# qinjr/SCoRe

Measured on AMD Instinct MI355X. Metric: train samples/sec @ batch=1024, higher is better.
Workload: dtype f32

## Files before the change

include/score_hip.h:

```cpp
#ifndef SCORE_HIP_H
#define SCORE_HIP_H

#include <stdint.h>

#ifdef __cplusplus
extern "C" {
#endif

#define SCORE_E_BADARG   (-1)
#define SCORE_E_SHAPE    (-2)
#define SCORE_E_WORKSPACE (-3)
#define SCORE_E_INDEX    (-4)

typedef void* score_context_t;
int score_context_create(score_context_t* ctx);
int score_context_destroy(score_context_t ctx);
int score_event_create(void** event);
int score_event_destroy(void* event);
int score_event_record(void* event, void* stream);
int score_stream_wait_event(void* stream, void* event);
int score_event_query(void* event);
int score_event_synchronize(void* event);

typedef struct {
// ... 17 lines not shown
  int32_t eb_dim;
  int32_t hidden_size;
  int32_t max_time_len;
  int32_t obj_per_time_slice;
  int32_t user_fnum;
  int32_t item_fnum;
  int32_t model_type;
} score_config_t;

typedef struct {
  char    name[64];
  int64_t offset;
  int32_t rows, cols;
  int32_t regularised;
  int32_t init;
} score_param_entry_t;

int score_param_layout(const score_config_t* cfg, score_param_entry_t* out, int32_t max_entries,
                       int64_t* n_floats, int64_t* n_reg_floats);

typedef struct {
  const int32_t* user_1hop;
  const int32_t* user_2hop;
  const int32_t* item_1hop;
  const int32_t* item_2hop;
  const int32_t* target_user;
  const int32_t* target_item;
  const int32_t* label;
  const int32_t* length;
  int32_t B;
  int32_t active_slices;
  const int32_t* length2;
} score_batch_t;

typedef struct {
  int64_t total_bytes;
  int64_t xside;
  int64_t atten_info;
  int64_t rsave;
  int64_t query;
  int64_t head_inp;
  int64_t att_score;
  int64_t logit;
  int64_t y_pred;
  int64_t loss;
  int64_t gru_out;
  int64_t gru_final;
  int64_t n_occurrences;
  int64_t plan_meta;
  int64_t plan_unique_rows;
  int64_t plan_remap[6];
} score_workspace_t;

int score_workspace_layout(const score_config_t* cfg, int32_t B, score_workspace_t* out);
int score_workspace_field(const score_config_t* cfg, int32_t B, const char* name, int64_t* offset, int64_t* second);


int score_stream_copy(float* dst, const float* src, int64_t n_floats, void* stream);

int score_table_init(float* table, int64_t n_local_rows, int32_t D, int64_t row_stride, int64_t row_first,
                     int64_t n_global_rows, uint64_t seed, void* stream);

int score_gather_fwd(const float* table, int64_t n_rows, int32_t D, const int32_t* idx,
                     int64_t n_idx, float* out, void* stream);

int score_coattn_fwd(const float* table, int64_t n_rows, int32_t D, int32_t F, int32_t K,
                     int32_t B, int32_t T, const int32_t* idx1, const int32_t* idx2,
                     const float* tgt, const float* W, const float* bias,
                     float* out1, int32_t ld1, float* out2, int32_t ld2,
                     float* info, int32_t ldi, float* rsave, int32_t mode, void* stream);

int score_coattn_bwd(const float* table, float* grad_table, int64_t n_rows, int32_t D, int32_t F,
                     int32_t K, int32_t B, int32_t T, const int32_t* idx1, const int32_t* idx2,
                     const float* W, const float* rsave,
                     const float* g1, int32_t ld1, const float* g2, int32_t ld2,
                     const float* ginfo, int32_t ldi, float* dzsum, float* dW,
                     float* scratch, int64_t scratch_floats, int32_t mode, void* stream);

int score_gemm(int32_t trans, int32_t M, int32_t N, int32_t K,
               const float* A, int32_t lda, const float* Bm, int32_t ldb,
               float* C, int32_t ldc, const float* bias, int32_t flags,
               float keep_prob, const uint8_t* drop_mask, uint64_t drop_seed,
               float* scratch, int64_t scratch_floats, void* stream);

int score_gemm_panel_products(int32_t trans_b, int32_t ngroups, int32_t M, int32_t N, int32_t K,
                              const float* const* A, int32_t lda, const float* const* Bm, int32_t ldb,
                              float* const* C, int32_t ldc, const float* const* bias,
                              float* images, int64_t image_floats, void* stream);
int score_gemm_panel_images(int32_t trans_b, int32_t ngroups, int32_t N, int32_t K, const float* const* Bm, int32_t ldb,
                            float* images, int64_t image_floats, void* stream);
int score_gemm_panel_run(int32_t ngroups, int32_t M, int32_t N, int32_t K, const float* const* A, int32_t lda,
                         float* const* C, int32_t ldc, const float* const* bias, const float* images,
                         int64_t image_floats, void* stream);

int score_gru_fwd(int32_t B, int32_t T, int32_t H, const float* xproj, const float* Wg, int32_t ldwg,
                  const float* Wc, int32_t ldwc, const int32_t* length,
                  float* out, int32_t ldo, float* gates_save, float* final_state, void* stream);

int score_gru_bwd(int32_t B, int32_t T, int32_t H, const float* Wg, int32_t ldwg, const float* Wc,
                  int32_t ldwc, const int32_t* length, const float* out, int32_t ldo,
                  const float* gates_save, const float* dout, int32_t lddo, const float* dfinal,
                  float* dxproj, float* rh, float* hprev, void* stream);

typedef struct {
  const int32_t* id_status;
  int32_t* skipped;
} score_guard_t;

int score_adam(float* p, float* m, float* v, const float* g, int64_t n, int64_t n_reg,
               float l2, float alpha, float beta1, float beta2, float eps, const score_guard_t* guard, void* stream);

int score_adam_dev(float* p, float* m, float* v, const float* g, int64_t n, int64_t n_reg, float l2,
                   const score_step_scalars_t* sc, float beta1, float beta2, float eps, const score_guard_t* guard,
                   void* stream);
int score_adam_rows_dev(float* p, float* m, float* v, const float* g, int64_t n_rows, int32_t D, uint8_t* row_flags,
                        const score_step_scalars_t* sc, float beta1, float beta2, float eps, const score_guard_t* guard,
                        void* stream);

int score_adam_rows(float* p, float* m, float* v, const float* g, int64_t n_rows, int32_t D,
                    uint8_t* row_flags, float alpha, float beta1, float beta2, float eps, const score_guard_t* guard,
                    void* stream);
int score_adam_rows_and_dense(float* p, float* m, float* v, const float* g, int64_t n_rows, int32_t D, uint8_t* row_flags,
                              float* wp, float* wm, float* wv, const float* wg, int64_t n, int64_t n_reg, float l2, float alpha,
                              float beta1, float beta2, float eps, const score_guard_t* guard, void* stream);

#define SCORE_ADAM_RING 64
typedef struct {
  float* p; float* m; float* v;
  const float* g;
  int64_t n_rows;
  int32_t D;
  int32_t reserved;
  uint8_t* row_flags;
  uint32_t* row_step;
  float* alpha_ring;
  float beta1, beta2, eps;
  int32_t reserved2;
  const int32_t* id_status;
  const int32_t* skipped_steps;
} score_adam_table_t;
int score_adam_touched(const score_adam_table_t* t, uint32_t step, float alpha, void* stream);
int score_adam_touched_and_dense(const score_adam_table_t* t, uint32_t step, float alpha, float* p, float* m, float* v,
                                 const float* g, int64_t n, int64_t n_reg, float l2, int32_t* skipped, void* stream);
int score_adam_unmark(const score_adam_table_t* t, uint32_t upto, void* stream);
int score_adam_touched_rows(const score_adam_table_t* t, const int32_t* rows, const int32_t* n_rows_dev, int64_t max_rows,
                            uint32_t step, float alpha, void* stream);
int score_adam_catchup_ids(const score_adam_table_t* t, const int32_t* ids, int64_t n_ids, uint32_t upto, void* stream);
int score_adam_catchup_ids_through(const score_adam_table_t* t, const int32_t* ids, int64_t n_ids, uint32_t step, float alpha,
                                   void* stream);
int score_adam_catchup_rows(const score_adam_table_t* t, int64_t row_begin, int64_t row_end, uint32_t upto, void* stream);


typedef struct {
  const float* table;
  int64_t n_table_rows;
  const float* w;
  float* workspace;
  int64_t workspace_bytes;
  int32_t scatter_mode;
  int32_t global_batch;
  int32_t gemm_mode;
  int32_t debug_flags;
  uint8_t* row_flags;
  void* gather_done_event;
  void* plan_done_event;
  const score_step_scalars_t* step_scalars;
// ... 101 lines not shown
```

score_amd/_lib.py:

```python
import ctypes as C
import os

_HERE = os.path.dirname(os.path.abspath(__file__))
LIB_PATH = os.path.join(_HERE, "lib", "libscore_hip.so")

MODEL_TYPES = {"SCORE": 0, "RIA": 1, "RCA": 2, "SCORE_USER": 3, "SCORE_ITEM": 4, "RRN": 5, "GCMC": 6, "GRU4Rec": 7, "Caser": 8, "DELF": 9,
               "DEEMS": 10, "SVDpp": 11}

MAX_PARAM_ENTRIES = 48

c_f = C.c_void_p
c_i = C.c_void_p


class Config(C.Structure):
    _fields_ = [("feature_size", C.c_int64), ("eb_dim", C.c_int32), ("hidden_size", C.c_int32),
                ("max_time_len", C.c_int32), ("obj_per_time_slice", C.c_int32),
                ("user_fnum", C.c_int32), ("item_fnum", C.c_int32), ("model_type", C.c_int32)]


class ParamEntry(C.Structure):
    _fields_ = [("name", C.c_char * 64), ("offset", C.c_int64), ("rows", C.c_int32), ("cols", C.c_int32),
                ("regularised", C.c_int32), ("init", C.c_int32)]


class Batch(C.Structure):
    _fields_ = [("user_1hop", c_i), ("user_2hop", c_i), ("item_1hop", c_i), ("item_2hop", c_i),
                ("target_user", c_i), ("target_item", c_i), ("label", c_i), ("length", c_i),
                ("B", C.c_int32), ("active_slices", C.c_int32), ("length2", c_i)]


class Workspace(C.Structure):
    _fields_ = [(n, C.c_int64) for n in
                ("total_bytes", "xside", "atten_info", "rsave", "query", "head_inp", "att_score",
                 "logit", "y_pred", "loss", "gru_out", "gru_final", "n_occurrences", "plan_meta",
                 "plan_unique_rows")] + [("plan_remap", C.c_int64 * 6)]


class State(C.Structure):
    _fields_ = [("table", c_f), ("n_table_rows", C.c_int64), ("w", c_f), ("workspace", c_f),
                ("workspace_bytes", C.c_int64), ("scatter_mode", C.c_int32), ("global_batch", C.c_int32),
                ("gemm_mode", C.c_int32), ("debug_flags", C.c_int32), ("row_flags", C.c_void_p),
                ("gather_done_event", C.c_void_p), ("plan_done_event", C.c_void_p), ("step_scalars", C.c_void_p),
                ("context", C.c_void_p), ("id_status", C.c_void_p), ("grads_done_event", C.c_void_p),
                ("loss_done_event", C.c_void_p), ("loss_host", C.c_void_p), ("plan_workspace", C.c_void_p),
                ("reserved4", C.c_int32), ("reserved3", C.c_int32)]


class Graph(C.Structure):
    _fields_ = [(n, C.c_void_p) for n in ("user_off1", "user_nbr1", "user_off2", "user_nbr2", "item_off1", "item_nbr1",
                                           "item_off2", "item_nbr2", "user_rows", "item_rows")] + \
               [(n, C.c_int32) for n in ("n_users", "n_items", "time_slice_num", "user_fnum", "item_fnum", "sample_mode")] + \
               [("user_deg2", C.c_void_p), ("item_deg2", C.c_void_p)]


class BatchOut(C.Structure):
    _fields_ = [(n, C.c_void_p) for n in ("user_1hop", "user_2hop", "item_1hop", "item_2hop", "target_user",
                                           "target_item", "label", "length")]


class AdamTable(C.Structure):
    _fields_ = [("p", C.c_void_p), ("m", C.c_void_p), ("v", C.c_void_p), ("g", C.c_void_p), ("n_rows", C.c_int64),
                ("D", C.c_int32), ("reserved", C.c_int32), ("row_flags", C.c_void_p), ("row_step", C.c_void_p),
                ("alpha_ring", C.c_void_p), ("beta1", C.c_float), ("beta2", C.c_float), ("eps", C.c_float),
                ("reserved2", C.c_int32), ("id_status", C.c_void_p), ("skipped_steps", C.c_void_p)]


class TrainStep(C.Structure):
    _fields_ = [("table", C.c_void_p), ("w", C.c_void_p), ("w_m", C.c_void_p), ("w_v", C.c_void_p), ("w_g", C.c_void_p),
                ("n_w", C.c_int64), ("n_reg", C.c_int64), ("skipped", C.c_void_p), ("reg_lambda", C.c_float),
                ("keep_prob", C.c_float), ("alpha", C.c_float), ("step", C.c_uint32), ("drop_seed", C.c_uint64),
                ("slice_lo", C.c_int64), ("slice_hi", C.c_int64), ("slice_upto", C.c_uint32), ("wait_ahead", C.c_int32),
                ("wait_sweep", C.c_int32), ("next_batch", C.c_void_p), ("next_ids", C.c_void_p), ("n_next_ids", C.c_int64),
                ("next_workspace", C.c_void_p), ("next_workspace_bytes", C.c_int64), ("loss_host", C.c_void_p),
                ("side_stream", C.c_void_p), ("ev_ahead", C.c_void_p), ("ev_sweep", C.c_void_p), ("ev_plan", C.c_void_p),
                ("ev_stage2", C.c_void_p), ("ev_b4", C.c_void_p), ("ev_grads", C.c_void_p), ("ev_loss", C.c_void_p),
                ("ev_plan_next", C.c_void_p), ("fwd_stage_events", C.c_void_p), ("plan_stream", C.c_void_p)]


class Guard(C.Structure):
    _fields_ = [("id_status", C.c_void_p), ("skipped", C.c_void_p)]


ADAM_RING = 64

_SIGS = {
    "score_context_create": [C.POINTER(C.c_void_p)],
    "score_context_destroy": [C.c_void_p],
    "score_id_status": [C.c_void_p, C.POINTER(C.c_int32), C.c_int32, C.c_void_p],
    "score_stream_copy": [c_f, c_f, C.c_int64, C.c_void_p],
    "score_table_init": [c_f, C.c_int64, C.c_int32, C.c_int64, C.c_int64, C.c_int64, C.c_uint64, C.c_void_p],
    "score_batch_assemble": [C.POINTER(Graph), c_i, c_i, C.c_int32, C.c_int32, C.c_int32, C.c_int32, C.c_int32,
                             C.c_int32, C.c_uint64, C.POINTER(BatchOut), C.c_void_p],
    "score_param_layout": [C.POINTER(Config), C.POINTER(ParamEntry), C.c_int32, C.POINTER(C.c_int64),
                           C.POINTER(C.c_int64)],
    "score_workspace_layout": [C.POINTER(Config), C.c_int32, C.POINTER(Workspace)],
    "score_workspace_field": [C.POINTER(Config), C.c_int32, C.c_char_p, C.POINTER(C.c_int64), C.POINTER(C.c_int64)],
    "score_gather_fwd": [c_f, C.c_int64, C.c_int32, c_i, C.c_int64, c_f, C.c_void_p],
    "score_coattn_fwd": [c_f, C.c_int64, C.c_int32, C.c_int32, C.c_int32, C.c_int32, C.c_int32, c_i, c_i,
                         c_f, c_f, c_f, c_f, C.c_int32, c_f, C.c_int32, c_f, C.c_int32, c_f, C.c_int32,
                         C.c_void_p],
    "score_coattn_bwd": [c_f, c_f, C.c_int64, C.c_int32, C.c_int32, C.c_int32, C.c_int32, C.c_int32, c_i, c_i,
                         c_f, c_f, c_f, C.c_int32, c_f, C.c_int32, c_f, C.c_int32, c_f, c_f, c_f, C.c_int64,
                         C.c_int32, C.c_void_p],
    "score_gemm": [C.c_int32, C.c_int32, C.c_int32, C.c_int32, c_f, C.c_int32, c_f, C.c_int32, c_f, C.c_int32,
                   c_f, C.c_int32, C.c_float, C.c_void_p, C.c_uint64, c_f, C.c_int64, C.c_void_p],
    "score_gemm_panel_images": [C.c_int32, C.c_int32, C.c_int32, C.c_int32, C.c_void_p, C.c_int32, c_f, C.c_int64, C.c_void_p],
    "score_gemm_panel_run": [C.c_int32, C.c_int32, C.c_int32, C.c_int32, C.c_void_p, C.c_int32, C.c_void_p, C.c_int32, C.c_void_p,
                             c_f, C.c_int64, C.c_void_p],
    "score_gemm_panel_products": [C.c_int32, C.c_int32, C.c_int32, C.c_int32, C.c_int32, C.c_void_p, C.c_int32, C.c_void_p,
                                  C.c_int32, C.c_void_p, C.c_int32, C.c_void_p, c_f, C.c_int64, C.c_void_p],
    "score_gru_fwd": [C.c_int32, C.c_int32, C.c_int32, c_f, c_f, C.c_int32, c_f, C.c_int32, c_i, c_f, C.c_int32,
                      c_f, c_f, C.c_void_p],
    "score_gru_bwd": [C.c_int32, C.c_int32, C.c_int32, c_f, C.c_int32, c_f, C.c_int32, c_i, c_f, C.c_int32, c_f,
                      c_f, C.c_int32, c_f, c_f, c_f, c_f, C.c_void_p],
    "score_adam": [c_f, c_f, c_f, c_f, C.c_int64, C.c_int64, C.c_float, C.c_float, C.c_float, C.c_float,
                   C.c_float, C.POINTER(Guard), C.c_void_p],
    "score_adam_dev": [c_f, c_f, c_f, c_f, C.c_int64, C.c_int64, C.c_float, C.c_void_p, C.c_float, C.c_float, C.c_float,
                       C.POINTER(Guard), C.c_void_p],
    "score_adam_rows_dev": [c_f, c_f, c_f, c_f, C.c_int64, C.c_int32, C.c_void_p, C.c_void_p, C.c_float, C.c_float,
                            C.c_float, C.POINTER(Guard), C.c_void_p],
    "score_adam_rows": [c_f, c_f, c_f, c_f, C.c_int64, C.c_int32, C.c_void_p, C.c_float, C.c_float, C.c_float,
                        C.c_float, C.POINTER(Guard), C.c_void_p],
    "score_adam_rows_and_dense": [c_f, c_f, c_f, c_f, C.c_int64, C.c_int32, C.c_void_p, c_f, c_f, c_f, c_f, C.c_int64, C.c_int64,
                                  C.c_float, C.c_float, C.c_float, C.c_float, C.c_float, C.POINTER(Guard), C.c_void_p],
    "score_adam_touched": [C.POINTER(AdamTable), C.c_uint32, C.c_float, C.c_void_p],
    "score_adam_touched_and_dense": [C.POINTER(AdamTable), C.c_uint32, C.c_float, c_f, c_f, c_f, c_f, C.c_int64, C.c_int64,
                                     C.c_float, C.c_void_p, C.c_void_p],
    "score_adam_unmark": [C.POINTER(AdamTable), C.c_uint32, C.c_void_p],
    "score_adam_touched_rows": [C.POINTER(AdamTable), c_i, c_i, C.c_int64, C.c_uint32, C.c_float, C.c_void_p],
    "score_adam_catchup_ids": [C.POINTER(AdamTable), c_i, C.c_int64, C.c_uint32, C.c_void_p],
    "score_adam_catchup_ids_through": [C.POINTER(AdamTable), c_i, C.c_int64, C.c_uint32, C.c_float, C.c_void_p],
    "score_adam_catchup_rows": [C.POINTER(AdamTable), C.c_int64, C.c_int64, C.c_uint32, C.c_void_p],
    "score_index_plan": [C.POINTER(Config), C.POINTER(State), C.POINTER(Batch), C.c_int32, C.c_int32, C.c_void_p],
    "score_sort_pairs": [C.c_void_p, C.c_void_p, C.c_void_p, C.c_void_p, C.c_int64, C.c_int32, C.c_void_p, C.c_int64,
                         C.POINTER(C.c_int32), C.c_void_p],
    "score_sort_pairs_temp_bytes": [C.c_int64],
    "score_segment_sum_rows": [c_i, c_f, C.c_int64, C.c_int32, C.c_int64, c_f, C.c_void_p, C.c_void_p, C.c_int64,
                               C.c_void_p],
    "score_segment_sum_scratch_bytes": [C.c_int64, C.c_int32],
    "score_rows_accumulate": [c_i, c_f, C.c_int64, C.c_int32, C.c_int64, c_f, C.c_void_p, C.c_void_p],
    "score_rows_accumulate_multi": [c_i, c_f, C.POINTER(C.c_int64), C.c_int32, C.c_int32, C.c_int64, c_f, C.c_void_p, C.c_void_p],
    "score_auc_logloss": [c_f, c_i, C.c_int64, C.c_void_p, C.c_void_p, C.c_int64, C.c_void_p],
    "score_auc_scratch_bytes": [C.c_int64],
    "score_ranking_quality": [c_f, c_i, C.c_int64, C.c_int32, c_f, c_i, c_f, C.c_int64, C.c_void_p],
    "score_persample_form": [C.POINTER(Config), C.POINTER(State), C.c_int32, C.c_int32],
    "score_event_create": [C.POINTER(C.c_void_p)],
    "score_event_destroy": [C.c_void_p],
    "score_event_record": [C.c_void_p, C.c_void_p],
    "score_stream_wait_event": [C.c_void_p, C.c_void_p],
    "score_event_query": [C.c_void_p],
    "score_event_synchronize": [C.c_void_p],
    "score_abi_struct_sizes": [C.POINTER(C.c_int64), C.c_int32],
    "score_train_step": [C.POINTER(Config), C.POINTER(State), C.POINTER(Batch), C.POINTER(TrainStep), C.c_void_p],
    "score_gemm_forms": [C.POINTER(Config), C.POINTER(State), C.c_int32, C.c_int32, C.POINTER(C.c_int32), C.POINTER(C.c_int32)],
    "score_forward": [C.POINTER(Config), C.POINTER(State), C.POINTER(Batch), C.c_float, C.c_float, C.c_void_p,
                      C.c_void_p, C.c_uint64, C.POINTER(C.c_void_p), C.c_void_p],
    "score_backward": [C.POINTER(Config), C.POINTER(State), C.POINTER(Batch), C.c_float, c_f, c_f,
                       C.POINTER(C.c_void_p), C.c_void_p],
}

EXPORTS = tuple(_SIGS)
_lib = None


class DevEvent(object):
    __slots__ = ("cuda_event", "_lib")

    def __init__(self):
        lib = load()
        h = C.c_void_p(0)
        check(lib.score_event_create(C.byref(h)), "score_event_create")
        self.cuda_event = h.value
        self._lib = lib

    def record(self, stream=None):
        import torch
        s = stream if stream is not None else torch.cuda.current_stream()
        check(self._lib.score_event_record(self.cuda_event, s.cuda_stream), "score_event_record")

    def wait(self, stream=None):
        import torch
        s = stream if stream is not None else torch.cuda.current_stream()
        check(self._lib.score_stream_wait_event(s.cuda_stream, self.cuda_event), "score_stream_wait_event")

    def query(self):
        rc = self._lib.score_event_query(self.cuda_event)
        if rc not in (0, 1):
            check(rc, "score_event_query")
# ... 99 lines not shown
```

score_amd/csrc/engine.hip:

```cpp
#include <string.h>
#include <stdlib.h>
#include <stdio.h>
#include <math.h>
#include <mutex>
#include <new>
#include "common.h"
#include "kernels.h"
#include "persample.h"

namespace {

const int FC1 = 200, FC2 = 80, AT1 = 80, AT2 = 40;
const int CASER_L = SCORE_CASER_L, CASER_HPAD = SCORE_CASER_HPAD;
const int MAX_ENTRIES = 48;

enum Family { FAM_SLICE, FAM_GCMC, FAM_G4R, FAM_CASER, FAM_DELF, FAM_DEEMS, FAM_SVDPP };

struct Dims {
  int64_t N;
  int D, H, T, K, Fu, Fi, mt;
  int Du, Di, I, Dq, NI, Dk, Dhead, nstate;
  int Is[2];
  bool coattn, attn;
  Family family;
// ... 397 lines not shown

void build_ws(const Dims& d, int B, WS* w) {
  struct Memo { bool ok; LayoutKey k; WS w; };
  static thread_local Memo memo = {};
  LayoutKey k = layout_key(d, B);
  if (!memo.ok || !same_key(memo.k, k)) {
    memset(&memo.k, 0, sizeof(memo.k));
    build_ws_raw(d, B, &memo.w);
    memo.k = k; memo.ok = true;
  }
  *w = memo.w;
}

struct SideStream { hipStream_t st; hipEvent_t fork, join, wx; int device; hipStream_t fwd_on; };
#define HIPTRY(call) do { hipError_t e_ = (call); if (e_ != hipSuccess) return (int)e_; } while (0)
#define SCORE_DEVICE_EVENT_FLAGS (hipEventDisableTiming | hipEventDisableSystemFence)
extern "C" int score_event_create(void** event) {
  if (!event) return SCORE_E_BADARG;
  hipEvent_t e;
  HIPTRY(hipEventCreateWithFlags(&e, SCORE_DEVICE_EVENT_FLAGS));
  *event = (void*)e;
  return 0;
}
extern "C" int score_event_destroy(void* event) {
  if (!event) return SCORE_E_BADARG;
  HIPTRY(hipEventDestroy((hipEvent_t)event));
  return 0;
}
extern "C" int score_event_record(void* event, void* stream) {
  if (!event) return SCORE_E_BADARG;
  HIPTRY(hipEventRecord((hipEvent_t)event, (hipStream_t)stream));
  return 0;
}
extern "C" int score_stream_wait_event(void* stream, void* event) {
  if (!event) return SCORE_E_BADARG;
  HIPTRY(hipStreamWaitEvent((hipStream_t)stream, (hipEvent_t)event, 0));
  return 0;
}
extern "C" int score_event_query(void* event) {
  if (!event) return SCORE_E_BADARG;
  const hipError_t e = hipEventQuery((hipEvent_t)event);
  return e == hipSuccess ? 0 : e == hipErrorNotReady ? 1 : (int)e;
}
extern "C" int score_event_synchronize(void* event) {
  if (!event) return SCORE_E_BADARG;
  HIPTRY(hipEventSynchronize((hipEvent_t)event));
  return 0;
}
static int side_stream_create(SideStream* sd) {
  int dev = 0;
  if (hipGetDevice(&dev) != hipSuccess) return SCORE_E_BADARG;
  hipStream_t st; hipEvent_t a, b, c;
  hipError_t e = hipStreamCreateWithFlags(&st, hipStreamNonBlocking);
  if (e != hipSuccess) return (int)e;
  if ((e = hipEventCreateWithFlags(&a, SCORE_DEVICE_EVENT_FLAGS)) != hipSuccess) { hipStreamDestroy(st); return (int)e; }
  if ((e = hipEventCreateWithFlags(&b, SCORE_DEVICE_EVENT_FLAGS)) != hipSuccess) { hipEventDestroy(a); hipStreamDestroy(st); return (int)e; }
  if ((e = hipEventCreateWithFlags(&c, SCORE_DEVICE_EVENT_FLAGS)) != hipSuccess) { hipEventDestroy(a); hipEventDestroy(b); hipStreamDestroy(st); return (int)e; }
  sd->st = st; sd->fork = a; sd->join = b; sd->wx = c; sd->device = dev; sd->fwd_on = nullptr;
  return 0;
}
static void side_stream_release(SideStream* sd) {
  if (!sd->st) return;
  hipStreamSynchronize(sd->st);
  hipEventDestroy(sd->fork); hipEventDestroy(sd->join); hipEventDestroy(sd->wx);
  hipStreamDestroy(sd->st);
  sd->st = nullptr;
}
#define SCORE_MAX_DEVICES 16
static SideStream g_default_ctx[SCORE_MAX_DEVICES];
static std::mutex g_default_mu;
static int side_stream(const score_state_t* st, SideStream** out) {
  if (st && st->context) { *out = reinterpret_cast<SideStream*>(st->context); return 0; }
  int dev = 0;
  if (hipGetDevice(&dev) != hipSuccess || dev < 0 || dev >= SCORE_MAX_DEVICES) return SCORE_E_BADARG;
  std::lock_guard<std::mutex> lock(g_default_mu);
  SideStream& sd = g_default_ctx[dev];
  if (!sd.st) SCORE_TRY(side_stream_create(&sd));
  *out = &sd;
  return 0;
}
enum {
  DF_GRU_STEPWISE = 1, DF_HEAD_FUSED_ANY_B = 2, DF_GRU_F32_REC = 4, DF_NO_PANEL = 8, DF_PANEL_DX = 16, DF_SORT_LIB = 32,
  DF_HEAD_UNFUSED = 64, DF_ATTN_UNFUSED = 128, DF_SORT_OWN = 256, DF_NO_PS = 512, DF_PS_FWD_ONLY = 1024, DF_PS_BWD_ONLY = 2048,
  DF_ONE_STREAM = 4096, DF_G4R_COMPOSED = 8192, DF_PRODUCTS_LATE = 16384
};
struct Flags {
  bool gru_stepwise, head_fused_any_b, gru_f32_rec, no_panel, panel_dx, sort_lib, head_unfused, attn_unfused, sort_own, no_ps,
      ps_fwd_only, ps_bwd_only, one_stream, g4r_composed, products_late;
};
static inline Flags flags_of(const score_state_t* st) {
  auto on = [st](int bit) { return (st->debug_flags & bit) != 0; };
  Flags o;
  o.gru_stepwise = on(DF_GRU_STEPWISE); o.head_fused_any_b = on(DF_HEAD_FUSED_ANY_B); o.gru_f32_rec = on(DF_GRU_F32_REC);
  o.no_panel = on(DF_NO_PANEL); o.panel_dx = on(DF_PANEL_DX); o.sort_lib = on(DF_SORT_LIB); o.sort_own = on(DF_SORT_OWN);
  o.head_unfused = on(DF_HEAD_UNFUSED); o.attn_unfused = on(DF_ATTN_UNFUSED); o.no_ps = on(DF_NO_PS);
  o.ps_fwd_only = on(DF_PS_FWD_ONLY); o.ps_bwd_only = on(DF_PS_BWD_ONLY); o.one_stream = on(DF_ONE_STREAM);
  o.g4r_composed = on(DF_G4R_COMPOSED); o.products_late = on(DF_PRODUCTS_LATE);
  return o;
}
static int side_stream(const score_state_t* st, hipStream_t s, SideStream** out) {
  SideStream* real = nullptr;
  SCORE_TRY(side_stream(st, &real));
  if (!st || !flags_of(st).one_stream) { *out = real; return 0; }
  static thread_local SideStream inl;
  const hipStream_t was = inl.fwd_on;
  inl = *real; inl.st = s; inl.fwd_on = was;
  *out = &inl;
  return 0;
}
static inline int fork_side(SideStream* side, hipStream_t s) {
  HIPTRY(hipEventRecord(side->fork, s));
  HIPTRY(hipStreamWaitEvent(side->st, side->fork, 0));
  return 0;
}

#define G(call) SCORE_TRY(call)
static inline int gemm_mode_call(int x3, int tr, int M, int N, int K, const float* A, int lda, const float* B,
                                 int ldb, float* C, int ldc, const float* bias, int flags, float keep,
                                 const uint8_t* mask, uint64_t seed, float* scratch, int64_t scratch_floats,
                                 void* s) {
  return score_gemm(tr, M, N, K, A, lda, B, ldb, C, ldc, bias, flags | x3, keep, mask, seed, scratch, scratch_floats,
                    s);
}
#define EV(i) \
  do { if (stage_events && stage_events[i]) HIPTRY(hipEventRecord((hipEvent_t)stage_events[i], s)); } while (0)

static inline uint32_t clamp_rows(int64_t n) { return (uint32_t)(n < 0x80000000ll ? n : 0x80000000ll); }
static inline int global_batch(const score_state_t* st, int B) { return st->global_batch > 0 ? st->global_batch : B; }

struct Pass {
  Dims d; Params P; WS w; Flags fl;
  const score_state_t* st; const score_batch_t* bt;
  int B, T, BT, H;
  int x3, Bg;
  uint32_t n_rows;
  int64_t weff_stride;
  float rs;
  float* ws; const float* W; float* scratch;
  hipStream_t s;
};
static int pass_fill(Pass* c, const score_state_t* st, const score_batch_t* bt, void* stream) {
  const Dims& d = c->d;
  build_layout(d, nullptr, 0, &c->P);
  c->st = st; c->bt = bt; c->fl = flags_of(st);
  c->B = bt->B; c->T = active_T(d, bt); c->H = d.H; c->BT = c->B * c->T;
  build_ws(d, c->B, &c->w);
  if (c->w.total * 4 > st->workspace_bytes) return SCORE_E_WORKSPACE;
  c->x3 = st->gemm_mode == 1 ? GF_X3 : 0; c->Bg = global_batch(st, c->B); c->n_rows = clamp_rows(st->n_table_rows);
  c->weff_stride = weff_copy_stride(d); c->rs = (float)(1.0 / sqrt(1.0 + 1e-3));
  c->ws = st->workspace; c->W = st->w; c->scratch = c->ws + c->w.scratch;
  c->s = (hipStream_t)stream;
  return 0;
}
static inline const float* wxcat(const Pass& c, int sd) { return c.ws + c.w.wxcat + (int64_t)sd * (c.d.Ic + 1) * 3 * c.H; }
static int weight_prep(const Pass& c, hipStream_t on) {
  const Dims& d = c.d; const Params& P = c.P; const WS& w = c.w; const float* W = c.W;
  return score_launch_weight_prep(W + P.gk[0], W + P.ck[0], W + P.gb[0], W + P.cb[0], W + P.gk[1], W + P.ck[1], W + P.gb[1],
                                  W + P.cb[1], d.Is[0], d.Is[1], d.Ic, d.H, c.ws + w.wxcat, d.Dk, AT1,
                                  d.attn ? W + P.at_w[1] : nullptr, c.ws + w.weff, c.ws + w.wq, SCORE_WEFF_COPIES, c.weff_stride, W,
                                  P.n_reg, c.ws + w.part, on);
}

static inline const float* gru_x_rows(const Pass& c, int sd) {
  return c.ws + (c.d.family == FAM_GCMC ? c.w.gcmc_z[sd] : (c.d.family == FAM_G4R && sd == 1) ? c.w.gru_out[0] : c.w.xside[sd]);
}

static void gru_header(const Pass& c, GruArgs* ga) {
  memset(ga, 0, sizeof(*ga));
  ga->B = c.B; ga->T = c.T; ga->H = c.H; ga->length = c.bt->length;
  ga->nw8 = 1;
  ga->tmp = c.ws + c.w.gru_tmp; ga->tmp_floats = c.w.gru_tmp_floats;
  ga->x3 = c.x3 != 0; ga->x3_rec = ga->x3 && !c.fl.gru_f32_rec; ga->stepwise = c.fl.gru_stepwise;
}
static void gru_side(const Pass& c, int sd, GruSide* g) {
  const int H = c.H;
  g->Wg = c.W + c.P.gk[sd] + (int64_t)c.d.Is[sd] * 2 * H; g->ldwg = 2 * H;
  g->Wc = c.W + c.P.ck[sd] + (int64_t)c.d.Is[sd] * H; g->ldwc = H;
  g->out = c.ws + c.w.gru_out[sd]; g->ldo = H; g->gates = c.ws + c.w.gates[sd];
}
static void gru_side_saved(const Pass& c, int sd, GruSide* g) {
// ... 216 lines not shown
  const int64_t per = score_gemm_panel_image_floats(p->Nh, p->K);
  for (int g = 0; g < p->n; ++g) {
    const int side = g / ns, half = g % ns;
    const float* cat = wxcat(c, side);
    p->src[g] = which == 0 ? cat + half * p->Nh : cat + (int64_t)half * p->Nh * 3 * H;
    p->img[g] = c.ws + (which == 0 ? c.w.pimg_x : c.w.pimg_d)[side] + half * per;
    PanelGroup& pg = p->pg[g];
    pg.A = A ? A[side] : nullptr; pg.img = p->img[g]; pg.C = C ? C[side] + half * p->Nh : nullptr;
    pg.bias = which == 0 ? cat + (int64_t)d.Is[side] * 3 * H + half * p->Nh : nullptr;
  }
}
static int panel_prep(const Pass& c, int which, hipStream_t on) {
  PanelGroups p;
  panel_groups(c, which, nullptr, nullptr, &p);
  return score_gemm_panel_prep(p.n, p.src, 3 * c.H, p.trans, p.Nh, p.K, p.img, on);
}
static int panel_launch(const Pass& c, int which, const float* const* A, float* const* C) {
  PanelGroups p;
  panel_groups(c, which, A, C, &p);
  return score_gemm_panel(p.n, p.pg, c.BT, p.Nh, p.K, p.lda, p.ldc, c.s);
}

static int loss_tail(const Pass& c, SideStream* sd, float reg_lambda) {
  const WS& w = c.w;
  hipStream_t ls = c.s;
  if (c.st->loss_done_event) { G(fork_side(sd, c.s)); ls = sd->st; }
  G(score_launch_loss_final(c.B, c.ws + w.lossb, c.ws + w.loss, reg_lambda, c.ws + w.part, c.Bg, ls, c.st->id_status));
  if (c.st->loss_done_event) HIPTRY(hipEventRecord((hipEvent_t)c.st->loss_done_event, ls));
  return 0;
}

static int row_scatter(const Pass& c, float* plan, float* grad_table) {
  const Dims& d = c.d; const Params& P = c.P; const WS& w = c.w; float* ws = c.ws; const float* W = c.W;
  PullArgs pa;
  memset(&pa, 0, sizeof(pa));
  pa.D = d.D; pa.K = d.K; pa.zero_is_dummy = 1;
  pa.flags = c.st->scatter_mode == 0 ? c.st->row_flags : nullptr;
  pa.uid = c.st->scatter_mode == 2 ? reinterpret_cast<const uint32_t*>(ws + w.uid) : nullptr;
  const float invK = 1.0f / (float)d.K;
  const float* Gm[6] = {ws + w.dxside[0], ws + w.dxside[1], ws + w.dxside[0], ws + w.dxside[1], ws + w.dtgt, ws + w.dtgt};
  const int ldg[6] = {d.I, d.I, d.I, d.I, d.Dq, d.Dq};
  const int gcol[6] = {0, d.Du, d.Di, 0, 0, d.Du};
  for (int g = 0; g < 6; ++g) { pa.G[g] = Gm[g]; pa.ldg[g] = ldg[g]; pa.gcol[g] = gcol[g]; pa.constA[g] = 1.0f; }
  if (d.coattn) {
    pa.cA[0] = ws + w.pcoef[0]; pa.cA[2] = ws + w.pcoef[1];
    pa.constA[1] = invK; pa.constA[3] = invK;
    pa.cB[0] = pa.cB[1] = ws + w.dzcoef[0]; pa.cB[2] = pa.cB[3] = ws + w.dzcoef[1];
    pa.Wv[0] = W + P.ca_w[0] + d.Di; pa.Wv[1] = W + P.ca_w[0] + 2 * d.Di;
    pa.Wv[2] = W + P.ca_w[1] + d.Du; pa.Wv[3] = W + P.ca_w[1] + 2 * d.Du;
  }
  const int64_t n_occ = (int64_t)c.B * (2 * (int64_t)c.T * d.K * (d.Fu + d.Fi) + d.Fu + d.Fi);
  return score_launch_pull(pa, reinterpret_cast<uint32_t*>(plan + w.keys_out), reinterpret_cast<uint32_t*>(plan + w.vals_out),
                           n_occ + 1, grad_table, ws + w.partials, w.partial_floats, c.s);
}

struct GradQueues { GemmQueue gq; ColsumJobs cq; };
static inline void queues_init(GradQueues* q) { q->gq.n = 0; q->cq.n = 0; q->cq.part_used = 0; }
static int queue_head(const Pass& c, GradQueues* q, float* gw, bool bn1_sums) {
  const Dims& d = c.d; const Params& P = c.P; const WS& w = c.w; float* ws = c.ws; const int B = c.B;
  G(gemm_queue_add(&q->gq, FC2, 1, B, ws + w.f2, FC2, ws + w.dlogit, 1, gw + P.fc_w[2], 1));
  G(colsum_queue_add(&q->cq, ws + w.dlogit, B, 1, 1, gw + P.fc_b[2], 0));
  G(gemm_queue_add(&q->gq, FC1, FC2, B, ws + w.f1, FC1, ws + w.dz2, FC2, gw + P.fc_w[1], FC2));
  G(colsum_queue_add(&q->cq, ws + w.dz2, B, FC2, FC2, gw + P.fc_b[1], 0));
  G(gemm_queue_add(&q->gq, d.Dhead, FC1, B, ws + w.bn, d.Dhead, ws + w.dz1, FC1, gw + P.fc_w[0], FC1));
  G(colsum_queue_add(&q->cq, ws + w.dz1, B, FC1, FC1, gw + P.fc_b[0], 0));
  if (bn1_sums) {
    G(colsum_queue_add(&q->cq, ws + w.dgstage, B, d.Dhead, d.Dhead, gw + P.bn_g, 0));
    G(colsum_queue_add(&q->cq, ws + w.dbn, B, d.Dhead, d.Dhead, gw + P.bn_b, 0));
  }
  return 0;
}
static int queue_head_tower(const Pass& c, GradQueues* q, float* gw, const DeemsArgs& a, int k) {
  const DeemsTower& t = a.t[k]; const DeemsVars v = deems_vars(c.P, k); const int B = c.B, ld = a.ld;
  G(gemm_queue_add(&q->gq, FC2, 1, B, t.f2, FC2, t.dlogit, 1, gw + v.fc_w[2], 1));
  G(colsum_queue_add(&q->cq, t.dlogit, B, 1, 1, gw + v.fc_b[2], 0));
  G(gemm_queue_add(&q->gq, FC1, FC2, B, t.f1, FC1, t.dz2, FC2, gw + v.fc_w[1], FC2));
  G(colsum_queue_add(&q->cq, t.dz2, B, FC2, FC2, gw + v.fc_b[1], 0));
  G(gemm_queue_add(&q->gq, t.Dh, FC1, B, a.bn + t.col, ld, t.dz1, FC1, gw + v.fc_w[0], FC1));
  G(colsum_queue_add(&q->cq, t.dz1, B, FC1, FC1, gw + v.fc_b[0], 0));
  G(colsum_queue_add(&q->cq, a.tmp + t.col, B, t.Dh, ld, gw + v.bn_g, 0));
  G(colsum_queue_add(&q->cq, a.dbn + t.col, B, t.Dh, ld, gw + v.bn_b, 0));
  return 0;
}
static int queue_attn(const Pass& c, GradQueues* q, float* gw) {
  const Dims& d = c.d; const Params& P = c.P; const WS& w = c.w; float* ws = c.ws; const int B = c.B, BT = c.BT;
  G(gemm_queue_add(&q->gq, AT2, 1, BT, ws + w.a2, AT2, ws + w.ds, 1, gw + P.at_w[3], 1));
  G(colsum_queue_add(&q->cq, ws + w.ds, BT, 1, 1, gw + P.at_b[3], 0));
  G(gemm_queue_add(&q->gq, AT1, AT2, BT, ws + w.a1, AT1, ws + w.da2, AT2, gw + P.at_w[2], AT2));
  G(colsum_queue_add(&q->cq, ws + w.da2, BT, AT2, AT2, gw + P.at_b[2], 0));
  G(gemm_queue_add(&q->gq, 2 * d.Dk, AT1, BT, ws + w.ainp, 2 * d.Dk, ws + w.da1, AT1, ws + w.dweff, AT1));
  G(colsum_queue_add(&q->cq, ws + w.da1, BT, AT1, AT1, gw + P.at_b[1], 0));
  G(gemm_queue_add(&q->gq, d.Dk, AT1, B, ws + w.q, d.Dk, ws + w.adzsum, AT1, ws + w.dwq, AT1));
  return 0;
}
static int queue_query(const Pass& c, GradQueues* q, float* gw) {
  const Dims& d = c.d; const Params& P = c.P; const WS& w = c.w;
  G(gemm_queue_add(&q->gq, d.Dq, d.Dk, c.B, c.ws + w.query, d.Dq, c.ws + w.dq, d.Dk, gw + P.at_w[0], d.Dk));
  G(colsum_queue_add(&q->cq, c.ws + w.dq, c.B, d.Dk, d.Dk, gw + P.at_b[0], 0));
  return 0;
}
static int queue_gru_side(const Pass& c, GradQueues* q, float* gw, int sd, int bias_rows) {
  const Dims& d = c.d; const Params& P = c.P; const WS& w = c.w; float* ws = c.ws;
  const int H = c.H, BT = c.BT, Is = d.Is[sd], ld = x_ld(d, sd);
  float* dxp = ws + w.dxproj[sd];
  const float* xin = gru_x_rows(c, sd);
  G(gemm_queue_add(&q->gq, Is, 2 * H, BT, xin, ld, dxp, 3 * H, gw + P.gk[sd], 2 * H));
  G(gemm_queue_add(&q->gq, Is, H, BT, xin, ld, dxp + 2 * H, 3 * H, gw + P.ck[sd], H));
  G(gemm_queue_add(&q->gq, H, 2 * H, BT, ws + w.hprev[sd], H, dxp, 3 * H, gw + P.gk[sd] + (int64_t)Is * 2 * H, 2 * H));
  G(gemm_queue_add(&q->gq, H, H, BT, ws + w.rh[sd], H, dxp + 2 * H, 3 * H, gw + P.ck[sd] + (int64_t)Is * H, H));
  const float* rows = bias_rows > 0 ? gru_bias_slab(c, sd) : dxp;
  const int nrows = bias_rows > 0 ? bias_rows : BT;
  G(colsum_queue_add(&q->cq, rows, nrows, 2 * H, 3 * H, gw + P.gb[sd], 0));
  G(colsum_queue_add(&q->cq, rows + 2 * H, nrows, H, 3 * H, gw + P.cb[sd], 0));
  return 0;
}

static int queue_delf(const Pass& c, GradQueues* q, float* gw) {
  const Dims& d = c.d; const Params& P = c.P; const WS& w = c.w; float* ws = c.ws; const int B = c.B, BT = c.BT;
  const int Cx[2] = {d.Di, d.Du};
  for (int s = 0; s < 2; ++s) {
    G(gemm_queue_add(&q->gq, Cx[s], Cx[s], BT, ws + w.xside[s], d.I, ws + w.delf_dpre[s], Cx[s], gw + P.dl_w[s], Cx[s]));
    G(colsum_queue_add(&q->cq, ws + w.delf_dpre[s], BT, Cx[s], Cx[s], gw + P.dl_b[s], 0));
  }
  const float* tu = ws + w.query; const float* ti = ws + w.query + d.Du;
  const float* ru = ws + w.delf_rep[0]; const float* ri = ws + w.delf_rep[1];
  const float* act = ws + w.delf_act; const float* dact = ws + w.delf_dact;
  const int LA = SCORE_DELF_ACT;
  const float* first[4] = {tu, ru, tu, ti}; const int ld1[4] = {d.Dq, d.Di, d.Dq, d.Dq}; const int n1[4] = {d.Du, d.Di, d.Du, d.Di};
  const float* second[4] = {ti, ri, ri, ru}; const int ld2[4] = {d.Dq, d.Du, d.Du, d.Di}; const int n2[4] = {d.Di, d.Du, d.Du, d.Di};
  for (int k = 0; k < 4; ++k) {
    float* gA = gw + P.dl_w[2 + 2 * k];
    G(gemm_queue_add(&q->gq, n1[k], 10, B, first[k], ld1[k], dact + 10 * k, LA, gA, 10));
    G(gemm_queue_add(&q->gq, n2[k], 10, B, second[k], ld2[k], dact + 10 * k, LA, gA + (int64_t)n1[k] * 10, 10));
    G(colsum_queue_add(&q->cq, dact + 10 * k, B, 10, LA, gw + P.dl_b[2 + 2 * k], 0));
    G(gemm_queue_add(&q->gq, 10, 4, B, act + 10 * k, LA, dact + 40 + 4 * k, LA, gw + P.dl_w[3 + 2 * k], 4));
    G(colsum_queue_add(&q->cq, dact + 40 + 4 * k, B, 4, LA, gw + P.dl_b[3 + 2 * k], 0));
  }
  G(gemm_queue_add(&q->gq, 4, 1, B, act + 56, LA, ws + w.dlogit, 1, gw + P.dl_w[10], 1));
  G(colsum_queue_add(&q->cq, ws + w.dlogit, B, 1, 1, gw + P.dl_b[10], 0));
  return 0;
}

static int queue_svdpp(const Pass& c, GradQueues* q, float* gw) {
  const int nv = c.d.Fu + c.d.Fi;
  for (int k = 0; k < nv; ++k)
    G(colsum_queue_add(&q->cq, c.ws + c.w.svdpp_dw + k, c.B, 1, nv, gw + c.P.sv_w + 4 * (int64_t)k, 0));
  return 0;
}

}

extern "C" int score_context_create(void** ctx) {
  if (!ctx) return SCORE_E_BADARG;
  SideStream* sd = new (std::nothrow) SideStream();
  if (!sd) return SCORE_E_BADARG;
  memset(sd, 0, sizeof(*sd));
  int rc = side_stream_create(sd);
  if (rc != 0) { delete sd; return rc; }
  *ctx = sd;
  return 0;
}

extern "C" int score_context_destroy(void* ctx) {
  if (ctx) {
    SideStream* sd = reinterpret_cast<SideStream*>(ctx);
    side_stream_release(sd);
    delete sd;
    return 0;
  }
  std::lock_guard<std::mutex> lock(g_default_mu);
  for (int i = 0; i < SCORE_MAX_DEVICES; ++i) side_stream_release(&g_default_ctx[i]);
  return 0;
}

extern "C" int score_id_status(int32_t* id_status, int32_t* bits, int32_t clear, void* stream) {
  if (!id_status) return SCORE_E_BADARG;
  hipStream_t s = (hipStream_t)stream;
  int32_t host = 0;
  HIPTRY(hipMemcpyAsync(&host, id_status, sizeof(host), hipMemcpyDeviceToHost, s));
  HIPTRY(hipStreamSynchronize(s));
  if (host && clear) {
    HIPTRY(hipMemsetAsync(id_status, 0, sizeof(host), s));
    HIPTRY(hipStreamSynchronize(s));
  }
  if (bits) *bits = host;
  return host ? SCORE_E_INDEX : 0;
}

extern "C" int score_param_layout(const score_config_t* cfg, score_param_entry_t* out, int32_t max_entries,
                                  int64_t* n_floats, int64_t* n_reg_floats) {
  Dims d;
  SCORE_TRY(make_dims(cfg, &d));
// ... 285 lines not shown

  {
    ReduceGroup rg;
    int cs_done = 0;
    G(gemm_queue_flush(&q.gq, 0, ws + w.dwslab, w.dwslab_floats, fs, &rg, &cq, ws + w.cs_part, w.cs_part_floats, &cs_done));
    W1Fold wf;
    memset(&wf, 0, sizeof(wf));
    wf.Dk = d.Dk; wf.NA = AT1; wf.dweff = ws + w.dweff; wf.dwq = ws + w.dwq; wf.gW1 = gw + P.at_w[1];
    G(score_launch_finish(&rg, &cq, ws + w.cs_part, w.cs_part_floats, fs, cs_done, &wf));
    if (fin_side) HIPTRY(hipEventRecord((hipEvent_t)st->grads_done_event, fs));
  }
  if (st->plan_done_event) HIPTRY(hipStreamWaitEvent(s, (hipEvent_t)st->plan_done_event, 0));
  G(row_scatter(c, st->plan_workspace ? st->plan_workspace : ws, grad_table));
  EV(4);
  EV(5);
  if (st->loss_done_event) HIPTRY(hipStreamWaitEvent(s, (hipEvent_t)st->loss_done_event, 0));
  return 0;
}
}

extern "C" int score_persample_form(const score_config_t* cfg, const score_state_t* st, int32_t B, int32_t active_slices) {
  Dims d;
  SCORE_TRY(make_dims(cfg, &d));
  if (!st || B <= 0 || active_slices < 0) return SCORE_E_BADARG;
  score_batch_t bt;
  memset(&bt, 0, sizeof(bt));
  bt.B = B; bt.active_slices = active_slices;
  PsPlan pp;
  return ps_path(d, st, &bt, active_T(d, &bt), &pp) ? 1 : 0;
}

namespace {
struct FwdState {
  float reg_lambda, keep_prob; const uint8_t *mask0, *mask1; uint64_t seed; void* const* stage_events;
  SideStream* sd;
  bool panel_x;
};

int fwd_open(const Pass& c, FwdState* f) {
  const Dims& d = c.d; const Params& P = c.P; const WS& w = c.w; const score_state_t* st = c.st; const score_batch_t* bt = c.bt;
  float* ws = c.ws; const float* W = c.W; const int B = c.B, x3 = c.x3; hipStream_t s = c.s;
  void* const* stage_events = f->stage_events;
  SideStream* sd = nullptr;
  G(side_stream(st, s, &sd));
  f->sd = sd;
  G(fork_side(sd, s));
  sd->fwd_on = s;
  G(score_launch_target_fwd(st->table, d.D, d.Fu, d.Fi, B, bt->target_user, bt->target_item, ws + w.query, d.Dq,
                            ws + w.head_inp, d.Dhead, d.off_ti, d.off_tu, sd->st, st->n_table_rows, st->id_status));
  G(weight_prep(c, sd->st));
  f->panel_x = panel_gemms(d, st, c.BT, 0);
  if (f->panel_x) G(panel_prep(c, 0, sd->st));
  if (panel_gemms(d, st, c.BT, 1)) G(panel_prep(c, 1, sd->st));
  HIPTRY(hipEventRecord(sd->wx, sd->st));
  if (d.attn) {
    float* scratch2 = ws + w.scratch2;
    G(gemm_mode_call(x3, 0, B, d.Dk, d.Dq, ws + w.query, d.Dq, W + P.at_w[0], d.Dk, ws + w.q, d.Dk, W + P.at_b[0], GF_BIAS,
                     1.f, nullptr, 0, scratch2, w.scratch_floats, sd->st));
    G(gemm_mode_call(x3, 0, B, AT1, d.Dk, ws + w.q, d.Dk, ws + w.wq, AT1, ws + w.qz, AT1, W + P.at_b[1], GF_BIAS, 1.f,
                     nullptr, 0, scratch2, w.scratch_floats, sd->st));
  }
  HIPTRY(hipEventRecord(sd->join, sd->st));
  EV(0);
  {
    CoattnArgs ca;
    CoattnCols k;
    coattn_args(c, &ca, &k);
    ca.id_status = st->id_status;
    ca.c[0].bit1 = 0; ca.c[0].bit2 = 3; ca.c[1].bit1 = 1; ca.c[1].bit2 = 2;
    const int32_t* tidx[2] = {bt->target_item, bt->target_user};
    for (int i = 0; i < 2; ++i) {
      CoattnCall& cc = ca.c[i];
      cc.tgt = ws + w.query + (i ? 0 : d.Du); cc.ldt = d.Dq; cc.tidx = tidx[i];
      cc.bias = d.coattn ? W + P.ca_b[i] : nullptr;
      cc.out1 = ws + w.xside[0] + k.col1[i]; cc.out2 = ws + w.xside[1] + k.col2[i]; cc.info = ws + w.info + k.info_col[i];
    }
    G(score_coattn_fwd_multi(ca, 2, d.D, B, s));
  }
  if (st->gather_done_event) HIPTRY(hipEventRecord((hipEvent_t)st->gather_done_event, s));
  EV(1);
  return 0;
}

int fwd_grus_two_sided(const Pass& c, const FwdState& f, const float* const* xin) {
  const Dims& d = c.d; const WS& w = c.w; float* ws = c.ws; const int H = c.H, BT = c.BT, x3 = c.x3; hipStream_t s = c.s;
  GruArgs ga;
  gru_header(c, &ga);
  float* xp[2] = {ws + w.xproj[0], ws + w.xproj[1]};
  if (d.Is[0] == d.Is[1]) {
    if (f.panel_x) {
      G(panel_launch(c, 0, xin, xp));
    } else {
      const float* Bx[2] = {wxcat(c, 0), wxcat(c, 1)};
      const float* bx[2] = {Bx[0] + (int64_t)d.Is[0] * 3 * H, Bx[1] + (int64_t)d.Is[1] * 3 * H};
      G(score_gemm_same_shape(0, 2, BT, 3 * H, d.Is[0], xin, x_ld(d, 0), Bx, 3 * H, xp, 3 * H, GF_BIAS, x3 != 0, c.scratch,
                              w.scratch_floats, s, bx));
    }
  }
  for (int sd = 0; sd < 2; ++sd) {
    const float* cat = wxcat(c, sd);
    if (d.Is[0] != d.Is[1])
      G(gemm_mode_call(x3, 0, BT, 3 * H, d.Is[sd], xin[sd], x_ld(d, sd), cat, 3 * H, xp[sd], 3 * H, cat + (int64_t)d.Is[sd] * 3 * H,
                       GF_BIAS, 1.f, nullptr, 0, c.scratch, w.scratch_floats, s));
    gru_side(c, sd, &ga.s[sd]);
    ga.s[sd].xproj = xp[sd]; ga.s[sd].final_state = ws + w.gru_final[sd];
  }
  return score_gru_fwd_multi(ga, 2, s);
}

int fwd_attention(const Pass& c, const FwdState& f) {
  const Dims& d = c.d; const Params& P = c.P; const WS& w = c.w; const score_batch_t* bt = c.bt;
  float* ws = c.ws; const float* W = c.W; const int B = c.B, T = c.T, H = c.H, BT = c.BT, x3 = c.x3; hipStream_t s = c.s;
  HIPTRY(hipStreamWaitEvent(s, f.sd->join, 0));
  int frc = c.fl.attn_unfused ? SCORE_E_SHAPE
                : score_launch_attn_fwd_fused(B, T, H, d.NI, AT1, AT2, ws + w.q, ws + w.gru_out[0], ws + w.gru_out[1],
                                              ws + w.info, ws + w.weff, ws + w.qz, W + P.at_w[2], W + P.at_b[2],
                                              W + P.at_w[3], W + P.at_b[3], bt->length, ws + w.ainp, ws + w.a1, ws + w.a2,
                                              ws + w.att_score, ws + w.head_inp, d.Dhead, d.off_u, d.off_i, s,
                                              SCORE_WEFF_COPIES, c.weff_stride);
  if (frc != SCORE_E_SHAPE) return frc;
  G(score_launch_attn_build_inp(B, T, H, d.NI, ws + w.q, ws + w.gru_out[0], ws + w.gru_out[1], ws + w.info,
                                ws + w.ainp, s));
  G(gemm_mode_call(x3, 0, BT, AT1, 2 * d.Dk, ws + w.ainp, 2 * d.Dk, ws + w.weff, AT1, ws + w.a1, AT1, ws + w.qz,
                   GF_BIAS | GF_RELU | (T << 16), 1.f, nullptr, 0, c.scratch, w.scratch_floats, s));
  int trc = c.fl.attn_unfused ? SCORE_E_SHAPE
                : score_launch_attn_tail_fwd(B, T, H, AT1, AT2, ws + w.a1, W + P.at_w[2], W + P.at_b[2], W + P.at_w[3],
                                             W + P.at_b[3], bt->length, ws + w.gru_out[0], ws + w.gru_out[1], ws + w.a2,
                                             ws + w.att_score, ws + w.head_inp, d.Dhead, d.off_u, d.off_i, s);
  if (trc != SCORE_E_SHAPE) return trc;
  G(gemm_mode_call(x3, 0, BT, AT2, AT1, ws + w.a1, AT1, W + P.at_w[2], AT2, ws + w.a2, AT2, W + P.at_b[2],
                   GF_BIAS | GF_RELU, 1.f, nullptr, 0, c.scratch, w.scratch_floats, s));
  return score_launch_attn_pool_fwd(B, T, H, AT2, ws + w.a2, W + P.at_w[3], W + P.at_b[3], bt->length,
                                    ws + w.gru_out[0], ws + w.gru_out[1], ws + w.att_score, ws + w.head_inp, d.Dhead,
                                    d.off_u, d.off_i, s);
}

int fwd_fc_head(const Pass& c, const FwdState& f) {
  const Dims& d = c.d; const Params& P = c.P; const WS& w = c.w; const score_state_t* st = c.st; const score_batch_t* bt = c.bt;
  float* ws = c.ws; const float* W = c.W; const int B = c.B, x3 = c.x3; hipStream_t s = c.s;
  const float keep_prob = f.keep_prob;
  const int dflag = keep_prob < 1.f ? GF_DROP : 0;
  int hrc = c.fl.head_unfused ? SCORE_E_SHAPE
                : score_launch_head_fwd_fused(B, d.Dhead, FC1, FC2, ws + w.head_inp, W + P.bn_g, W + P.bn_b, c.rs, W + P.fc_w[0],
                                              W + P.fc_b[0], W + P.fc_w[1], W + P.fc_b[1], W + P.fc_w[2], W + P.fc_b[2],
                                              keep_prob, f.mask0, f.mask1, f.seed, f.seed ^ 0x5DEECE66Dull,
                                              bt->label, ws + w.bn, ws + w.f1, ws + w.f2, ws + w.logit, ws + w.y_pred,
                                              ws + w.lossb, ws + w.dlogit, c.Bg, s,
                                              st->step_scalars ? &st->step_scalars->drop_seed : nullptr, ws + w.dz2,
                                              c.fl.head_fused_any_b ? 1 : 0);
  if (hrc == 0) return loss_tail(c, f.sd, f.reg_lambda);
  if (hrc != SCORE_E_SHAPE) return hrc;
  if (st->step_scalars && keep_prob < 1.f) return SCORE_E_SHAPE;
  G(score_launch_bn_fwd(B, d.Dhead, ws + w.head_inp, W + P.bn_g, W + P.bn_b, c.rs, ws + w.bn, s));
  G(gemm_mode_call(x3, 0, B, FC1, d.Dhead, ws + w.bn, d.Dhead, W + P.fc_w[0], FC1, ws + w.f1, FC1, W + P.fc_b[0],
                   GF_BIAS | GF_RELU | dflag, keep_prob, f.mask0, f.seed, c.scratch, w.scratch_floats, s));
  G(gemm_mode_call(x3, 0, B, FC2, FC1, ws + w.f1, FC1, W + P.fc_w[1], FC2, ws + w.f2, FC2, W + P.fc_b[1],
                   GF_BIAS | GF_RELU | dflag, keep_prob, f.mask1, f.seed ^ 0x5DEECE66Dull, c.scratch, w.scratch_floats, s));
  G(score_launch_head_out(B, FC2, ws + w.f2, W + P.fc_w[2], W + P.fc_b[2], bt->label, ws + w.logit, ws + w.y_pred,
                          ws + w.lossb, ws + w.dlogit, ws + w.loss, f.reg_lambda, ws + w.part, c.Bg, s, st->id_status));
  if (st->loss_done_event) HIPTRY(hipEventRecord((hipEvent_t)st->loss_done_event, s));
  return 0;
}

int fwd_slice(const Pass& c, const FwdState& f) {
  const Dims& d = c.d; const WS& w = c.w; float* ws = c.ws; const int B = c.B, H = c.H; hipStream_t s = c.s;
  void* const* stage_events = f.stage_events;
  HIPTRY(hipStreamWaitEvent(s, f.sd->wx, 0));
  const float* xin[2] = {ws + w.xside[0], ws + w.xside[1]};
  G(fwd_grus_two_sided(c, f, xin));
  EV(2);
  if (d.attn) {
    G(fwd_attention(c, f));
  } else {
    G(score_launch_copy2d(B, H, ws + w.gru_final[0], H, ws + w.head_inp, d.Dhead, s));
    G(score_launch_copy2d(B, H, ws + w.gru_final[1], H, ws + w.head_inp + H, d.Dhead, s));
  }
  EV(3);
  if (!d.attn) HIPTRY(hipStreamWaitEvent(s, f.sd->join, 0));
  G(fwd_fc_head(c, f));
  EV(4);
  return 0;
}

int fwd_gcmc(const Pass& c, const FwdState& f) {
  const Dims& d = c.d; const Params& P = c.P; const WS& w = c.w;
  float* ws = c.ws; const float* W = c.W; const int B = c.B, H = c.H, BT = c.BT; hipStream_t s = c.s;
  void* const* stage_events = f.stage_events;
  for (int sd = 0; sd < 2; ++sd) {
    const int Dx = d.Is[sd];
    G(gemm_mode_call(c.x3, 0, BT, Dx, Dx, ws + w.xside[sd], d.I, W + P.gm_a[sd], Dx, ws + w.gcmc_a[sd], Dx, nullptr, GF_RELU, 1.f,
                     nullptr, 0, c.scratch, w.scratch_floats, s));
    G(gemm_mode_call(c.x3, 0, BT, Dx, Dx, ws + w.gcmc_a[sd], Dx, W + P.gm_c[sd], Dx, ws + w.gcmc_z[sd], Dx, nullptr, GF_RELU, 1.f,
                     nullptr, 0, c.scratch, w.scratch_floats, s));
  }
  HIPTRY(hipStreamWaitEvent(s, f.sd->wx, 0));
  const float* xin[2] = {ws + w.gcmc_z[0], ws + w.gcmc_z[1]};
  G(fwd_grus_two_sided(c, f, xin));
  EV(2);
  EV(3);
  HIPTRY(hipStreamWaitEvent(s, f.sd->join, 0));
// ... 97 lines not shown
extern "C" int score_forward(const score_config_t* cfg, const score_state_t* st, const score_batch_t* bt,
                             float reg_lambda, float keep_prob, const uint8_t* drop_mask0,
                             const uint8_t* drop_mask1, uint64_t drop_seed, void* const* stage_events,
                             void* stream) {
  Pass c;
  SCORE_TRY(make_dims(cfg, &c.d));
  if (!st || !bt || !st->table || !st->w || !st->workspace || bt->B <= 0) return SCORE_E_BADARG;
  if (!bt->user_1hop || !bt->user_2hop || !bt->item_1hop || !bt->item_2hop || !bt->target_user ||
      !bt->target_item || !bt->label || !bt->length)
    return SCORE_E_BADARG;
  if ((c.d.family == FAM_DELF || c.d.family == FAM_DEEMS) && !bt->length2) return SCORE_E_BADARG;
  if (!(keep_prob > 0.f) || keep_prob > 1.f) return SCORE_E_BADARG;
  SCORE_TRY(pass_fill(&c, st, bt, stream));
  {
    PsPlan pp;
    if (!c.fl.ps_bwd_only && ps_path(c.d, st, bt, c.T, &pp))
      return forward_ps(c, pp, reg_lambda, keep_prob, drop_mask0, drop_mask1, drop_seed, stage_events);
  }
  FwdState f = {reg_lambda, keep_prob, drop_mask0, drop_mask1, drop_seed, stage_events, nullptr, false};
  SCORE_TRY(fwd_open(c, &f));
  switch (c.d.family) {
    case FAM_SLICE: return fwd_slice(c, f);
    case FAM_GCMC: return fwd_gcmc(c, f);
    case FAM_G4R: return fwd_g4r(c, f);
    case FAM_CASER: return fwd_caser(c, f);
    case FAM_DELF: return fwd_delf(c, f);
    case FAM_DEEMS: return fwd_deems(c, f);
    case FAM_SVDPP: return fwd_svdpp(c, f);
  }
  return SCORE_E_BADARG;
}

namespace {
struct BwdState {
  float keep_prob; float* gw; float* grad_table; void* const* stage_events;
  SideStream* side;
  GradQueues q;
  const float* dfinal[2];
  int gru_bias_rows;
};
inline int64_t slab_half(const WS& w) { return (w.dwslab_floats / 4) & ~(int64_t)3; }

int bwd_open(const Pass& c, BwdState* b) {
  hipStream_t s = c.s;
  void* const* stage_events = b->stage_events;
  SideStream* side = nullptr;
  G(side_stream(c.st, s, &side));
  b->side = side;
  const bool forked = side->fwd_on == s;
  side->fwd_on = nullptr;
  if (!forked) G(fork_side(side, s));
  HIPTRY(hipMemsetAsync(b->gw, 0, c.P.n_floats * sizeof(float), side->st));
  EV(0);
  return 0;
}

int bwd_fc_head(const Pass& c, BwdState* b) {
  const Dims& d = c.d; const Params& P = c.P; const WS& w = c.w;
  float* ws = c.ws; const float* W = c.W; float* gw = b->gw; const int B = c.B, x3 = c.x3; hipStream_t s = c.s;
  const float keep_prob = b->keep_prob; const int64_t SF = w.scratch_floats;
  if (c.fl.head_unfused || !score_head_fwd_fused_fits(B, d.Dhead, FC1, FC2))
    G(score_launch_outer_relu_bwd(B, FC2, ws + w.dlogit, W + P.fc_w[2], ws + w.f2, keep_prob, ws + w.dz2, s));
  int hbrc = c.fl.head_unfused ? SCORE_E_SHAPE
                 : score_launch_head_bwd_fused(B, d.Dhead, FC1, FC2, ws + w.dz2, W + P.fc_w[1], ws + w.f1, keep_prob,
                                               W + P.fc_w[0], ws + w.head_inp, W + P.bn_g, c.rs, ws + w.dz1, ws + w.dbn,
                                               ws + w.dhead, ws + w.dgstage, s);
  if (hbrc != 0 && hbrc != SCORE_E_SHAPE) return hbrc;
  G(queue_head(c, &b->q, gw, hbrc == 0));
  if (hbrc == SCORE_E_SHAPE) {
    G(gemm_mode_call(x3, 1, B, FC1, FC2, ws + w.dz2, FC2, W + P.fc_w[1], FC2, ws + w.dz1, FC1, nullptr, GF_RELUGRAD, keep_prob,
                     reinterpret_cast<const uint8_t*>(ws + w.f1), 0, c.scratch, SF, s));
    G(gemm_mode_call(x3, 1, B, d.Dhead, FC1, ws + w.dz1, FC1, W + P.fc_w[0], FC1, ws + w.dbn, d.Dhead, nullptr, 0, 1.f,
                     nullptr, 0, c.scratch, SF, s));
    G(score_launch_bn_bwd(B, d.Dhead, ws + w.head_inp, W + P.bn_g, c.rs, ws + w.dbn, ws + w.dhead, gw + P.bn_g,
                          gw + P.bn_b, ws + w.dgstage, c.scratch, SF, &b->q.cq, s));
  }
  return 0;
}

int bwd_attention(const Pass& c, BwdState* b) {
  const Dims& d = c.d; const Params& P = c.P; const WS& w = c.w; const score_batch_t* bt = c.bt;
  float* ws = c.ws; const float* W = c.W; const int B = c.B, T = c.T, H = c.H, BT = c.BT, x3 = c.x3; hipStream_t s = c.s;
  const int64_t SF = w.scratch_floats;
  G(queue_attn(c, &b->q, b->gw));
  const bool pool_in_fused = !c.fl.attn_unfused && (int64_t)B * T < 8192 &&
                             score_attn_inp_bwd_fused_fits(B, T, H, d.NI, AT1, AT2, d.Dhead, d.off_u, d.off_i, true);
  int prc = pool_in_fused ? 0 : c.fl.attn_unfused ? SCORE_E_SHAPE
                : score_launch_attn_pool_bwd(B, T, H, AT2, ws + w.a2, W + P.at_w[3], bt->length, ws + w.gru_out[0],
                                             ws + w.gru_out[1], ws + w.att_score, ws + w.dhead, d.Dhead, d.off_u,
                                             d.off_i, ws + w.ds, ws + w.da2, s, AT1, W + P.at_w[2], ws + w.a1, ws + w.da1);
  if (prc != 0 && prc != SCORE_E_SHAPE) return prc;
  const bool da1_done = prc == 0;
  if (!da1_done) {
    G(score_launch_attn_pool_bwd(B, T, H, AT2, ws + w.a2, W + P.at_w[3], bt->length, ws + w.gru_out[0],
                                 ws + w.gru_out[1], ws + w.att_score, ws + w.dhead, d.Dhead, d.off_u, d.off_i,
                                 ws + w.ds, ws + w.da2, s));
    G(gemm_mode_call(x3, 1, BT, AT1, AT2, ws + w.da2, AT2, W + P.at_w[2], AT2, ws + w.da1, AT1, nullptr, GF_RELUGRAD, 1.f,
                     reinterpret_cast<const uint8_t*>(ws + w.a1), 0, c.scratch, SF, s));
  }
  int brc = c.fl.attn_unfused ? SCORE_E_SHAPE
            : pool_in_fused
                ? score_launch_attn_inp_bwd_fused(B, T, H, d.NI, AT1, nullptr, ws + w.weff, ws + w.q, ws + w.gru_out[0],
                                                  ws + w.gru_out[1], ws + w.info, ws + w.att_score, ws + w.dhead, d.Dhead,
                                                  d.off_u, d.off_i, ws + w.dgru[0], ws + w.dgru[1], ws + w.dinfo, ws + w.dq, s,
                                                  AT2, ws + w.a2, ws + w.a1, W + P.at_w[3], W + P.at_w[2], bt->length,
                                                  ws + w.ds, ws + w.da2, ws + w.da1)
                : score_launch_attn_inp_bwd_fused(B, T, H, d.NI, AT1, ws + w.da1, ws + w.weff, ws + w.q, ws + w.gru_out[0],
                                                  ws + w.gru_out[1], ws + w.info, ws + w.att_score, ws + w.dhead, d.Dhead,
                                                  d.off_u, d.off_i, ws + w.dgru[0], ws + w.dgru[1], ws + w.dinfo, ws + w.dq, s);
  if (pool_in_fused && brc != 0) return brc == SCORE_E_SHAPE ? SCORE_E_BADARG : brc;
  if (brc != 0 && brc != SCORE_E_SHAPE) return brc;
  if (brc == SCORE_E_SHAPE) {
    G(gemm_mode_call(x3, 1, BT, 2 * d.Dk, AT1, ws + w.da1, AT1, ws + w.weff, AT1, ws + w.dainp, 2 * d.Dk, nullptr, 0,
                     1.f, nullptr, 0, c.scratch, SF, s));
    G(score_launch_attn_inp_bwd(B, T, H, d.NI, ws + w.dainp, ws + w.q, ws + w.gru_out[0], ws + w.gru_out[1],
                                ws + w.info, ws + w.att_score, ws + w.dhead, d.Dhead, d.off_u, d.off_i,
                                nullptr, ws + w.dgru[0], ws + w.dgru[1], ws + w.dinfo, ws + w.dq, s));
  }
  return 0;
}

int bwd_zero_dinfo(const Pass& c) {
  HIPTRY(hipMemsetAsync(c.ws + c.w.dinfo, 0, (int64_t)c.BT * 4 * c.d.K * sizeof(float), c.s));
  return 0;
}
int bwd_final_state(const Pass& c, BwdState* b, int sd, int head_col, bool zero_dout) {
  const WS& w = c.w; float* ws = c.ws; const int H = c.H;
  if (head_col >= 0) G(score_launch_copy2d(c.B, H, ws + w.dhead + head_col, c.d.Dhead, ws + w.dfinal[sd], H, c.s));
  b->dfinal[sd] = ws + w.dfinal[sd];
  if (zero_dout) HIPTRY(hipMemsetAsync(ws + w.dgru[sd], 0, (int64_t)c.BT * H * sizeof(float), c.s));
  return 0;
}
int bwd_final_states(const Pass& c, BwdState* b, bool from_head) {
  for (int sd = 0; sd < 2; ++sd) G(bwd_final_state(c, b, sd, from_head ? sd * c.H : -1, true));
  return bwd_zero_dinfo(c);
}

int bwd_side_products(const Pass& c, BwdState* b) {
  const Dims& d = c.d; const Params& P = c.P; const WS& w = c.w; const score_state_t* st = c.st;
  float* ws = c.ws; const float* W = c.W; float* gw = b->gw; const int B = c.B, x3 = c.x3; hipStream_t s = c.s;
  const int64_t SF = w.scratch_floats;
  SideStream* side = b->side;
  G(fork_side(side, s));
  const bool q_on_side = st->scatter_mode != 2;
  hipStream_t qs = q_on_side ? side->st : s;
  if (d.attn) {
    float* scratch2 = q_on_side ? ws + w.scratch2 : c.scratch;
    G(score_launch_attn_dzsum(B, c.T, AT1, ws + w.da1, ws + w.adzsum, qs));
    G(gemm_mode_call(x3, 1, B, d.Dk, AT1, ws + w.adzsum, AT1, ws + w.wq, AT1, ws + w.dq, d.Dk, nullptr, GF_ACC, 1.f, nullptr,
                     0, scratch2, SF, qs));
    G(queue_query(c, &b->q, gw));
    G(gemm_mode_call(x3, 1, B, d.Dq, d.Dk, ws + w.dq, d.Dk, W + P.at_w[0], d.Dk, ws + w.dquery, d.Dq, nullptr, 0, 1.f,
                     nullptr, 0, scratch2, SF, qs));
    if (q_on_side) HIPTRY(hipEventRecord(side->wx, side->st));
    else G(fork_side(side, s));
  }
  G(gemm_queue_flush(&b->q.gq, x3 != 0, ws + w.dwslab, slab_half(w), side->st));
  if (d.attn) G(score_launch_attn_w1_grad(d.Dk, AT1, ws + w.dweff, ws + w.dwq, gw + P.at_w[1], side->st));
  if (q_on_side) G(colsum_queue_flush(&b->q.cq, ws + w.cs_part, w.cs_part_floats / 2, side->st));
  HIPTRY(hipEventRecord(side->join, side->st));
  return 0;
}

int bwd_grus_two_sided(const Pass& c, BwdState* b) {
  GruArgs ga;
  gru_header(c, &ga);
  for (int sd = 0; sd < 2; ++sd) {
    gru_side(c, sd, &ga.s[sd]);
    gru_side_bwd(c, sd, b->dfinal[sd], &ga.s[sd]);
  }
  G(score_gru_bwd_multi(ga, 2, c.s));
  b->gru_bias_rows = ga.bias_slab_rows;
  return 0;
}

int bwd_dx_slice(const Pass& c, BwdState* b) {
  const Dims& d = c.d; const WS& w = c.w; float* ws = c.ws; const int H = c.H, BT = c.BT, x3 = c.x3; hipStream_t s = c.s;
  const int64_t SF = w.scratch_floats;
  for (int sd = 0; sd < 2; ++sd) {
    G(queue_gru_side(c, &b->q, b->gw, sd, b->gru_bias_rows));
    if (d.Is[sd] != d.I)
      HIPTRY(hipMemsetAsync(ws + w.dxside[sd], 0, (int64_t)BT * d.I * sizeof(float), s));
    if (d.Is[0] != d.Is[1])
      G(gemm_mode_call(x3, 1, BT, d.Is[sd], 3 * H, ws + w.dxproj[sd], 3 * H, wxcat(c, sd), 3 * H, ws + w.dxside[sd], d.I, nullptr, 0,
                       1.f, nullptr, 0, c.scratch, SF, s));
  }
  if (d.Is[0] == d.Is[1]) {
    const float* Ad[2] = {ws + w.dxproj[0], ws + w.dxproj[1]};
    float* Cd[2] = {ws + w.dxside[0], ws + w.dxside[1]};
    if (panel_gemms(d, c.st, BT, 1)) {
      G(panel_launch(c, 1, Ad, Cd));
    } else {
      const float* Bd[2] = {wxcat(c, 0), wxcat(c, 1)};
      G(score_gemm_same_shape(1, 2, BT, d.Is[0], 3 * H, Ad, 3 * H, Bd, 3 * H, Cd, d.I, 0, x3 != 0, c.scratch, SF, s));
    }
  }
  return 0;
}

int bwd_dx_gcmc(const Pass& c, BwdState* b) {
  const Dims& d = c.d; const Params& P = c.P; const WS& w = c.w;
  float* ws = c.ws; const float* W = c.W; float* gw = b->gw; const int H = c.H, BT = c.BT, x3 = c.x3; hipStream_t s = c.s;
  const int64_t SF = w.scratch_floats;
  GemmQueue& gq = b->q.gq;
  for (int sd = 0; sd < 2; ++sd) {
    G(queue_gru_side(c, &b->q, gw, sd, b->gru_bias_rows));
    HIPTRY(hipMemsetAsync(ws + w.dxside[sd], 0, (int64_t)BT * d.I * sizeof(float), s));
    const int Dx = d.Is[sd];
    float* dz = ws + w.gcmc_dz[sd];
    float* da = ws + w.gcmc_da[sd];
    G(gemm_mode_call(x3, 1, BT, Dx, 3 * H, ws + w.dxproj[sd], 3 * H, wxcat(c, sd), 3 * H, dz, Dx, nullptr, GF_RELUGRAD, 1.f,
                     reinterpret_cast<const uint8_t*>(ws + w.gcmc_z[sd]), 0, c.scratch, SF, s));
    G(gemm_queue_add(&gq, Dx, Dx, BT, ws + w.gcmc_a[sd], Dx, dz, Dx, gw + P.gm_c[sd], Dx));
    G(gemm_mode_call(x3, 1, BT, Dx, Dx, dz, Dx, W + P.gm_c[sd], Dx, da, Dx, nullptr, GF_RELUGRAD, 1.f,
                     reinterpret_cast<const uint8_t*>(ws + w.gcmc_a[sd]), 0, c.scratch, SF, s));
    G(gemm_queue_add(&gq, Dx, Dx, BT, ws + w.xside[sd], d.I, da, Dx, gw + P.gm_a[sd], Dx));
    G(gemm_mode_call(x3, 1, BT, Dx, Dx, da, Dx, W + P.gm_a[sd], Dx, ws + w.dxside[sd], d.I, nullptr, 0, 1.f, nullptr, 0,
                     c.scratch, SF, s));
  }
  return 0;
}

int bwd_dx_g4r(const Pass& c, BwdState* b) {
  const Dims& d = c.d; const WS& w = c.w; float* ws = c.ws; const int H = c.H, BT = c.BT; hipStream_t s = c.s;
  G(queue_gru_side(c, &b->q, b->gw, 0, b->gru_bias_rows));
  HIPTRY(hipMemsetAsync(ws + w.dxside[0], 0, (int64_t)BT * d.I * sizeof(float), s));
  G(gemm_mode_call(c.x3, 1, BT, d.Di, 3 * H, ws + w.dxproj[0], 3 * H, wxcat(c, 0), 3 * H, ws + w.dxside[0], d.I, nullptr, 0, 1.f,
                   nullptr, 0, c.scratch, w.scratch_floats, s));
  G(queue_gru_side(c, &b->q, b->gw, 1, b->gru_bias_rows));
  HIPTRY(hipMemsetAsync(ws + w.dxside[1], 0, (int64_t)BT * d.I * sizeof(float), s));
  return 0;
}

int bwd_close(const Pass& c, BwdState* b) {
  const Dims& d = c.d; const Params& P = c.P; const WS& w = c.w; const score_state_t* st = c.st; const score_batch_t* bt = c.bt;
  float* ws = c.ws; const float* W = c.W; float* gw = b->gw; float* grad_table = b->grad_table;
  const int B = c.B, x3 = c.x3; hipStream_t s = c.s;
  void* const* stage_events = b->stage_events;
  SideStream* side = b->side;
  GemmQueue& gq = b->q.gq;
  ColsumJobs& cq = b->q.cq;
  const int64_t half = slab_half(w);
  ReduceGroup rg; rg.n = rg.blocks = 0;
  const bool products_early = st->scatter_mode != 2 && !c.fl.products_late && gq.n > 0;
  const bool fin_side = st->grads_done_event != nullptr;
  const bool fin_early = products_early && fin_side;
  if (products_early) {
    G(fork_side(side, s));
    G(gemm_queue_flush(&gq, x3 != 0, ws + w.dwslab + half, w.dwslab_floats - half, side->st, &rg));
    HIPTRY(hipEventRecord(side->join, side->st));
  }
  EV(3);
  const bool atomic = st->scatter_mode == 1;
  {
    CoattnArgs ca;
    CoattnCols k;
    coattn_args(c, &ca, &k);
    ca.gtable = grad_table;
    for (int i = 0; i < 2; ++i) {
      CoattnCall& cc = ca.c[i];
      cc.g1 = ws + w.dxside[0] + k.col1[i]; cc.g2 = ws + w.dxside[1] + k.col2[i]; cc.ginfo = ws + w.dinfo + k.info_col[i];
      cc.dzsum = ws + w.dzsum[i]; cc.pcoef = ws + w.pcoef[i]; cc.dzcoef = ws + w.dzcoef[i];
    }
// ... 201 lines not shown
```

score_amd/csrc/gemm.hip:

```cpp
#include <cstring>
#include "common.h"
#include "kernels.h"

typedef float f32x16 __attribute__((ext_vector_type(16)));

#define BK_ALIGN 32
#ifndef GEMM_SPLITK_MIN_K
#define GEMM_SPLITK_MIN_K 512
#define GEMM_SPLITK_MIN_CHUNK 128
#endif

#define KF_MASK (15 | 64 | 0x7FFF0000)

template <int TRANS, int WM, int WN, int BK>
__device__ __forceinline__ void gemm_f32_body(const GemmGroup& grp, int blk, const float* __restrict__ bias, int flags,
                                              float keep, const uint8_t* __restrict__ mask, uint64_t seed) {
  int pi = 0, local = blk;
  while (pi + 1 < grp.n && local >= ((grp.p[pi].nblocks + 7) & ~7)) { local -= (grp.p[pi].nblocks + 7) & ~7; ++pi; }
  const GemmProb& pr = grp.p[pi];
  if (local >= pr.nblocks) return;
  const int M = pr.M, N = pr.N, K = pr.K, lda = pr.lda, ldb = pr.ldb, ldc = pr.ldc, k_chunk = pr.k_chunk;
  const float* __restrict__ A = pr.A;
  const float* __restrict__ Bm = pr.B;
  float* __restrict__ C = pr.C;
// ... 103 lines not shown
    __syncthreads();
    if (k0 + BK >= kend) break;
    store_tiles(ra1, rb1);
    __syncthreads();
    if (k0 + 3 * BK < kend) load_tiles(k0 + 3 * BK, ra1, rb1);
    mfma_tile();
    __syncthreads();
  }

#pragma unroll
  for (int i = 0; i < WM; ++i)
#pragma unroll
    for (int j = 0; j < WN; ++j) {
      const int col = bn + bcol + 32 * j;
      if (col >= N) continue;
#pragma unroll
      for (int r = 0; r < 16; ++r) {
        const int row = bm + wm * 32 * WM + 32 * i + (r & 3) + 8 * (r >> 2) + 4 * khalf;
        if (row >= M) continue;
        if (slab) {
          slab[((int64_t)bz * M + row) * N + col] = acc[i][j][r];
        } else {
          float v = gemm_epilogue(acc[i][j][r], row, col, N, pr.bias ? pr.bias : bias, flags, keep, mask, seed);
          float* dst = C + (int64_t)row * ldc + col;
          *dst = (flags & GF_ACC) ? *dst + v : v;
        }
      }
    }
}
template <int TRANS, int WM, int WN, int BK>
__global__ __launch_bounds__(256) void gemm_f32_kernel(const GemmGroup grp, const float* __restrict__ bias, int flags,
                                                       float keep, const uint8_t* __restrict__ mask, uint64_t seed) {
  gemm_f32_body<TRANS, WM, WN, BK>(grp, (int)blockIdx.x, bias, flags, keep, mask, seed);
}

__global__ void splitk_reduce_kernel(const float* __restrict__ slab, int nsplit, int M, int N,
                                     float* __restrict__ C, int ldc, const float* __restrict__ bias, int flags,
                                     float keep, const uint8_t* __restrict__ mask, uint64_t seed) {
  int64_t i = (int64_t)blockIdx.x * blockDim.x + threadIdx.x;
  if (i >= (int64_t)M * N) return;
  int row = (int)(i / N), col = (int)(i - (int64_t)row * N);
  const int64_t stride = (int64_t)M * N;
  float s = 0.f;
  int z = 0;
  for (; z + 8 <= nsplit; z += 8) {
    float v[8];
#pragma unroll
    for (int q = 0; q < 8; ++q) v[q] = slab[(int64_t)(z + q) * stride + i];
#pragma unroll
    for (int q = 0; q < 8; ++q) s += v[q];
  }
  for (; z < nsplit; ++z) s += slab[(int64_t)z * stride + i];
  float v = gemm_epilogue(s, row, col, N, bias, flags, keep, mask, seed);
  float* dst = C + (int64_t)row * ldc + col;
  *dst = (flags & GF_ACC) ? *dst + v : v;
}

__device__ __forceinline__ void splitk_reduce_group_body(const ReduceGroup& g, int blk) {
  int ji = 0;
  while (ji + 1 < g.n && blk >= g.j[ji + 1].first_block) ++ji;
  const ReduceJob& job = g.j[ji];
  const int64_t n = (int64_t)job.M * job.N;
  const int64_t i = (int64_t)(blk - job.first_block) * blockDim.x + threadIdx.x;
  if (i >= n) return;
  const int row = (int)(i / job.N), col = (int)(i - (int64_t)row * job.N);
  float s = 0.f;
  int z = 0;
  for (; z + 8 <= job.ns; z += 8) {
    float v[8];
#pragma unroll
    for (int q = 0; q < 8; ++q) v[q] = job.slab[(int64_t)(z + q) * n + i];
#pragma unroll
    for (int q = 0; q < 8; ++q) s += v[q];
  }
  for (; z < job.ns; ++z) s += job.slab[(int64_t)z * n + i];
  job.C[(int64_t)row * job.ldc + col] = s;
}
__global__ void splitk_reduce_group_kernel(const ReduceGroup g) { splitk_reduce_group_body(g, (int)blockIdx.x); }

static void fill_prob(GemmProb* p, int M, int N, int K, const float* A, int lda, const float* B, int ldb, float* C,
                      int ldc, int k_chunk, float* slab, int gx, int gy, int gz) {
  p->A = A; p->B = B; p->C = C; p->slab = slab; p->bias = nullptr; p->M = M; p->N = N; p->K = K; p->lda = lda; p->ldb = ldb;
  p->ldc = ldc; p->k_chunk = k_chunk; p->gx = gx; p->gy = gy; p->nblocks = gx * gy * gz;
}

extern "C" int score_gemm(int32_t trans, int32_t M, int32_t N, int32_t K, const float* A, int32_t lda,
                          const float* Bm, int32_t ldb, float* C, int32_t ldc, const float* bias,
                          int32_t flags, float keep_prob, const uint8_t* drop_mask, uint64_t drop_seed,
                          float* scratch, int64_t scratch_floats, void* stream) {
  if (!A || !Bm || !C || M <= 0 || N <= 0 || K <= 0) return SCORE_E_BADARG;
  if (trans < 0 || trans > 2) return SCORE_E_BADARG;
  if ((flags & GF_BIAS) && !bias) return SCORE_E_BADARG;
  if (flags < 0) return SCORE_E_BADARG;
  if ((flags & GF_RELUGRAD) && (!drop_mask || (flags & GF_DROP))) return SCORE_E_BADARG;
  hipStream_t s = (hipStream_t)stream;
  const bool a_kc = trans != 2, b_kc = trans == 1;
  const bool al_a = (lda & 3) == 0 && (reinterpret_cast<uintptr_t>(A) & 15) == 0;
  const bool al_b = (ldb & 3) == 0 && (reinterpret_cast<uintptr_t>(Bm) & 15) == 0;
  const bool x3_ok = al_a && al_b && (a_kc ? (K & 3) == 0 : (M & 3) == 0) && (b_kc ? (K & 3) == 0 : (N & 3) == 0);
  const bool x3_shape = (trans == 0 && M >= 4096 && N >= 64) ||
                        (trans == 1 && M >= 4096 && N >= 256) ||
                        (trans == 2 && (int64_t)M * N >= 32768 && K >= 4096);
  const bool x3_force = (flags & 32) != 0;
  if ((flags & (GF_X3 | 32)) && x3_ok && M >= 64 && N >= 32 && K >= 32 && (x3_shape || x3_force)) {
    auto rounds = [&](int wm_) {
      int64_t blocks = (int64_t)((N + 127) / 128) * ((M + 64 * wm_ - 1) / (64 * wm_));
      return (double)((blocks + 255) / 256) * (wm_ == 2 ? 1.0 : 0.57);
    };
    const int wm3 = rounds(1) < rounds(2) ? 1 : 2;
    dim3 g3((N + 127) / 128, (M + 64 * wm3 - 1) / (64 * wm3), 1);
    int ns = 1;
    int64_t t3 = (int64_t)g3.x * g3.y;
    if (t3 < 256 && K >= 512 && scratch) {
      ns = (int)((320 + t3 - 1) / t3);
      if (ns > K / 128) ns = K / 128;
      while (ns > 1 && (int64_t)ns * M * N > scratch_floats) --ns;
      if (ns < 1) ns = 1;
    }
    int kc = K;
    float* sl = nullptr;
    if (ns > 1) {
      kc = (int)align_up64(cdiv64(K, ns), 32);
      ns = (int)cdiv64(K, kc);
      g3.z = ns;
      sl = ns > 1 ? scratch : nullptr;
    }
    GemmGroup grp;
    grp.n = 1;
    fill_prob(&grp.p[0], M, N, K, A, lda, Bm, ldb, C, ldc, kc, sl, (int)g3.x, (int)g3.y, (int)g3.z);
    grp.total_blocks = (grp.p[0].nblocks + 7) & ~7;
    SCORE_TRY(score_launch_gemm_bf16x3(trans, wm3, grp, bias, flags & KF_MASK, keep_prob, drop_mask, drop_seed, s));
    if (sl) {
      int64_t n = (int64_t)M * N;
      hipLaunchKernelGGL(splitk_reduce_kernel, dim3((unsigned)cdiv64(n, 256)), dim3(256), 0, s, sl, ns, M, N, C, ldc,
                         bias, flags & KF_MASK, keep_prob, drop_mask, drop_seed);
      SCORE_CHECK_LAUNCH();
    }
    return 0;
  }
  flags &= KF_MASK;
  int WMs = 1, WNs = 1;
  auto nblocks = [&](int wm_, int wn_) { return (int64_t)((N + 64 * wn_ - 1) / (64 * wn_)) * ((M + 64 * wm_ - 1) / (64 * wm_)); };
  const int64_t want = 384;
  const int64_t ksplit_cap = (K >= GEMM_SPLITK_MIN_K && scratch) ? K / GEMM_SPLITK_MIN_CHUNK : 1;
  if (N > 64 && nblocks(1, 2) * ksplit_cap >= want) WNs = 2;
  if (M > 64 && nblocks(2, WNs) * ksplit_cap >= want) WMs = 2;
  const int BMh = 64 * WMs, BNh = 64 * WNs;
  dim3 grid((N + BNh - 1) / BNh, (M + BMh - 1) / BMh, 1);
  int nsplit = 1;
  int64_t tiles = (int64_t)grid.x * grid.y;
  if (tiles < 256 && K >= GEMM_SPLITK_MIN_K && scratch) {
    nsplit = (int)((320 + tiles - 1) / tiles);
    int max_split = K / GEMM_SPLITK_MIN_CHUNK;
    if (nsplit > max_split) nsplit = max_split;
    while (nsplit > 1 && (int64_t)nsplit * M * N > scratch_floats) --nsplit;
    if (nsplit < 1) nsplit = 1;
  }
  int k_chunk = K;
  float* slab = nullptr;
  if (nsplit > 1) {
    k_chunk = (int)align_up64(cdiv64(K, nsplit), BK_ALIGN);
    nsplit = (int)cdiv64(K, k_chunk);
    grid.z = nsplit;
    slab = nsplit > 1 ? scratch : nullptr;
  }
  GemmGroup grp;
  grp.n = 1;
  fill_prob(&grp.p[0], M, N, K, A, lda, Bm, ldb, C, ldc, k_chunk, slab, (int)grid.x, (int)grid.y, (int)grid.z);
  grp.total_blocks = (grp.p[0].nblocks + 7) & ~7;
#define LAUNCH(TR, WMv, WNv)                                                                                       \
  hipLaunchKernelGGL((gemm_f32_kernel<TR, WMv, WNv, 16>), dim3(grp.total_blocks), dim3(256), 0, s, grp, bias, flags, \
                     keep_prob, drop_mask, drop_seed)
#define LAUNCH_T(TR)                                      \
  do {                                                    \
    if (WMs == 2 && WNs == 2) LAUNCH(TR, 2, 2);           \
    else if (WMs == 2) LAUNCH(TR, 2, 1);                  \
    else if (WNs == 2) LAUNCH(TR, 1, 2);                  \
    else LAUNCH(TR, 1, 1);                                \
  } while (0)
  if (trans == 0) LAUNCH_T(0);
  else if (trans == 1) LAUNCH_T(1);
  else LAUNCH_T(2);
#undef LAUNCH_T
#undef LAUNCH
  SCORE_CHECK_LAUNCH();
  if (slab) {
    int64_t n = (int64_t)M * N;
    hipLaunchKernelGGL(splitk_reduce_kernel, dim3((unsigned)cdiv64(n, 256)), dim3(256), 0, s, slab, nsplit, M, N,
                       C, ldc, bias, flags, keep_prob, drop_mask, drop_seed);
    SCORE_CHECK_LAUNCH();
  }
  return 0;
}

int score_gemm_same_shape(int trans, int nprob, int M, int N, int K, const float* const* A, int lda,
                          const float* const* B, int ldb, float* const* C, int ldc, int flags, int x3, float* scratch,
                          int64_t scratch_floats, hipStream_t s, const float* const* bias) {
  if (nprob <= 0 || nprob > GEMM_GROUP_MAX || trans < 0 || trans > 2 || (flags & ~(GF_ACC | GF_BIAS))) return SCORE_E_BADARG;
  if ((flags & GF_BIAS) && !bias) return SCORE_E_BADARG;
  bool al = (lda & 3) == 0 && (ldb & 3) == 0;
  for (int i = 0; i < nprob; ++i)
    al = al && (reinterpret_cast<uintptr_t>(A[i]) & 15) == 0 && (reinterpret_cast<uintptr_t>(B[i]) & 15) == 0;
  const bool a_kc = trans != 2, b_kc = trans == 1;
  const bool x3_ok = al && (a_kc ? (K & 3) == 0 : (M & 3) == 0) && (b_kc ? (K & 3) == 0 : (N & 3) == 0) && M >= 64 &&
                     N >= 32 && K >= 32;
  const bool x3_shape = (trans == 0 && M >= 4096 && N >= 64) || (trans == 1 && M >= 4096 && N >= 256);
  GemmGroup grp;
  grp.n = nprob; grp.total_blocks = 0;
  if (x3 && x3_ok && x3_shape) {
    const int64_t t2 = (int64_t)nprob * ((N + 127) / 128) * ((M + 127) / 128);
    const int64_t t1 = (int64_t)nprob * ((N + 127) / 128) * ((M + 63) / 64);
    auto rounds = [](int64_t blocks, double w) { return (double)((blocks + 255) / 256) * w; };
    const int wm = rounds(t1, 0.57) < rounds(t2, 1.0) ? 1 : 2;
    if ((wm == 2 ? t2 : t1) >= 128) {
      for (int i = 0; i < nprob; ++i) {
        fill_prob(&grp.p[i], M, N, K, A[i], lda, B[i], ldb, C[i], ldc, K, nullptr, (N + 127) / 128,
                  (M + 64 * wm - 1) / (64 * wm), 1);
        grp.p[i].bias = bias ? bias[i] : nullptr;
        grp.total_blocks += (grp.p[i].nblocks + 7) & ~7;
      }
      return score_launch_gemm_bf16x3(trans, wm, grp, nullptr, flags, 1.f, nullptr, 0, s);
    }
  }
  const int64_t tiles = (int64_t)nprob * ((N + 63) / 64) * ((M + 63) / 64);
  if (tiles < 128 && K >= GEMM_SPLITK_MIN_K && scratch) {
    for (int i = 0; i < nprob; ++i)
      SCORE_TRY(score_gemm(trans, M, N, K, A[i], lda, B[i], ldb, C[i], ldc, bias ? bias[i] : nullptr, flags | (x3 ? GF_X3 : 0),
                           1.f, nullptr, 0, scratch, scratch_floats, s));
    return 0;
  }
  for (int i = 0; i < nprob; ++i) {
    fill_prob(&grp.p[i], M, N, K, A[i], lda, B[i], ldb, C[i], ldc, K, nullptr, (N + 63) / 64, (M + 63) / 64, 1);
    grp.p[i].bias = bias ? bias[i] : nullptr;
    grp.total_blocks += (grp.p[i].nblocks + 7) & ~7;
  }
#define LS(TR) hipLaunchKernelGGL((gemm_f32_kernel<TR, 1, 1, 16>), dim3(grp.total_blocks), dim3(256), 0, s, grp, nullptr, \
                                  flags, 1.f, nullptr, 0)
  if (trans == 0) LS(0); else if (trans == 1) LS(1); else LS(2);
#undef LS
  SCORE_CHECK_LAUNCH();
  return 0;
}

int gemm_queue_add(GemmQueue* q, int M, int N, int K, const float* A, int lda, const float* B, int ldb, float* C,
                   int ldc) {
  if (!q || !A || !B || !C || M <= 0 || N <= 0 || K <= 0) return SCORE_E_BADARG;
  if (q->n >= 2 * GEMM_GROUP_MAX) return SCORE_E_WORKSPACE;
  GemmQueueJob& j = q->j[q->n++];
  j.A = A; j.B = B; j.C = C; j.M = M; j.N = N; j.K = K; j.lda = lda; j.ldb = ldb; j.ldc = ldc;
  return 0;
}

__global__ void gemm_colsum_kernel(const GemmGroup grp, const ColsumJobs jobs, float* __restrict__ part, int gemm_blocks, int gx);
int gemm_queue_flush(GemmQueue* q, int x3, float* slab, int64_t slab_floats, hipStream_t s, ReduceGroup* defer,
                     const ColsumJobs* with_colsums, float* cs_part, int64_t cs_part_floats, int* colsums_done) {
  if (colsums_done) *colsums_done = 0;
  if (defer) defer->n = defer->blocks = 0;
  if (!q || q->n == 0) return 0;
  if (!slab) return SCORE_E_BADARG;
  GemmGroup g3, gf;
  g3.n = gf.n = 0; g3.total_blocks = gf.total_blocks = 0;
  int fam[2 * GEMM_GROUP_MAX];
  int64_t work[2] = {0, 0};
  for (int i = 0; i < q->n; ++i) {
    const GemmQueueJob& j = q->j[i];
    const bool al = (j.lda & 3) == 0 && (j.ldb & 3) == 0 && (reinterpret_cast<uintptr_t>(j.A) & 15) == 0 &&
                    (reinterpret_cast<uintptr_t>(j.B) & 15) == 0 && (j.M & 3) == 0 && (j.N & 3) == 0;
    fam[i] = (x3 && al && j.M >= 64 && j.N >= 32 && (int64_t)j.M * j.N >= 16384 && j.K >= 4096) ? 1 : 0;
    const int64_t tiles = fam[i] ? (int64_t)((j.M + 127) / 128) * ((j.N + 127) / 128)
                                 : (int64_t)((j.M + 63) / 64) * ((j.N + 63) / 64);
    work[fam[i]] += tiles * j.K;
  }
  int kc[2];
  kc[1] = (int)align_up64(cdiv64(work[1] > 0 ? work[1] : 1, 512), 32);
  if (kc[1] < 256) kc[1] = 256;
  for (int guard = 0; guard < 256; ++guard) {
    int64_t blocks = 0;
    for (int i = 0; i < q->n; ++i)
      if (fam[i]) {
        const GemmQueueJob& j = q->j[i];
        blocks += ((int64_t)((j.M + 127) / 128) * ((j.N + 127) / 128) * cdiv64(j.K, kc[1]) + 7) & ~(int64_t)7;
      }
    if (blocks <= 512 || kc[1] >= 1 << 24) break;
    kc[1] += (int)align_up64(kc[1] / 64 > 32 ? kc[1] / 64 : 32, 32);
  }
  kc[0] = (int)align_up64(cdiv64(work[0] > 0 ? work[0] : 1, 1024), BK_ALIGN);
  if (kc[0] < 128) kc[0] = 128;
  ReduceGroup rg;
  rg.n = 0;
  int rblocks = 0;
  int64_t used = 0;
  for (int i = 0; i < q->n; ++i) {
    const GemmQueueJob& j = q->j[i];
    GemmGroup& g = fam[i] ? g3 : gf;
    if (g.n >= GEMM_GROUP_MAX) return SCORE_E_WORKSPACE;
    const int gx = fam[i] ? (j.N + 127) / 128 : (j.N + 63) / 64, gy = fam[i] ? (j.M + 127) / 128 : (j.M + 63) / 64;
    int chunk = kc[fam[i]];
    int ns = (int)cdiv64(j.K, chunk);
    const int64_t mn = (int64_t)j.M * j.N;
    while (ns > 1 && used + (int64_t)ns * mn > slab_floats) {
      chunk *= 2;
      ns = (int)cdiv64(j.K, chunk);
    }
    float* sl = nullptr;
    if (ns > 1) {
      sl = slab + used;
      used += align_up64((int64_t)ns * mn, 4);
      ReduceJob& r = rg.j[rg.n++];
      r.slab = sl; r.C = j.C; r.ns = ns; r.M = j.M; r.N = j.N; r.ldc = j.ldc; r.first_block = rblocks; r.pad = 0;
      rblocks += (int)cdiv64(mn, 256);
    } else {
      chunk = j.K;
    }
    fill_prob(&g.p[g.n], j.M, j.N, j.K, j.A, j.lda, j.B, j.ldb, j.C, j.ldc, chunk, sl, gx, gy, ns);
    g.total_blocks += (g.p[g.n].nblocks + 7) & ~7;
    ++g.n;
  }
  if (g3.n) SCORE_TRY(score_launch_gemm_bf16x3(2, 2, g3, nullptr, 0, 1.f, nullptr, 0, s));
  if (gf.n && with_colsums && with_colsums->n > 0 && cs_part && with_colsums->part_used <= cs_part_floats) {
    int gx = 1;
    for (int i = 0; i < with_colsums->n; ++i)
      gx = max(gx, (with_colsums->job[i].N + with_colsums->job[i].cols - 1) / with_colsums->job[i].cols);
    const int64_t cs_blocks = (int64_t)gx * COLSUM_MAX_PARTS * with_colsums->n;
    hipLaunchKernelGGL(gemm_colsum_kernel, dim3((unsigned)(gf.total_blocks + cs_blocks)), dim3(256), 0, s, gf, *with_colsums, cs_part,
                       gf.total_blocks, gx);
    SCORE_CHECK_LAUNCH();
    if (colsums_done) *colsums_done = 1;
  } else if (gf.n) {
    hipLaunchKernelGGL((gemm_f32_kernel<2, 1, 1, 16>), dim3(gf.total_blocks), dim3(256), 0, s, gf, nullptr, 0, 1.f, nullptr,
                       0);
    SCORE_CHECK_LAUNCH();
  }
  rg.blocks = rblocks;
  if (defer) {
    *defer = rg;
  } else if (rg.n) {
    hipLaunchKernelGGL(splitk_reduce_group_kernel, dim3(rblocks), dim3(256), 0, s, rg);
    SCORE_CHECK_LAUNCH();
  }
  q->n = 0;
  return 0;
}

__global__ __launch_bounds__(256) void colsum_stage1(const float* __restrict__ X, int M, int N, int ld, int cols,
                                                     int rows_per_block, float* __restrict__ part) {
  __shared__ float sh[256];
  const int tx = threadIdx.x % cols, ty = threadIdx.x / cols, nty = 256 / cols;
  const int n = blockIdx.x * cols + tx;
  const int m0 = blockIdx.y * rows_per_block, m1 = min(M, m0 + rows_per_block);
  float s = 0.f;
  if (n < N)
    for (int m = m0 + ty; m < m1; m += nty) s += X[(int64_t)m * ld + n];
  sh[threadIdx.x] = s;
  __syncthreads();
  if (ty == 0 && n < N) {
    float t = 0.f;
    for (int r = 0; r < nty; ++r) t += sh[r * cols + tx];
    part[(int64_t)blockIdx.y * N + n] = t;
  }
}
__global__ void colsum_stage2(const float* __restrict__ part, int nparts, int N, float* __restrict__ out,
                              int accumulate) {
  int n = blockIdx.x * blockDim.x + threadIdx.x;
  if (n >= N) return;
  float s = 0.f;
  for (int p = 0; p < nparts; ++p) s += part[(int64_t)p * N + n];
  out[n] = accumulate ? out[n] + s : s;
}

int score_launch_colsum(const float* X, int M, int N, int ld, float* out, int accumulate, float* scratch,
                        int64_t scratch_floats, hipStream_t s) {
  int cols = 1;
  while (cols < N && cols < 64) cols <<= 1;
  int rpb = 128;
  int nparts = (M + rpb - 1) / rpb;
  if (nparts > 32) { nparts = 32; rpb = (M + nparts - 1) / nparts; nparts = (M + rpb - 1) / rpb; }
  if ((int64_t)nparts * N > scratch_floats) return SCORE_E_WORKSPACE;
  hipLaunchKernelGGL(colsum_stage1, dim3((N + cols - 1) / cols, nparts), dim3(256), 0, s, X, M, N, ld, cols, rpb,
                     scratch);
  SCORE_CHECK_LAUNCH();
  hipLaunchKernelGGL(colsum_stage2, dim3((N + 63) / 64), dim3(64), 0, s, scratch, nparts, N, out, accumulate);
  SCORE_CHECK_LAUNCH();
  return 0;
}

__device__ __forceinline__ void colsum_multi_stage1_body(const ColsumJobs& jobs, float* __restrict__ part, int bx, int by, int bz) {
  __shared__ float sh[256];
  const ColsumJob& j = jobs.job[bz];
  const int cols = j.cols, nty = 256 / cols;
  if (by >= j.nparts || bx * cols >= j.N) return;
  const int tx = threadIdx.x % cols, ty = threadIdx.x / cols;
  const int n = bx * cols + tx;
  const int m0 = by * j.rpb, m1 = min(j.M, m0 + j.rpb);
  float s = 0.f;
  if (n < j.N) {
    const float* x = j.X + n;
    int m = m0 + ty;
    float s0 = 0.f, s1 = 0.f, s2 = 0.f, s3 = 0.f;
    if (j.scale) {
      const float* sc = j.scale;
      for (; m + 3 * nty < m1; m += 4 * nty) {
        const float v0 = x[(int64_t)m * j.ld], v1 = x[(int64_t)(m + nty) * j.ld];
        const float v2 = x[(int64_t)(m + 2 * nty) * j.ld], v3 = x[(int64_t)(m + 3 * nty) * j.ld];
        const float c0 = sc[m], c1 = sc[m + nty], c2 = sc[m + 2 * nty], c3 = sc[m + 3 * nty];
        s0 = fmaf(v0, c0, s0); s1 = fmaf(v1, c1, s1); s2 = fmaf(v2, c2, s2); s3 = fmaf(v3, c3, s3);
      }
      for (; m < m1; m += nty) s0 = fmaf(x[(int64_t)m * j.ld], sc[m], s0);
    } else {
      for (; m + 3 * nty < m1; m += 4 * nty) {
        const float v0 = x[(int64_t)m * j.ld], v1 = x[(int64_t)(m + nty) * j.ld];
        const float v2 = x[(int64_t)(m + 2 * nty) * j.ld], v3 = x[(int64_t)(m + 3 * nty) * j.ld];
        s0 += v0; s1 += v1; s2 += v2; s3 += v3;
      }
      for (; m < m1; m += nty) s0 += x[(int64_t)m * j.ld];
    }
    s = (s0 + s1) + (s2 + s3);
  }
  sh[threadIdx.x] = s;
  __syncthreads();
  if (ty == 0 && n < j.N) {
    float t = 0.f;
    for (int r = 0; r < nty; ++r) t += sh[r * cols + tx];
    part[j.part_off + (int64_t)by * j.N + n] = t;
  }
// ... 140 lines not shown
```

score_amd/csrc/gemm_bf16x3.hip:

```cpp
#include <type_traits>
#include "common.h"
#include "kernels.h"

typedef __bf16 bf16x8 __attribute__((ext_vector_type(8)));
typedef float f32x16 __attribute__((ext_vector_type(16)));

#define TBN 128
#define TBK 32
#define TLD 40

template <int TRANS, int WM>
__global__ __launch_bounds__(256, 2) void gemm_bf16x3_kernel(const GemmGroup grp, const float* __restrict__ bias, int flags,
                                                             float keep, const uint8_t* __restrict__ mask,
                                                             uint64_t seed) {
  int pi = 0, local = (int)blockIdx.x;
  while (pi + 1 < grp.n && local >= ((grp.p[pi].nblocks + 7) & ~7)) { local -= (grp.p[pi].nblocks + 7) & ~7; ++pi; }
  const GemmProb& pr = grp.p[pi];
  if (local >= pr.nblocks) return;
  const int M = pr.M, N = pr.N, K = pr.K, lda = pr.lda, ldb = pr.ldb, ldc = pr.ldc, k_chunk = pr.k_chunk;
  const float* __restrict__ A = pr.A;
  const float* __restrict__ Bm = pr.B;
  float* __restrict__ C = pr.C;
  float* __restrict__ slab = pr.slab;
  constexpr int TBM = 64 * WM;
  constexpr int EA = TBM * TBK / 256;
  __shared__ __attribute__((aligned(16))) unsigned short Ap[3][TBM * TLD];
  __shared__ __attribute__((aligned(16))) unsigned short Bp[3][TBN * TLD];
  const int tid = threadIdx.x;
  const int lane = tid & 63;
  const int wave = tid >> 6;
  const int wm = wave >> 1, wn = wave & 1;
  int bx, by, bz;
  xcd_tile_coords_n(pr.nblocks, local, pr.gx, pr.gy, bx, by, bz);
  const int bm = by * TBM, bn = bx * TBN;
  const int kbeg = bz * k_chunk;
  const int kend = min(K, kbeg + k_chunk);
  constexpr bool A_KCONTIG = (TRANS != 2);
  constexpr bool B_KCONTIG = (TRANS == 1);

  constexpr int XA = A_KCONTIG ? EA : 16;
  constexpr int NA4 = XA / 4;
  float xa[XA], xb[16];
  uint32_t pa[3 * XA / 2], pb[24];
  uint32_t offa[NA4], offb[4];
  int ka[NA4], kb4[4];
  const bool a_mine = A_KCONTIG || (tid >> 3) * 4 < TBM;
#pragma unroll
  for (int rep = 0; rep < NA4; ++rep) {
    if (A_KCONTIG) {
      const int q = tid + 256 * (rep >> 1);
      const int kq = (q & 3) * 8 + (rep & 1) * 4;
      offa[rep] = (uint32_t)min(bm + (q >> 2), M - 1) * (uint32_t)lda + (uint32_t)kq;
      ka[rep] = kq;
    } else {
      offa[rep] = (uint32_t)((tid & 7) * 4 + rep) * (uint32_t)lda + (uint32_t)min(bm + (tid >> 3) * 4, M - 4);
      ka[rep] = (tid & 7) * 4 + rep;
    }
  }
#pragma unroll
  for (int rep = 0; rep < 4; ++rep) {
    if (B_KCONTIG) {
      const int q = tid + 256 * (rep >> 1);
      const int kq = (q & 3) * 8 + (rep & 1) * 4;
      offb[rep] = (uint32_t)min(bn + (q >> 2), N - 1) * (uint32_t)ldb + (uint32_t)kq;
      kb4[rep] = kq;
    } else {
      offb[rep] = (uint32_t)((tid & 7) * 4 + rep) * (uint32_t)ldb + (uint32_t)min(bn + (tid >> 3) * 4, N - 4);
      kb4[rep] = (tid & 7) * 4 + rep;
    }
  }
  constexpr int NQ = NA4 + 4;
  auto quad_src = [&](int qd, int e) -> float& {
    if (qd < NA4) return A_KCONTIG ? xa[qd * 4 + e] : xa[e * 4 + qd];
    return B_KCONTIG ? xb[(qd - NA4) * 4 + e] : xb[e * 4 + (qd - NA4)];
  };
  auto quad_k = [&](int qd, int e) -> int {
    if (qd < NA4) return A_KCONTIG ? ka[qd] : ka[e];
    return B_KCONTIG ? kb4[qd - NA4] : kb4[e];
  };
  auto quad_dst = [&](int qd, int p, int d) -> uint32_t& {
    if (qd < NA4) return A_KCONTIG ? pa[p * 2 * NA4 + qd * 2 + d] : pa[p * 8 + qd * 2 + d];
    return B_KCONTIG ? pb[p * 8 + (qd - NA4) * 2 + d] : pb[p * 8 + (qd - NA4) * 2 + d];
  };
  auto load_one = [&](int which, int rep, int k0, auto kcheck) {
    constexpr bool KCHECK = decltype(kcheck)::value;
    const bool kc = which == 0 ? A_KCONTIG : B_KCONTIG;
    const float* X = which == 0 ? A : Bm;
    const int ld = which == 0 ? lda : ldb;
    const uint32_t off = which == 0 ? offa[rep] : offb[rep];
    const int krel = which == 0 ? ka[rep] : kb4[rep];
    const float* src = X + (kc ? (int64_t)k0 : (int64_t)k0 * ld) + off;
    if (KCHECK) src = (k0 + krel < kend) ? src : X;
#if defined(X3_PROBE_NOLOADA) || defined(X3_PROBE_NOLOADB)
#ifdef X3_PROBE_NOLOADA
    if (which == 0) return;
#endif
#ifdef X3_PROBE_NOLOADB
    if (which == 1) return;
#endif
#endif
    const float4 v = ld4(src);
    float* dst = which == 0 ? &xa[rep * 4] : &xb[rep * 4];
    dst[0] = v.x; dst[1] = v.y; dst[2] = v.z; dst[3] = v.w;
  };
  auto load_all = [&](int k0, auto kcheck) {
#pragma unroll
    for (int rep = 0; rep < NA4; ++rep) load_one(0, rep, k0, kcheck);
#pragma unroll
    for (int rep = 0; rep < 4; ++rep) load_one(1, rep, k0, kcheck);
  };
  uint32_t sh[4], sm[4], sl[4];
  auto split_micro = [&](int m, int k1, int k2, auto kcheck) {
    constexpr bool KCHECK = decltype(kcheck)::value;
    const int qd = m / 5, step = m % 5;
    if (step < 4) {
      float x = quad_src(qd, step);
      if (KCHECK) x = (k1 + quad_k(qd, step) < kend) ? x : 0.f;
#ifdef X3_PROBE_NOSPLIT
      sh[step] = sm[step] = sl[step] = __float_as_uint(x);
#else
      split3(x, sh[step], sm[step], sl[step]);
#endif
      if (step == 3) {
        const bool is_a = qd < NA4;
        const bool kc = is_a ? A_KCONTIG : B_KCONTIG;
        if (kc) {
          load_one(is_a ? 0 : 1, is_a ? qd : qd - NA4, k2, kcheck);
        } else if (qd == (is_a ? NA4 - 1 : NQ - 1)) {
#pragma unroll
          for (int rep = 0; rep < 4; ++rep) load_one(is_a ? 0 : 1, rep, k2, kcheck);
        }
      }
    } else {
      quad_dst(qd, 0, 0) = pack2(sh[0], sh[1]); quad_dst(qd, 0, 1) = pack2(sh[2], sh[3]);
      quad_dst(qd, 1, 0) = pack2(sm[0], sm[1]); quad_dst(qd, 1, 1) = pack2(sm[2], sm[3]);
      quad_dst(qd, 2, 0) = pack2(sl[0], sl[1]); quad_dst(qd, 2, 1) = pack2(sl[2], sl[3]);
    }
  };
  auto write_tiles = [&]() {
#ifdef X3_PROBE_NOLDSW
    if (pa[0] != 0x12345678u || pb[0] != 0x12345678u) return;
#endif
    if (A_KCONTIG) {
#pragma unroll
      for (int pr = 0; pr < NA4 / 2; ++pr) {
        const int q = tid + 256 * pr;
#pragma unroll
        for (int p = 0; p < 3; ++p)
          *reinterpret_cast<uint4*>(&Ap[p][(q >> 2) * TLD + (q & 3) * 8]) =
              make_uint4(pa[p * 2 * NA4 + pr * 4], pa[p * 2 * NA4 + pr * 4 + 1], pa[p * 2 * NA4 + pr * 4 + 2],
                         pa[p * 2 * NA4 + pr * 4 + 3]);
      }
    } else if (a_mine) {
#pragma unroll
      for (int e = 0; e < 4; ++e)
#pragma unroll
        for (int p = 0; p < 3; ++p)
          *reinterpret_cast<uint2*>(&Ap[p][((tid >> 3) * 4 + e) * TLD + (tid & 7) * 4]) =
              make_uint2(pa[p * 8 + e * 2], pa[p * 8 + e * 2 + 1]);
    }
    if (B_KCONTIG) {
#pragma unroll
      for (int pr = 0; pr < 2; ++pr) {
        const int q = tid + 256 * pr;
#pragma unroll
        for (int p = 0; p < 3; ++p)
          *reinterpret_cast<uint4*>(&Bp[p][(q >> 2) * TLD + (q & 3) * 8]) =
              make_uint4(pb[p * 8 + pr * 4], pb[p * 8 + pr * 4 + 1], pb[p * 8 + pr * 4 + 2], pb[p * 8 + pr * 4 + 3]);
      }
    } else {
#pragma unroll
      for (int e = 0; e < 4; ++e)
#pragma unroll
        for (int p = 0; p < 3; ++p)
          *reinterpret_cast<uint2*>(&Bp[p][((tid >> 3) * 4 + e) * TLD + (tid & 7) * 4]) =
              make_uint2(pb[p * 8 + e * 2], pb[p * 8 + e * 2 + 1]);
    }
  };

  f32x16 acc[WM][2];
#pragma unroll
  for (int i = 0; i < WM; ++i)
#pragma unroll
    for (int j = 0; j < 2; ++j)
#pragma unroll
      for (int e = 0; e < 16; ++e) acc[i][j][e] = 0.f;

  const int r31 = lane & 31, kh = lane >> 5;
  constexpr int KS = TBK / 16;
  constexpr int NM1 = 6 * WM * 2;
  constexpr int NM = KS * NM1;
  constexpr int NF1 = 3 * (WM + 2);
  constexpr int MU = NQ * 5;
  bf16x8 af[KS][WM][3], bf[KS][2][3];
  auto read_frag = [&](int ks, int f) {
    const int p = f / (WM + 2), i = f % (WM + 2);
#ifdef X3_PROBE_NOLDSR
    {
      uint4 z = make_uint4(pa[0], pa[1], pb[0], pb[1] + (uint32_t)f);
      if (i < WM) af[ks][i][p] = __builtin_bit_cast(bf16x8, z); else bf[ks][i - WM][p] = __builtin_bit_cast(bf16x8, z);
      return;
    }
#endif
    if (i < WM) {
      const uint4 va = *reinterpret_cast<const uint4*>(&Ap[p][(wm * 32 * WM + i * 32 + r31) * TLD + ks * 16 + kh * 8]);
      af[ks][i][p] = __builtin_bit_cast(bf16x8, va);
    } else {
      const uint4 vb = *reinterpret_cast<const uint4*>(&Bp[p][(wn * 64 + (i - WM) * 32 + r31) * TLD + ks * 16 + kh * 8]);
      bf[ks][i - WM][p] = __builtin_bit_cast(bf16x8, vb);
    }
  };
  auto phase = [&](int k0, auto kcheck) {
    constexpr int TA[6] = {1, 0, 2, 0, 1, 0}, TB[6] = {1, 2, 0, 1, 0, 0};
#pragma unroll
    for (int f = 0; f < NF1; ++f) read_frag(0, f);
#ifdef X3_SETPRIO
    __builtin_amdgcn_s_setprio(X3_SETPRIO);
#endif
#pragma unroll
    for (int g = 0; g < NM; ++g) {
      const int ks = g / NM1, t = (g % NM1) / (WM * 2), i = (g / 2) % WM, j = g % 2;
      if (KS > 1 && g >= NM1 - NF1 - 2 && g < NM1 - 2) read_frag(1, g - (NM1 - NF1 - 2));
#ifdef X3_PROBE_NOMFMA
      acc[i][j][g % 16] += (float)af[ks][i][TA[t]][0] * (float)bf[ks][j][TB[t]][0];
#else
      acc[i][j] = __builtin_amdgcn_mfma_f32_32x32x16_bf16(af[ks][i][TA[t]], bf[ks][j][TB[t]], acc[i][j], 0, 0, 0);
#endif
#pragma unroll
      for (int m = g * MU / NM; m < (g + 1) * MU / NM; ++m) split_micro(m, k0 + TBK, k0 + 2 * TBK, kcheck);
      __builtin_amdgcn_sched_barrier(0);
    }
#ifdef X3_SETPRIO
    __builtin_amdgcn_s_setprio(0);
#endif
  };

  const int nfull = (kend - kbeg) / TBK;
  load_all(kbeg, std::true_type());
#pragma unroll
  for (int m = 0; m < MU; ++m) {
    const int qd = m / 5, step = m % 5;
    (void)qd; (void)step;
    split_micro(m, kbeg, kbeg + TBK, std::true_type());
  }
  int k0 = kbeg;
  for (int t = 0; t + 2 < nfull; ++t, k0 += TBK) {
    write_tiles();
    __syncthreads();
    phase(k0, std::false_type());
    __syncthreads();
  }
  for (; k0 < kend; k0 += TBK) {
    write_tiles();
    __syncthreads();
    phase(k0, std::true_type());
    __syncthreads();
  }

#pragma unroll
  for (int i = 0; i < WM; ++i)
#pragma unroll
    for (int j = 0; j < 2; ++j) {
      const int col = bn + wn * 64 + j * 32 + r31;
      if (col >= N) continue;
      const float* bsrc = pr.bias ? pr.bias : bias;
      const int bg = flags >> 16;
      float eb[16], ey[16], ec[16];
      const bool has_b = !slab && (flags & GF_BIAS), has_y = !slab && (flags & GF_RELUGRAD), has_c = !slab && (flags & GF_ACC);
      int rows[16];
#pragma unroll
      for (int r = 0; r < 16; ++r) rows[r] = min(bm + wm * 32 * WM + i * 32 + (r & 3) + 8 * (r >> 2) + 4 * kh, M - 1);
      if (has_b) {
        if (bg) {
#pragma unroll
          for (int r = 0; r < 16; ++r) eb[r] = bsrc[(int64_t)(rows[r] / bg) * N + col];
        } else {
          const float b0 = bsrc[col];
#pragma unroll
          for (int r = 0; r < 16; ++r) eb[r] = b0;
        }
      }
      if (has_y) {
#pragma unroll
        for (int r = 0; r < 16; ++r) ey[r] = reinterpret_cast<const float*>(mask)[(int64_t)rows[r] * N + col];
      }
      if (has_c) {
#pragma unroll
        for (int r = 0; r < 16; ++r) ec[r] = C[(int64_t)rows[r] * ldc + col];
      }
#pragma unroll
      for (int r = 0; r < 16; ++r) {
        const int row = bm + wm * 32 * WM + i * 32 + (r & 3) + 8 * (r >> 2) + 4 * kh;
        if (row >= M) continue;
#ifdef X3_PROBE_NOSTORE
        if (acc[i][j][r] != 12345.678f) continue;
#endif
        if (slab) {
          slab[((int64_t)bz * M + row) * N + col] = acc[i][j][r];
        } else {
          float v = acc[i][j][r];
          if (has_b) v += eb[r];
          if (flags & GF_RELU) v = fmaxf(v, 0.f);
          if (flags & GF_DROP) {
            const uint64_t e = (uint64_t)row * (uint64_t)N + (uint64_t)col;
            const bool on = mask ? (mask[e] != 0) : (hash_uniform(seed, e) < keep);
            v = on ? v / keep : 0.f;
          }
          if (has_y) v = ey[r] > 0.f ? v / keep : 0.f;
          C[(int64_t)row * ldc + col] = has_c ? ec[r] + v : v;
        }
      }
    }
}

int score_launch_gemm_bf16x3(int trans, int wm, const GemmGroup& g, const float* bias, int flags, float keep,
                             const uint8_t* mask, uint64_t seed, hipStream_t s) {
#define LX(TR, WMv)                                                                                              \
  hipLaunchKernelGGL((gemm_bf16x3_kernel<TR, WMv>), dim3(g.total_blocks), dim3(256), 0, s, g, bias, flags, keep, mask, \
                     seed)
  if (wm == 2) {
    if (trans == 0) LX(0, 2);
    else if (trans == 1) LX(1, 2);
    else LX(2, 2);
  } else {
    if (trans == 0) LX(0, 1);
    else if (trans == 1) LX(1, 1);
    else LX(2, 1);
  }
#undef LX
  SCORE_CHECK_LAUNCH();
  return 0;
}
```

score_amd/csrc/gru_x3.hip:

```cpp
#include <algorithm>
#include "common.h"
#include "kernels.h"
#if defined(XGP_DIVRCP)
#define SCORE_GRU_RCP(x) __frcp_rn(x)
#endif
#include "cell.h"

namespace {

typedef __bf16 bf16x8 __attribute__((ext_vector_type(8)));
typedef float f32x4 __attribute__((ext_vector_type(4)));

constexpr int XH = 128, XNW = 8, XRB = 16;
#ifndef XG_PREFETCH
#define XG_PREFETCH 3
#endif
constexpr int XKS = XH / 32;
constexpr int XLD = XH + 8;
constexpr int XLD2 = 2 * XH + 8;

#if defined(XGP_NOSTORE)
#define XG_STORE(lhs, v) do { if ((v) == 123.456f) lhs = (v); } while (0)
#else
#define XG_STORE(lhs, v) lhs = (v)
// ... 93 lines not shown
  float x[3][4];
  auto fetch_x = [&](int g, int t) {
    const int64_t u3 = ((int64_t)min(t, T - 1) * 3 * H + g * H) * 4;
#pragma unroll
    for (int r = 0; r < 4; ++r) x[g][r] = ldg(sd.xproj, u3, rb3[r]);
  };
  fetch_x(0, 0); fetch_x(1, 0); fetch_x(2, 0);
#if XG_PREFETCH
  const int pfl = min(lane, 23), pfL = wave * 24 + pfl;
  const uint32_t pfoff = (uint32_t)(((int64_t)min(b0 + pfL / 12, a.B - 1) * T * 3 * H) * 4 + (pfL % 12) * 128);
  float pfv = 0.f;
  uint32_t pfsink = 0;
#endif
  const int aoff = lc * XLD + 8 * lq;
  auto step = [&](const int t) {
    const int64_t u3 = (int64_t)t * 3 * H * 4;
#if XG_PREFETCH
    pfsink ^= __float_as_uint(pfv);
    pfv = ldg(sd.xproj, (int64_t)min(t + XG_PREFETCH, T - 1) * 3 * H * 4, pfoff);
#endif
    f32x4 ar = {0.f, 0.f, 0.f, 0.f}, au = {0.f, 0.f, 0.f, 0.f};
    {
      bf16x8 af[XKS][3];
#pragma unroll
      for (int s = 0; s < XKS; ++s) get3(hp, PS, aoff + 32 * s, af[s]);
#pragma unroll
      for (int s = 0; s < XKS; ++s) {
        ar = mfma6(af[s], wr[s], ar);
        au = mfma6(af[s], wu[s], au);
      }
    }
#pragma unroll
    for (int r = 0; r < 4; ++r) {
      const int i = lq * 4 + r;
      const float rg = gru_sigmoid(ar[r] + x[0][r]);
      if (rok[r]) XG_STORE(*stp(sd.gates, u3, rb3[r]), rg);
      put3(rp, PS, i * XLD + j, rg * h[r]);
    }
    fetch_x(0, t + 1);
    __syncthreads();
    f32x4 ac = {0.f, 0.f, 0.f, 0.f};
    float u[4];
    {
      bf16x8 af[XKS][3];
#pragma unroll
      for (int s = 0; s < XKS; ++s) get3(rp, PS, aoff + 32 * s, af[s]);
#pragma unroll
      for (int r = 0; r < 4; ++r) {
        u[r] = gru_sigmoid(au[r] + x[1][r]);
        if (rok[r]) XG_STORE(*stp(sd.gates, u3 + H * 4, rb3[r]), u[r]);
      }
      fetch_x(1, t + 1);
#pragma unroll
      for (int s = 0; s < XKS; ++s) ac = mfma6(af[s], wc[s], ac);
    }
#pragma unroll
    for (int r = 0; r < 4; ++r) {
      const int i = lq * 4 + r;
      const float c = gru_tanh(ac[r] + x[2][r]);
      const float hn = gru_blend(u[r], h[r], c);
      const bool live = t < len[r];
      if (rok[r]) {
        XG_STORE(*stp(sd.gates, u3 + 2 * H * 4, rb3[r]), c);
        XG_STORE(*stp(sd.out, (int64_t)t * sd.ldo * 4, rbo[r]), (live ? hn : 0.f));
      }
      h[r] = live ? hn : h[r];
      put3(hp, PS, i * XLD + j, h[r]);
    }
    fetch_x(2, t + 1);
    __syncthreads();
  };
  step(0);
  for (int t = 1; t < T; ++t) step(t);
#if XG_PREFETCH
  asm volatile("" : : "v"(pfsink ^ __float_as_uint(pfv)));
#endif
  if (sd.final_state) {
#pragma unroll
    for (int r = 0; r < 4; ++r)
      sd.final_state[(int64_t)min(b0 + lq * 4 + r, a.B - 1) * H + j] = h[r];
  }
}

__global__ __launch_bounds__(64 * XNW) void gru_bwd_x3_kernel(const GruArgs a) {
  constexpr int H = XH, PS = XRB * XLD, PS2 = XRB * XLD2;
  __shared__ __attribute__((aligned(16))) unsigned short dpc[3 * PS], dpg[3 * PS2];
  __shared__ float sbias[3][64 * XNW];
  const int tiles_b = (a.B + XRB - 1) / XRB;
  const int side = blockIdx.x / tiles_b;
  const GruSide& sd = a.s[side];
  const int b0 = (blockIdx.x - side * tiles_b) * XRB;
  const int tid = threadIdx.x, lane = tid & 63, wave = tid >> 6;
  sbias[0][tid] = 0.f; sbias[1][tid] = 0.f; sbias[2][tid] = 0.f;
  const int lc = lane & 15, lq = lane >> 4;
  const int T = a.T;
  const int j = wave * 16 + lc;

  bf16x8 wct[XKS][3], wgt[2 * XKS][3];
#pragma unroll
  for (int s = 0; s < 2 * XKS; ++s) {
    float xg[8];
#pragma unroll
    for (int jj = 0; jj < 8; ++jj) xg[jj] = sd.Wg[(int64_t)j * sd.ldwg + 32 * s + 8 * lq + jj];
    split8(xg, wgt[s]);
    if (s < XKS) {
      float xc[8];
#pragma unroll
      for (int jj = 0; jj < 8; ++jj) xc[jj] = sd.Wc[(int64_t)j * sd.ldwc + 32 * s + 8 * lq + jj];
      split8(xc, wct[s]);
    }
  }
  int len[4];
  bool rok[4];
  const int nreal = a.B - (b0 + lq * 4);
  uint32_t rb3[4], rbh[4], rbo[4], rbd[4];
  float dh[4];
  const bool want_bias = sd.bias_slab != nullptr;
#pragma unroll
  for (int r = 0; r < 4; ++r) {
    const int b = b0 + lq * 4 + r;
    rok[r] = true;
    const int bc = min(b, a.B - 1);
    len[r] = a.length[bc];
    rb3[r] = (uint32_t)(((int64_t)bc * T * 3 * H + j) * 4);
    rbh[r] = (uint32_t)(((int64_t)bc * T * H + j) * 4);
    rbo[r] = (uint32_t)(((int64_t)bc * T * sd.ldo + j) * 4);
    rbd[r] = (uint32_t)(((int64_t)bc * T * sd.lddo + j) * 4);
    dh[r] = (sd.dfinal && rok[r]) ? sd.dfinal[(int64_t)bc * H + j] : 0.f;
  }
  float n_u[4], n_c[4], n_r[4], n_hp[4], n_do[4];
  auto fetch_ucd = [&](int t) {
    const int64_t tc = max(t, 0);
#pragma unroll
    for (int r = 0; r < 4; ++r) {
      n_u[r] = ldg(sd.gates, (tc * 3 * H + H) * 4, rb3[r]); n_c[r] = ldg(sd.gates, (tc * 3 * H + 2 * H) * 4, rb3[r]);
      n_do[r] = ldg(sd.dout, tc * sd.lddo * 4, rbd[r]);
    }
  };
  auto fetch_r = [&](int t) {
    const int64_t tc = max(t, 0);
#pragma unroll
    for (int r = 0; r < 4; ++r) n_r[r] = ldg(sd.gates, tc * 3 * H * 4, rb3[r]);
  };
  auto fetch_hp = [&](int t) {
    const int64_t tp = max(t - 1, 0);
#pragma unroll
    for (int r = 0; r < 4; ++r) n_hp[r] = ldg(sd.out, tp * sd.ldo * 4, rbo[r]);
  };
  fetch_ucd(T - 1); fetch_r(T - 1); fetch_hp(T - 1);
  const int aoff = lc * XLD + 8 * lq, aoff2 = lc * XLD2 + 8 * lq;

  auto step = [&](const int t) {
    float c_hp[4];
#pragma unroll
    for (int r = 0; r < 4; ++r) c_hp[r] = (t < len[r] && t > 0) ? n_hp[r] : 0.f;
    __builtin_amdgcn_sched_barrier(0);
    fetch_hp(t - 1);
    float su = 0.f, sc = 0.f;
#pragma unroll
    for (int r = 0; r < 4; ++r) {
      const int i = lq * 4 + r;
      const bool live = t < len[r];
      const float u = n_u[r], c = n_c[r];
      const float d = dh[r] + n_do[r];
      const float dc = gru_dc(d, u), du = gru_du(d, c_hp[r], c);
      const float v_dpu = gru_dpu(du, u, live);
      const float v_dpc = gru_dpc(dc, c, live);
      dh[r] = live ? d * u : dh[r];
      su += r < nreal ? v_dpu : 0.f;
      sc += r < nreal ? v_dpc : 0.f;
      if (rok[r]) {
        XG_STORE(*stp(sd.hprev, (int64_t)t * H * 4, rbh[r]), c_hp[r]);
        XG_STORE(*stp(sd.dxproj, ((int64_t)t * 3 * H + H) * 4, rb3[r]), v_dpu);
        XG_STORE(*stp(sd.dxproj, ((int64_t)t * 3 * H + 2 * H) * 4, rb3[r]), v_dpc);
      }
      put3(dpc, PS, i * XLD + j, v_dpc);
      put3(dpg, PS2, i * XLD2 + H + j, v_dpu);
    }
    if (want_bias) { atomicAdd(&sbias[1][tid], su); atomicAdd(&sbias[2][tid], sc); }
    __builtin_amdgcn_sched_barrier(0);
    fetch_ucd(t - 1);
    __syncthreads();
    {
      f32x4 acc = {0.f, 0.f, 0.f, 0.f};
#pragma unroll
      for (int s = 0; s < XKS; ++s) {
        bf16x8 af[3];
        get3(dpc, PS, aoff + 32 * s, af);
        acc = mfma6(af, wct[s], acc);
      }
      float sr = 0.f;
#pragma unroll
      for (int r = 0; r < 4; ++r) {
        const int i = lq * 4 + r;
        const bool live = t < len[r];
        const float rr = live ? n_r[r] : 0.f, hp = c_hp[r];
        const float drh = acc[r];
        const float v_dpr = gru_dpr(drh, hp, rr, live);
        dh[r] += live ? drh * rr : 0.f;
        sr += r < nreal ? v_dpr : 0.f;
        if (rok[r]) {
          XG_STORE(*stp(sd.dxproj, (int64_t)t * 3 * H * 4, rb3[r]), v_dpr);
          XG_STORE(*stp(sd.rh, (int64_t)t * H * 4, rbh[r]), (rr * hp));
        }
        put3(dpg, PS2, i * XLD2 + j, v_dpr);
      }
      if (want_bias) atomicAdd(&sbias[0][tid], sr);
      __builtin_amdgcn_sched_barrier(0);
      fetch_r(t - 1);
    }
    __syncthreads();
    {
      f32x4 acc = {0.f, 0.f, 0.f, 0.f};
#pragma unroll
      for (int s = 0; s < 2 * XKS; ++s) {
        bf16x8 af[3];
        get3(dpg, PS2, aoff2 + 32 * s, af);
        acc = mfma6(af, wgt[s], acc);
      }
#pragma unroll
      for (int r = 0; r < 4; ++r) dh[r] += acc[r];
    }
    __syncthreads();
    };
  step(T - 1);
  for (int t = T - 2; t >= 0; --t) step(t);
  if (want_bias) {
    float sb_r = sbias[0][tid], sb_u = sbias[1][tid], sb_c = sbias[2][tid];
    sb_r += __shfl_xor(sb_r, 16, 64); sb_u += __shfl_xor(sb_u, 16, 64); sb_c += __shfl_xor(sb_c, 16, 64);
    sb_r += __shfl_xor(sb_r, 32, 64); sb_u += __shfl_xor(sb_u, 32, 64); sb_c += __shfl_xor(sb_c, 32, 64);
    if (lq == 0) {
      float* o = sd.bias_slab + (int64_t)(blockIdx.x - side * tiles_b) * 3 * H;
      o[j] = sb_r; o[H + j] = sb_u; o[2 * H + j] = sb_c;
    }
  }
}

}

bool score_gru_x3_ok(int H, int nw8) { return H == XH && nw8 != 0; }
static bool x3_fits(const GruArgs& a, int nsides) {
  int64_t ld = 3 * XH;
  for (int i = 0; i < nsides; ++i) ld = std::max<int64_t>(ld, std::max(a.s[i].ldo, a.s[i].lddo));
  return (int64_t)a.B * a.T * ld * 4 < ((int64_t)1 << 32);
}

int score_gru_fwd_x3(GruArgs& a, int nsides, hipStream_t s) {
  if (!score_gru_x3_ok(a.H, a.nw8) || a.B <= 0 || a.T <= 0 || !x3_fits(a, nsides)) return SCORE_E_SHAPE;
  dim3 grid(nsides * ((a.B + XRB - 1) / XRB));
  hipLaunchKernelGGL(gru_fwd_x3_kernel, grid, dim3(64 * XNW), 0, s, a);
  SCORE_CHECK_LAUNCH();
  return 0;
}

int score_gru_bwd_x3(GruArgs& a, int nsides, hipStream_t s) {
  if (!score_gru_x3_ok(a.H, a.nw8) || a.B <= 0 || a.T <= 0 || !x3_fits(a, nsides)) return SCORE_E_SHAPE;
  dim3 grid(nsides * ((a.B + XRB - 1) / XRB));
  hipLaunchKernelGGL(gru_bwd_x3_kernel, grid, dim3(64 * XNW), 0, s, a);
  SCORE_CHECK_LAUNCH();
  bool slabs = true;
  for (int i = 0; i < nsides; ++i) slabs = slabs && a.s[i].bias_slab != nullptr;
  a.bias_slab_rows = slabs ? (a.B + XRB - 1) / XRB : 0;
  return 0;
}
```

score_amd/csrc/head_fused.hip:

```cpp
#include "common.h"
#include "kernels.h"
#include "cell.h"
#include "head_tiles.h"

namespace {

struct HeadFwdArgs {
  int B, Dh, N1, N2, Bglobal;
  const float* x; const float* gamma; const float* beta; float rs;
  const float* W1; const float* b1; const float* W2; const float* b2; const float* W3; const float* b3;
  float keep; int drop; const uint8_t* mask0; const uint8_t* mask1; uint64_t seed0, seed1;
  const uint64_t* seed_dev;
  const int32_t* label;
  float* bn; float* f1; float* f2; float* logit; float* y; float* lossb; float* dlogit;
  float* dz2;
  int phase;
};

__global__ __launch_bounds__(64 * HF_NW) void head_fwd_fused_kernel(const HeadFwdArgs a) {
  extern __shared__ float sm[];
  const uint64_t seed0 = a.seed_dev ? *a.seed_dev : a.seed0;
  const uint64_t seed1 = a.seed_dev ? (seed0 ^ 0x5DEECE66Dull) : a.seed1;
  const int Dh = a.Dh, N1 = a.N1, N2 = a.N2;
  const int Kp0 = (Dh + 15) & ~15, LD0 = Kp0 + 4;
// ... 115 lines not shown
    if (n0[0] >= 0 && col < N2) {
      const float bias = bias2;
#pragma unroll
      for (int r = 0; r < 4; ++r) {
        const int i = lq * 4 + r, row = b0 + i;
        const float v = relu_dropout(acc[0][r], bias, a.drop, a.keep, a.mask1, seed1, row, col, N2);
        f2s[i * LD2 + col] = v;
        if (row < a.B) a.f2[(int64_t)row * N2 + col] = v;
      }
    }
  }
  __syncthreads();

  if (wave == 0) {
    const int i = lane >> 2, part = lane & 3;
    float s = 0.f;
    for (int n = part; n < N2; n += 4) s = fmaf(f2s[i * LD2 + n], a.W3[n], s);
    s += __shfl_xor(s, 1, 64);
    s += __shfl_xor(s, 2, 64);
    const int row = b0 + i;
    if (part == 0 && row < a.B) {
      const float z = s + a.b3[0];
      const float p = sigmoidf_(z);
      const float lab = (float)a.label[row];
      a.logit[row] = z;
      a.y[row] = p;
      a.lossb[row] = logloss_term(p, lab);
      const float dl = logloss_dlogit(p, lab, a.Bglobal);
      a.dlogit[row] = dl;
      xs[i] = dl;
    }
  }
  __syncthreads();
  if (a.dz2) {
    for (int e = tid; e < HF_ROWS * N2; e += 64 * HF_NW) {
      const int i = e / N2, n = e - i * N2, row = b0 + i;
      const float q = xs[i] * a.W3[n] / a.keep;
      if (row < a.B) a.dz2[(int64_t)row * N2 + n] = f2s[i * LD2 + n] > 0.f ? q : 0.f;
    }
  }
}


constexpr int AF_NW = 8;

struct AttnFwdArgs {
  int B, T, H, NI, N1, N2, S;
  const float* q; const float* ur; const float* ir; const float* info;
  const float* Weff; const float* qz;
  const float* W4; const float* b4; const float* w5; const float* b5; const int32_t* length;
  float* inp; float* a1; float* a2; float* score; float* head; int ldh, off_u, off_i;
  int wcopies; int64_t wstride;
};

__device__ __forceinline__ void af_build(const AttnFwdArgs& a, float* __restrict__ xs, int LD, int Kp, int row0,
                                         int row_end, int t0, int nthr) {
  const int Dk = 2 * a.H + a.NI, Dk4 = Dk >> 2, K2 = 2 * Dk;
  const int total = 16 * Dk4;
  constexpr int U = 4;
  for (int e0 = t0; e0 < total; e0 += U * nthr) {
    float4 k[U], qq[U];
    int ii[U], jj[U], gg[U];
    bool ok[U];
#pragma unroll
    for (int u = 0; u < U; ++u) {
      const int e = e0 + u * nthr;
      const int ec = e < total ? e : 0;
      ii[u] = ec / Dk4; jj[u] = (ec - ii[u] * Dk4) * 4;
      gg[u] = row0 + ii[u];
      ok[u] = e < total && gg[u] < row_end;
      const int g = gg[u] < row_end ? gg[u] : row_end - 1;
      const int j = jj[u];
      const float* src = j < a.H ? a.ur + (int64_t)g * a.H + j
                                 : (j < 2 * a.H ? a.ir + (int64_t)g * a.H + (j - a.H) : a.info + (int64_t)g * a.NI + (j - 2 * a.H));
      k[u] = ld4(src);
      qq[u] = ld4(a.q + (int64_t)(g / a.T) * Dk + j);
    }
#pragma unroll
    for (int u = 0; u < U; ++u) {
      if (e0 + u * nthr >= total) continue;
      float4 kk = k[u], qk = make_float4(qq[u].x * kk.x, qq[u].y * kk.y, qq[u].z * kk.z, qq[u].w * kk.w);
      if (ok[u]) {
#ifndef AFP_NOINP
        st4(a.inp + (int64_t)gg[u] * K2 + jj[u], kk);
        st4(a.inp + (int64_t)gg[u] * K2 + Dk + jj[u], qk);
#endif
      } else {
        kk = make_float4(0.f, 0.f, 0.f, 0.f); qk = kk;
      }
      *reinterpret_cast<float4*>(xs + ii[u] * LD + jj[u]) = kk;
      *reinterpret_cast<float4*>(xs + ii[u] * LD + Dk + jj[u]) = qk;
    }
  }
  for (int e = t0; e < 16 * (Kp - K2); e += nthr) {
    const int i = e / (Kp - K2), j = e - i * (Kp - K2);
    xs[i * LD + K2 + j] = 0.f;
  }
}

template <int KQ>
__global__ __launch_bounds__(64 * AF_NW) void attn_fwd_fused_kernel(const AttnFwdArgs a) {
  extern __shared__ float sm[];
  const int T = a.T, H = a.H, N1 = a.N1, N2 = a.N2;
  const int Dk = 2 * H + a.NI, K2 = 2 * Dk, Kp = 4 * KQ, LD = Kp + 4;
  const int L1 = N1 + 1, L2 = N2 + 1;
  float* xs0 = sm;
  float* xs1 = xs0 + 16 * LD;
  float* a1s = xs1 + 16 * LD;
  float* w4s = a1s + a.S * T * L1;
  float* a2s = w4s + N1 * N2;
  float* scs = a2s + a.S * T * L2;
  const int tid = threadIdx.x, lane = tid & 63, wave = tid >> 6;
  const int lc = lane & 15, lq = lane >> 4;
  const int b0 = blockIdx.x * a.S;
  const int ns = min(a.S, a.B - b0);
  const int row0 = b0 * T, row_end = row0 + ns * T;
  const int ntile = (ns * T + 15) >> 4;
  const int ntn = (N1 + 15) >> 4;

  float breg[KQ];
  if (wave < ntn) {
    const int col = wave * 16 + lc;
    const float* Wsrc = a.Weff + (int64_t)((blockIdx.x >> 3) % a.wcopies) * a.wstride;
#pragma unroll
    for (int s_ = 0; s_ < KQ; ++s_) {
      const int k = lq * KQ + s_;
#ifdef AFP_NOPRELOAD
      const float w = (float)(k + col) * 1e-3f;
#else
      const float w = Wsrc[(int64_t)(k < K2 ? k : K2 - 1) * N1 + (col < N1 ? col : N1 - 1)];
#endif
      breg[s_] = w * ((k < K2 && col < N1) ? 1.0f : 0.0f);
    }
  }
  for (int i = tid; i < N1 * N2; i += 64 * AF_NW) w4s[i] = a.W4[i];
  af_build(a, xs0, LD, Kp, row0, row_end, tid, 64 * AF_NW);
  __syncthreads();
  for (int m = 0; m < ntile; ++m) {
    float* xs = (m & 1) ? xs1 : xs0;
    if (wave < ntn) {
      hf_f32x4 acc[1] = {{0.f, 0.f, 0.f, 0.f}};
      const int n0[1] = {wave * 16};
      const float* xrow = xs + lc * LD + lq * KQ;
#ifndef AFP_NOMFMA
#ifdef AFP_TWOACC
      hf_f32x4 acc2 = {0.f, 0.f, 0.f, 0.f};
#pragma unroll
      for (int s4 = 0; s4 < KQ; s4 += 4) {
        const float4 av = *reinterpret_cast<const float4*>(xrow + s4);
        acc[0] = __builtin_amdgcn_mfma_f32_16x16x4f32(av.x, breg[s4 + 0], acc[0], 0, 0, 0);
        acc2 = __builtin_amdgcn_mfma_f32_16x16x4f32(av.y, breg[s4 + 1], acc2, 0, 0, 0);
        acc[0] = __builtin_amdgcn_mfma_f32_16x16x4f32(av.z, breg[s4 + 2], acc[0], 0, 0, 0);
        acc2 = __builtin_amdgcn_mfma_f32_16x16x4f32(av.w, breg[s4 + 3], acc2, 0, 0, 0);
      }
      acc[0] += acc2;
#else
#pragma unroll
      for (int s4 = 0; s4 < KQ; s4 += 4) {
        const float4 av = *reinterpret_cast<const float4*>(xrow + s4);
        acc[0] = __builtin_amdgcn_mfma_f32_16x16x4f32(av.x, breg[s4 + 0], acc[0], 0, 0, 0);
        acc[0] = __builtin_amdgcn_mfma_f32_16x16x4f32(av.y, breg[s4 + 1], acc[0], 0, 0, 0);
        acc[0] = __builtin_amdgcn_mfma_f32_16x16x4f32(av.z, breg[s4 + 2], acc[0], 0, 0, 0);
        acc[0] = __builtin_amdgcn_mfma_f32_16x16x4f32(av.w, breg[s4 + 3], acc[0], 0, 0, 0);
      }
#endif
#else
      acc[0][0] = xrow[0] * breg[0] + breg[KQ - 1];
#endif
// ... 255 lines not shown
          o.x = fmaf(d3.x, qq[u].x, d1.x) + pl[u].x * sc[u]; o.y = fmaf(d3.y, qq[u].y, d1.y) + pl[u].y * sc[u];
          o.z = fmaf(d3.z, qq[u].z, d1.z) + pl[u].z * sc[u]; o.w = fmaf(d3.w, qq[u].w, d1.w) + pl[u].w * sc[u];
          float* dst = j < H ? a.dur + (int64_t)gg[u] * H + j
                             : (j < 2 * H ? a.dir + (int64_t)gg[u] * H + (j - H) : a.dinfo + (int64_t)gg[u] * NI + (j - 2 * H));
          st4(dst, o);
          pr = make_float4(d3.x * kv[u].x, d3.y * kv[u].y, d3.z * kv[u].z, d3.w * kv[u].w);
        }
        *reinterpret_cast<float4*>(o1) = pr;
      }
    }
    __syncthreads();
    for (int e = tid; e < ns * Dk4; e += 64 * AF_NW) {
      const int s_ = e / Dk4, j = (e - s_ * Dk4) * 4;
      const int lo = max(0, s_ * T - m * 16), hi = min(16, (s_ + 1) * T - m * 16);
      if (lo < hi) {
        float4 acc = *reinterpret_cast<const float4*>(dqs + s_ * Dk + j);
        for (int i = lo; i < hi; ++i) {
          const float4 v = *reinterpret_cast<const float4*>(ot + i * LDO + j);
          acc.x += v.x; acc.y += v.y; acc.z += v.z; acc.w += v.w;
        }
        *reinterpret_cast<float4*>(dqs + s_ * Dk + j) = acc;
      }
    }
    __syncthreads();
  }
  for (int e = tid; e < ns * Dk4; e += 64 * AF_NW) {
    const int s_ = e / Dk4, j = (e - s_ * Dk4) * 4;
    st4(a.dq + (int64_t)(b0 + s_) * Dk + j, *reinterpret_cast<const float4*>(dqs + s_ * Dk + j));
  }
}


__global__ __launch_bounds__(64 * HF_NW) void head_bwd_fused_kernel(const HeadBwdArgs a) {
  head_bwd_body(a, (int)blockIdx.y, (int)gridDim.y);
}

}

bool score_head_fwd_fused_fits(int B, int Dh, int N1, int N2) {
  const int LD0 = ((Dh + 15) & ~15) + 4, LD1 = ((N1 + 15) & ~15) + 4, LD2 = ((N2 + 15) & ~15) + 4;
  return B > 0 && (size_t)HF_ROWS * (LD0 + LD1 + LD2) * sizeof(float) <= 150 * 1024;
}

int score_launch_head_fwd_fused(int B, int Dh, int N1, int N2, const float* x, const float* gamma, const float* beta,
                                float rs, const float* W1, const float* b1, const float* W2, const float* b2,
                                const float* W3, const float* b3, float keep, const uint8_t* mask0, const uint8_t* mask1,
                                uint64_t seed0, uint64_t seed1, const int32_t* label, float* bn, float* f1, float* f2,
                                float* logit, float* y, float* lossb, float* dlogit, int Bglobal, hipStream_t s,
                                const uint64_t* seed_dev, float* dz2, int single_launch) {
  const int LD0 = ((Dh + 15) & ~15) + 4, LD1 = ((N1 + 15) & ~15) + 4, LD2 = ((N2 + 15) & ~15) + 4;
  const size_t lds = (size_t)HF_ROWS * (LD0 + LD1 + LD2) * sizeof(float);
  if (!score_head_fwd_fused_fits(B, Dh, N1, N2)) return SCORE_E_SHAPE;
  static thread_local bool attr_set = false;
  if (!attr_set && lds > 48 * 1024) {
    hipError_t e = hipFuncSetAttribute(reinterpret_cast<const void*>(head_fwd_fused_kernel),
                                       hipFuncAttributeMaxDynamicSharedMemorySize, 150 * 1024);
    if (e != hipSuccess) return (int)e;
    attr_set = true;
  }
  HeadFwdArgs a;
  a.B = B; a.Dh = Dh; a.N1 = N1; a.N2 = N2; a.Bglobal = Bglobal;
  a.x = x; a.gamma = gamma; a.beta = beta; a.rs = rs;
  a.W1 = W1; a.b1 = b1; a.W2 = W2; a.b2 = b2; a.W3 = W3; a.b3 = b3;
  a.keep = keep; a.drop = keep < 1.f ? 1 : 0; a.mask0 = mask0; a.mask1 = mask1; a.seed0 = seed0; a.seed1 = seed1; a.seed_dev = seed_dev;
  a.label = label; a.bn = bn; a.f1 = f1; a.f2 = f2; a.logit = logit; a.y = y; a.lossb = lossb; a.dlogit = dlogit;
  a.dz2 = dz2;
  const int mt = (B + HF_ROWS - 1) / HF_ROWS, nt1 = (N1 + 15) >> 4;
  const bool split = !single_launch && nt1 >= 4 && mt >= 32;
  if (!split) {
    a.phase = 0;
    hipLaunchKernelGGL(head_fwd_fused_kernel, dim3(mt), dim3(64 * HF_NW), lds, s, a);
    SCORE_CHECK_LAUNCH();
    return 0;
  }
  a.phase = 1;
  hipLaunchKernelGGL(head_fwd_fused_kernel, dim3(mt, 4), dim3(64 * HF_NW), lds, s, a);
  SCORE_CHECK_LAUNCH();
  a.phase = 2;
  hipLaunchKernelGGL(head_fwd_fused_kernel, dim3(mt), dim3(64 * HF_NW), lds, s, a);
  SCORE_CHECK_LAUNCH();
  return 0;
}

int score_launch_attn_fwd_fused(int B, int T, int H, int NI, int N1, int N2, const float* q, const float* ur,
                                const float* ir, const float* info, const float* Weff, const float* qz, const float* W4,
                                const float* b4, const float* w5, const float* b5, const int32_t* length, float* inp,
                                float* a1, float* a2, float* score, float* head, int ldh, int off_u, int off_i,
                                hipStream_t s, int weff_copies, int64_t weff_copy_stride) {
  if (B <= 0 || T <= 0 || (H & 3) || (NI & 3) || N1 > 16 * 5 || N1 <= 0 || N2 <= 0 || (int64_t)B * T >= (1LL << 30))
    return SCORE_E_SHAPE;
  const int K2 = 2 * (2 * H + NI), Kp = (K2 + 15) & ~15, LD = Kp + 4;
  int S = B >= 4 * 256 ? 4 : B >= 2 * 256 ? 2 : 1;
  size_t lds = 0;
  for (; S >= 1; S >>= 1) {
    lds = ((size_t)2 * 16 * LD + (size_t)S * T * (N1 + 1) + (size_t)N1 * N2 + (size_t)S * T * (N2 + 1) + (size_t)S * T) * sizeof(float);
    if (lds <= 150 * 1024) break;
  }
  if (S < 1) return SCORE_E_SHAPE;
  const int kq = Kp / 4;
  if (kq != 148 && kq != 52 && kq != 44 && kq != 36 && kq != 84) return SCORE_E_SHAPE;
  static thread_local bool attr_set = false;
  if (!attr_set) {
    for (const void* f : {reinterpret_cast<const void*>(attn_fwd_fused_kernel<148>),
                          reinterpret_cast<const void*>(attn_fwd_fused_kernel<52>),
                          reinterpret_cast<const void*>(attn_fwd_fused_kernel<44>),
                          reinterpret_cast<const void*>(attn_fwd_fused_kernel<36>),
                          reinterpret_cast<const void*>(attn_fwd_fused_kernel<84>)}) {
      hipError_t e = hipFuncSetAttribute(f, hipFuncAttributeMaxDynamicSharedMemorySize, 150 * 1024);
      if (e != hipSuccess) return (int)e;
    }
    attr_set = true;
  }
  AttnFwdArgs a;
  a.B = B; a.T = T; a.H = H; a.NI = NI; a.N1 = N1; a.N2 = N2; a.S = S;
  a.q = q; a.ur = ur; a.ir = ir; a.info = info; a.Weff = Weff; a.qz = qz;
  a.W4 = W4; a.b4 = b4; a.w5 = w5; a.b5 = b5; a.length = length;
  a.inp = inp; a.a1 = a1; a.a2 = a2; a.score = score; a.head = head; a.ldh = ldh; a.off_u = off_u; a.off_i = off_i;
  a.wcopies = weff_copies > 0 ? weff_copies : 1; a.wstride = weff_copy_stride;
  const dim3 grid((B + S - 1) / S), block(64 * AF_NW);
  switch (Kp / 4) {
    case 148: hipLaunchKernelGGL(attn_fwd_fused_kernel<148>, grid, block, lds, s, a); break;
    case 52: hipLaunchKernelGGL(attn_fwd_fused_kernel<52>, grid, block, lds, s, a); break;
    case 44: hipLaunchKernelGGL(attn_fwd_fused_kernel<44>, grid, block, lds, s, a); break;
    case 36: hipLaunchKernelGGL(attn_fwd_fused_kernel<36>, grid, block, lds, s, a); break;
    case 84: hipLaunchKernelGGL(attn_fwd_fused_kernel<84>, grid, block, lds, s, a); break;
    default: return SCORE_E_SHAPE;
  }
  SCORE_CHECK_LAUNCH();
  return 0;
}

static bool ab_plan(int B, int T, int H, int NI, int N1, int N2, int ldh, int off_u, int off_i, bool pool, int* S_out,
                    size_t* lds_out) {
  const int Dk = 2 * H + NI, K2 = 2 * Dk;
  if (B <= 0 || T <= 0 || (H & 3) || (NI & 3) || N1 != 4 * AB_KQ || K2 > 16 * AF_NW * AB_NTW || (int64_t)B * T >= (1LL << 30) ||
      (ldh & 3) || (off_u >= 0 && (off_u & 3)) || (off_i >= 0 && (off_i & 3)) || (pool && N2 <= 0))
    return false;
  const int S = B >= 4 * 256 ? 4 : B >= 2 * 256 ? 2 : 1;
  const int RT = ((S * T + 15) >> 4) << 4;
  const size_t lds = ((size_t)RT * (N1 + 4) + (size_t)16 * (K2 + 4) + (size_t)S * Dk +
                      (pool ? (size_t)S * T + (size_t)S * T * (N2 + 1) + (size_t)N1 * (N2 + 1) : 0)) * sizeof(float);
  if (lds > 150 * 1024) return false;
  *S_out = S; *lds_out = lds;
  return true;
}
bool score_attn_inp_bwd_fused_fits(int B, int T, int H, int NI, int N1, int N2, int ldh, int off_u, int off_i, bool pool) {
  int S; size_t lds;
  return ab_plan(B, T, H, NI, N1, N2, ldh, off_u, off_i, pool, &S, &lds);
}

int score_launch_attn_inp_bwd_fused(int B, int T, int H, int NI, int N1, const float* da1, const float* Weff, const float* q,
                                    const float* ur, const float* ir, const float* info, const float* score,
                                    const float* dhead, int ldh, int off_u, int off_i, float* dur, float* dir, float* dinfo,
                                    float* dq, hipStream_t s, int N2, const float* a2, const float* a1, const float* w5,
                                    const float* W4, const int32_t* length, float* ds, float* da2, float* da1_out) {
  const int pool = a2 != nullptr;
  if (pool && (!a1 || !w5 || !W4 || !length || !ds || !da2 || !da1_out)) return SCORE_E_BADARG;
  int S; size_t lds;
  if (!ab_plan(B, T, H, NI, N1, N2, ldh, off_u, off_i, pool != 0, &S, &lds)) return SCORE_E_SHAPE;
  static thread_local bool attr_set = false;
  if (!attr_set) {
    hipError_t e = hipFuncSetAttribute(reinterpret_cast<const void*>(attn_inp_bwd_fused_kernel),
                                       hipFuncAttributeMaxDynamicSharedMemorySize, 150 * 1024);
    if (e != hipSuccess) return (int)e;
    attr_set = true;
  }
  AttnBwdArgs a;
  a.B = B; a.T = T; a.H = H; a.NI = NI; a.S = S;
  a.da1 = da1; a.Weff = Weff; a.q = q; a.ur = ur; a.ir = ir; a.info = info; a.score = score; a.dhead = dhead;
  a.ldh = ldh; a.off_u = off_u; a.off_i = off_i; a.dur = dur; a.dir = dir; a.dinfo = dinfo; a.dq = dq;
  a.pool = pool; a.N2 = pool ? N2 : 0; a.a2 = a2; a.a1 = a1; a.w5 = w5; a.W4 = W4; a.length = length; a.ds = ds; a.da2 = da2;
  a.da1_out = da1_out;
  hipLaunchKernelGGL(attn_inp_bwd_fused_kernel, dim3((B + S - 1) / S), dim3(64 * AF_NW), lds, s, a);
  SCORE_CHECK_LAUNCH();
  return 0;
}

int score_launch_head_bwd_fused(int B, int Dh, int N1, int N2, const float* dz2, const float* W2, const float* f1, float keep,
                                const float* W1, const float* x, const float* gamma, float rs, float* dz1, float* dbn,
                                float* dhead, float* tmp, hipStream_t s) {
  if (B <= 0 || Dh <= 0 || N1 != 200 || N2 != 80) return SCORE_E_SHAPE;
  HeadBwdArgs a;
  a.B = B; a.Dh = Dh; a.ld = Dh; a.dz2 = dz2; a.W2 = W2; a.f1 = f1; a.keep = keep; a.W1 = W1; a.x = x; a.gamma = gamma; a.rs = rs;
// ... 8 lines not shown
```

score_amd/csrc/kernels.h:

```cpp
#pragma once
#include "common.h"

#define GEMM_GROUP_MAX 16
struct GemmProb {
  const float* A; const float* B; float* C; float* slab;
  const float* bias;
  int M, N, K, lda, ldb, ldc, k_chunk, gx, gy, nblocks;
};
struct GemmGroup { int n; int total_blocks; GemmProb p[GEMM_GROUP_MAX]; };
enum { GF_BIAS = 1, GF_RELU = 2, GF_ACC = 4, GF_DROP = 8, GF_X3 = 16, GF_X3F = 32, GF_RELUGRAD = 64 };
__device__ __forceinline__ int64_t bias_index(int flags, int row, int col, int N) {
  const int g = flags >> 16;
  return g ? (int64_t)(row / g) * N + col : col;
}
__device__ __forceinline__ float gemm_epilogue(float v, int row, int col, int N, const float* bias, int flags,
                                               float keep, const uint8_t* mask, uint64_t seed) {
  if (flags & GF_BIAS) v += bias[bias_index(flags, row, col, N)];
  if (flags & GF_RELU) v = fmaxf(v, 0.f);
  if (flags & GF_DROP) {
    uint64_t e = (uint64_t)row * (uint64_t)N + (uint64_t)col;
    bool on = mask ? (mask[e] != 0) : (hash_uniform(seed, e) < keep);
    v = on ? v / keep : 0.f;
  }
  if (flags & GF_RELUGRAD) {
    const float y = reinterpret_cast<const float*>(mask)[(int64_t)row * N + col];
    v = y > 0.f ? v / keep : 0.f;
  }
  return v;
}
int score_launch_gemm_bf16x3(int trans, int wm, const GemmGroup& g, const float* bias, int flags, float keep,
                             const uint8_t* mask, uint64_t seed, hipStream_t s);
struct GemmQueueJob { const float* A; const float* B; float* C; int M, N, K, lda, ldb, ldc; };
struct GemmQueue { int n; GemmQueueJob j[2 * GEMM_GROUP_MAX]; };
int gemm_queue_add(GemmQueue* q, int M, int N, int K, const float* A, int lda, const float* B, int ldb, float* C,
                   int ldc);
struct ReduceJob { const float* slab; float* C; int ns, M, N, ldc, first_block, pad; };
struct ReduceGroup { int n; int blocks; ReduceJob j[2 * GEMM_GROUP_MAX]; };
struct ColsumJobs;
int gemm_queue_flush(GemmQueue* q, int x3, float* slab, int64_t slab_floats, hipStream_t s, ReduceGroup* defer = nullptr,
                     const ColsumJobs* with_colsums = nullptr, float* cs_part = nullptr, int64_t cs_part_floats = 0,
                     int* colsums_done = nullptr);
#define COLSUM_MAX_JOBS 24
#define COLSUM_MAX_PARTS 128
struct ColsumJob { const float* X; float* out; const float* scale; int M, N, ld, acc, cols, rpb, nparts; int64_t part_off; };
struct ColsumJobs { ColsumJob job[COLSUM_MAX_JOBS]; int n; int64_t part_used; };
int colsum_queue_add(ColsumJobs* q, const float* X, int M, int N, int ld, float* out, int acc, const float* scale = nullptr);
int colsum_queue_flush(ColsumJobs* q, float* part, int64_t part_floats, hipStream_t s);
struct W1Fold { int Dk, NA; const float* dweff; const float* dwq; float* gW1; const float* slab_e; const float* slab_q; int ns_e, ns_q; };
int score_launch_finish(const ReduceGroup* rg, ColsumJobs* q, float* part, int64_t part_floats, hipStream_t s, int stage1_done = 0,
                        const W1Fold* w1 = nullptr);
int score_launch_colsum(const float* X, int M, int N, int ld, float* out, int accumulate,
                        float* scratch, int64_t scratch_floats, hipStream_t s);
struct CoattnCall {
  const int32_t* idx1; const int32_t* idx2;
  const float* tgt; int ldt;
  const int32_t* tidx;
  const float* W; const float* bias;
  float* out1; int ld1; float* out2; int ld2;
  float* info; int ldi; float* rsave;
  const float* g1; const float* g2; const float* ginfo;
  float* dzsum; float* slab;
  float* pcoef; float* dzcoef;
  int F, GS, nslots, first_block;
  int bit1, bit2;
};
struct CoattnArgs {
  CoattnCall c[2];
  const float* table; float* gtable;
  int D4, K, T, n_units, mode;
  int Tidx;
  uint32_t n_rows; int32_t* id_status;
};
int score_coattn_fwd_multi(CoattnArgs& a, int ncalls, int D, int B, hipStream_t s);
int score_coattn_bwd_multi(CoattnArgs& a, int ncalls, int D, int B, float* const dW[2], float* scratch,
                           int64_t scratch_floats, int atomic_scatter, ColsumJobs* cq, hipStream_t s);
int score_launch_target_fwd(const float* table, int D, int Fu, int Fi, int B, const int32_t* tu,
                            const int32_t* ti, float* query, int ldq, float* head, int ldh,
                            int off_ti, int off_tu, hipStream_t s, int64_t n_rows = 0, int32_t* id_status = nullptr);
int score_launch_target_bwd(float* grad_table, int D, int Fu, int Fi, int B, int T, const int32_t* tu,
                            const int32_t* ti, const float* dquery, int ldq, const float* dhead, int ldh,
                            int off_ti, int off_tu, const float* query, const float* W1, const float* W2,
                            const float* dzsum1, const float* dzsum2, float* S ,
                            float* dW1, float* dB1, float* dW2, float* dB2, float* dtgt_out, float* scratch,
                            int64_t scratch_floats, ColsumJobs* cq, struct GemmQueue* gq, hipStream_t s,
                            int64_t n_rows = 0);
int score_launch_attn_build_inp(int B, int T, int H, int NI, const float* q, const float* ur, const float* ir,
                                const float* info, float* inp, hipStream_t s);
int score_launch_attn_pool_fwd(int B, int T, int H, int NA, const float* a2, const float* w5, const float* b5,
                               const int32_t* length, const float* ur, const float* ir, float* score, float* head,
                               int ldh, int off_u, int off_i, hipStream_t s);
int score_launch_attn_tail_fwd(int B, int T, int H, int N1, int N2, const float* a1, const float* W4, const float* b4,
                               const float* w5, const float* b5, const int32_t* length, const float* ur, const float* ir,
                               float* a2, float* score, float* head, int ldh, int off_u, int off_i, hipStream_t s);
int score_launch_attn_pool_bwd(int B, int T, int H, int NA, const float* a2, const float* w5,
                               const int32_t* length, const float* ur, const float* ir, const float* score,
                               const float* dhead, int ldh, int off_u, int off_i, float* ds, float* da2,
                               hipStream_t s, int N1 = 0, const float* W4 = nullptr, const float* a1 = nullptr,
                               float* da1 = nullptr);
int score_launch_attn_inp_bwd(int B, int T, int H, int NI, const float* dinp, const float* q, const float* ur,
                              const float* ir, const float* info, const float* score, const float* dhead, int ldh,
                              int off_u, int off_i, const float* dqd, float* dur, float* dir, float* dinfo, float* dq,
                              hipStream_t s);
int score_launch_attn_inp_bwd_fused(int B, int T, int H, int NI, int N1, const float* da1, const float* Weff, const float* q,
                                    const float* ur, const float* ir, const float* info, const float* score,
                                    const float* dhead, int ldh, int off_u, int off_i, float* dur, float* dir, float* dinfo,
                                    float* dq, hipStream_t s, int N2 = 0, const float* a2 = nullptr, const float* a1 = nullptr,
                                    const float* w5 = nullptr, const float* W4 = nullptr, const int32_t* length = nullptr,
                                    float* ds = nullptr, float* da2 = nullptr, float* da1_out = nullptr);
bool score_attn_inp_bwd_fused_fits(int B, int T, int H, int NI, int N1, int N2, int ldh, int off_u, int off_i, bool pool);
#define SCORE_WEFF_COPIES 8
int score_launch_attn_dzsum(int B, int T, int NA, const float* dz, float* dzsum, hipStream_t s);
int score_launch_attn_w1_grad(int Dk, int NA, const float* dweff, const float* dwq, float* gW1, hipStream_t s);
int score_launch_bn_fwd(int B, int Dh, const float* x, const float* gamma, const float* beta, float rs, float* y,
                        hipStream_t s);
int score_launch_bn_bwd(int B, int Dh, const float* x, const float* gamma, float rs, const float* dy, float* dx,
                        float* dgamma, float* dbeta, float* tmp, float* scratch, int64_t scratch_floats,
                        ColsumJobs* cq, hipStream_t s);
int score_launch_weight_prep(const float* gk0, const float* ck0, const float* gb0, const float* cb0, const float* gk1,
                             const float* ck1, const float* gb1, const float* cb1, int I0, int I1, int Imax, int H, float* cat,
                             int Dk, int NA, const float* W1, float* weff, float* wq, int copies, int64_t copy_stride,
                             const float* wreg, int64_t n_reg, float* part, hipStream_t s);
int score_launch_head_out(int B, int NF, const float* f2, const float* w3, const float* b3, const int32_t* label,
                          float* logit, float* y, float* lossb, float* dlogit, float* loss, float lambda,
                          const float* part, int Bglobal, hipStream_t s, const int32_t* id_status = nullptr);
int score_launch_loss_final(int B, const float* lossb, float* loss, float lambda, const float* part, int Bglobal,
                            hipStream_t s, const int32_t* id_status = nullptr);
int score_launch_head_fwd_fused(int B, int Dh, int N1, int N2, const float* x, const float* gamma, const float* beta,
                                float rs, const float* W1, const float* b1, const float* W2, const float* b2,
                                const float* W3, const float* b3, float keep, const uint8_t* mask0, const uint8_t* mask1,
                                uint64_t seed0, uint64_t seed1, const int32_t* label, float* bn, float* f1, float* f2,
                                float* logit, float* y, float* lossb, float* dlogit, int Bglobal, hipStream_t s,
                                const uint64_t* seed_dev = nullptr, float* dz2 = nullptr, int single_launch = 0);
bool score_head_fwd_fused_fits(int B, int Dh, int N1, int N2);
int score_launch_head_bwd_fused(int B, int Dh, int N1, int N2, const float* dz2, const float* W2, const float* f1, float keep,
                                const float* W1, const float* x, const float* gamma, float rs, float* dz1, float* dbn,
                                float* dhead, float* tmp, hipStream_t s);
int score_launch_attn_fwd_fused(int B, int T, int H, int NI, int N1, int N2, const float* q, const float* ur,
                                const float* ir, const float* info, const float* Weff, const float* qz, const float* W4,
                                const float* b4, const float* w5, const float* b5, const int32_t* length, float* inp,
                                float* a1, float* a2, float* score, float* head, int ldh, int off_u, int off_i,
                                hipStream_t s, int weff_copies = 1, int64_t weff_copy_stride = 0);
int score_launch_outer_relu_bwd(int B, int NF, const float* dlogit, const float* w, const float* f, float keep,
                                float* dz, hipStream_t s);
int score_launch_copy2d(int64_t rows, int cols, const float* src, int lds_, float* dst, int ldd, hipStream_t s);

struct PlanFillArgs {
  const int32_t* idx[6];
  int64_t off[7];
  int F[6];
  int K, G, shift;
  int T, TA;
  uint32_t n_rows;
  int32_t* id_status;
};
struct PullArgs {
  const float* G[6]; int ldg[6]; int gcol[6];
  const float* cA[6]; const float* cB[6];
  const float* Wv[6];
  float constA[6];
  const uint32_t* uid;
  int D, K, LPRp;
  int zero_is_dummy;
  uint8_t* flags;
};
struct PlanRemapArgs { int32_t* out[6]; int F[6]; int K; int T, TA; };
int score_launch_plan_unique(const PlanRemapArgs& ra, const uint32_t* keys, const uint32_t* vals, int64_t n,
                             uint32_t* flags_scratch, uint32_t* uid, uint32_t* unique_keys, int32_t* unique_rows,
                             int32_t* meta, int G, int shift, void* temp, size_t temp_bytes, hipStream_t s,
                             bool remap = true);
int score_scan_temp_bytes(int64_t n, size_t* bytes);
int score_plan_temp_bytes(int64_t n, int end_bit, size_t* bytes);
int score_launch_plan(const PlanFillArgs& a, int key_bits, uint32_t* keys_in, uint32_t* vals_in, uint32_t* keys_out,
                      uint32_t* vals_out, void* temp, size_t temp_bytes, hipStream_t s, int which = 0);
int score_launch_plan_own(const PlanFillArgs& a, int key_bits, uint32_t* keys_in, uint32_t* vals_in, uint32_t* keys_out,
                          uint32_t* vals_out, void* temp, size_t temp_bytes, hipStream_t s);
size_t score_sort_temp_bytes(int64_t n);
int score_pull_window(int64_t n);
int score_launch_pull(PullArgs& a, const uint32_t* keys, const uint32_t* vals, int64_t n, float* out,
                      float* partials, int64_t partial_floats, hipStream_t s);

struct GruSide {
  const float* xproj;
  const float* Wg; int ldwg;
  const float* Wc; int ldwc;
  float* out; int ldo;
  float* gates;
  float* final_state;
  const float* dout; int lddo;
  const float* dfinal;
  float* dxproj;
  float* rh;
  float* hprev;
  float* bias_slab;
  const int32_t* length;
};
struct GruArgs {
  GruSide s[2];
  const int32_t* length;
  int B, T, H;
  int nw8;
  float* tmp; int64_t tmp_floats; int x3; int stepwise;
  int x3_rec;
  int bias_slab_rows;
};
int score_gemm_same_shape(int trans, int nprob, int M, int N, int K, const float* const* A, int lda,
                          const float* const* B, int ldb, float* const* C, int ldc, int flags, int x3, float* scratch,
                          int64_t scratch_floats, hipStream_t s, const float* const* bias = nullptr);
struct PanelGroup { const float* A; const float* img; float* C; const float* bias; };
bool score_gemm_panel_ok(int ngroups, int M, int N, int K, int lda, int ldc, int* mt_out);
int64_t score_gemm_panel_image_floats(int N, int K);
int score_gemm_panel_prep(int nimg, const float* const* B, int ldb, int trans, int N, int K, float* const* img, hipStream_t s);
int score_gemm_panel(int ngroups, const PanelGroup* g, int M, int N, int K, int lda, int ldc, hipStream_t s);
bool score_gru_stream_ok(int H);
int64_t score_gru_stream_tmp_floats(int H, int nsides);
int score_gru_fwd_stream(GruArgs& a, int nsides, hipStream_t s);
int score_gru_bwd_stream(GruArgs& a, int nsides, hipStream_t s);
bool score_gru_x3_ok(int H, int nw8);
int score_gru_fwd_x3(GruArgs& a, int nsides, hipStream_t s);
int score_gru_bwd_x3(GruArgs& a, int nsides, hipStream_t s);
int score_gru_fwd_multi(GruArgs& a, int nsides, hipStream_t s);
int score_gru_bwd_multi(GruArgs& a, int nsides, hipStream_t s);
bool score_gru_reg_route(const GruArgs& a, int nsides);
int score_launch_gcmc_head_fwd(int B, int H, const float* hu, const float* hi, const float* W4, const float* W5,
                               const int32_t* label, float* y, float* lossb, float* p, float* n, float* g, int Bglobal,
// ... 75 lines not shown
```

Before: 909,300.

## Recompute attention-input and GRU hprev/rh rows inside weight-gradient GEMM loads

Adds a 'view' mode to the bf16x3 weight-gradient GEMM, so its A operand is rebuilt on the fly from the source tensors. The attention input rows come from q, the GRU outputs and info, and the GRU hprev and r*h rows come from out, gates and length. The forward attention kernel no longer stores ainp, and the GRU backward kernel skips writing the hprev/rh buffers. This removes large intermediate writes and reads, at the cost of extra index math and gathered loads inside the GEMM tile loader. The path runs by default, and new debug flags restore the stored-operand path.

```diff
diff --git a/include/score_hip.h b/include/score_hip.h
--- a/include/score_hip.h
+++ b/include/score_hip.h
@@ -123,6 +123,11 @@
                float* C, int32_t ldc, const float* bias, int32_t flags,
                float keep_prob, const uint8_t* drop_mask, uint64_t drop_seed,
                float* scratch, int64_t scratch_floats, void* stream);
+
+int score_gemm_tn_view(int32_t kind, int32_t M, int32_t N, int32_t K, int32_t T, int32_t H, int32_t NI,
+                       const float* p0, const float* p1, const float* p2, const float* q, const int32_t* length,
+                       int32_t ldo, const float* A, const float* Bm, int32_t ldb, float* C, int32_t ldc, int32_t x3,
+                       float* scratch, int64_t scratch_floats, int32_t* used_view, void* stream);
 
 int score_gemm_panel_products(int32_t trans_b, int32_t ngroups, int32_t M, int32_t N, int32_t K,
                               const float* const* A, int32_t lda, const float* const* Bm, int32_t ldb,
diff --git a/score_amd/_lib.py b/score_amd/_lib.py
--- a/score_amd/_lib.py
+++ b/score_amd/_lib.py
@@ -11,6 +11,10 @@
 
 c_f = C.c_void_p
 c_i = C.c_void_p
+
+DF_STORED_OPERANDS = 32768
+DF_STORED_ATTN_ROWS = 65536
+DF_STORED_GRU_ROWS = 131072
 
 
 class Config(C.Structure):
@@ -105,6 +109,9 @@
                          C.c_int32, C.c_void_p],
     "score_gemm": [C.c_int32, C.c_int32, C.c_int32, C.c_int32, c_f, C.c_int32, c_f, C.c_int32, c_f, C.c_int32,
                    c_f, C.c_int32, C.c_float, C.c_void_p, C.c_uint64, c_f, C.c_int64, C.c_void_p],
+    "score_gemm_tn_view": [C.c_int32, C.c_int32, C.c_int32, C.c_int32, C.c_int32, C.c_int32, C.c_int32, c_f, c_f, c_f, c_f, c_i,
+                           C.c_int32, c_f, c_f, C.c_int32, c_f, C.c_int32, C.c_int32, c_f, C.c_int64, C.POINTER(C.c_int32),
+                           C.c_void_p],
     "score_gemm_panel_images": [C.c_int32, C.c_int32, C.c_int32, C.c_int32, C.c_void_p, C.c_int32, c_f, C.c_int64, C.c_void_p],
     "score_gemm_panel_run": [C.c_int32, C.c_int32, C.c_int32, C.c_int32, C.c_void_p, C.c_int32, C.c_void_p, C.c_int32, C.c_void_p,
                              c_f, C.c_int64, C.c_void_p],
diff --git a/score_amd/csrc/engine.hip b/score_amd/csrc/engine.hip
--- a/score_amd/csrc/engine.hip
+++ b/score_amd/csrc/engine.hip
@@ -503,11 +503,12 @@
 enum {
   DF_GRU_STEPWISE = 1, DF_HEAD_FUSED_ANY_B = 2, DF_GRU_F32_REC = 4, DF_NO_PANEL = 8, DF_PANEL_DX = 16, DF_SORT_LIB = 32,
   DF_HEAD_UNFUSED = 64, DF_ATTN_UNFUSED = 128, DF_SORT_OWN = 256, DF_NO_PS = 512, DF_PS_FWD_ONLY = 1024, DF_PS_BWD_ONLY = 2048,
-  DF_ONE_STREAM = 4096, DF_G4R_COMPOSED = 8192, DF_PRODUCTS_LATE = 16384
+  DF_ONE_STREAM = 4096, DF_G4R_COMPOSED = 8192, DF_PRODUCTS_LATE = 16384, DF_STORED_OPERANDS = 32768,
+  DF_STORED_ATTN_ROWS = 65536, DF_STORED_GRU_ROWS = 131072
 };
 struct Flags {
   bool gru_stepwise, head_fused_any_b, gru_f32_rec, no_panel, panel_dx, sort_lib, head_unfused, attn_unfused, sort_own, no_ps,
-      ps_fwd_only, ps_bwd_only, one_stream, g4r_composed, products_late;
+      ps_fwd_only, ps_bwd_only, one_stream, g4r_composed, products_late, stored_attn_rows, stored_gru_rows;
 };
 static inline Flags flags_of(const score_state_t* st) {
   auto on = [st](int bit) { return (st->debug_flags & bit) != 0; };
@@ -517,6 +518,8 @@
   o.head_unfused = on(DF_HEAD_UNFUSED); o.attn_unfused = on(DF_ATTN_UNFUSED); o.no_ps = on(DF_NO_PS);
   o.ps_fwd_only = on(DF_PS_FWD_ONLY); o.ps_bwd_only = on(DF_PS_BWD_ONLY); o.one_stream = on(DF_ONE_STREAM);
   o.g4r_composed = on(DF_G4R_COMPOSED); o.products_late = on(DF_PRODUCTS_LATE);
+  o.stored_attn_rows = on(DF_STORED_OPERANDS) || on(DF_STORED_ATTN_ROWS);
+  o.stored_gru_rows = on(DF_STORED_OPERANDS) || on(DF_STORED_GRU_ROWS);
   return o;
 }
 static int side_stream(const score_state_t* st, hipStream_t s, SideStream** out) {
@@ -899,13 +902,18 @@
   G(colsum_queue_add(&q->cq, a.dbn + t.col, B, t.Dh, ld, gw + v.bn_b, 0));
   return 0;
 }
-static int queue_attn(const Pass& c, GradQueues* q, float* gw) {
+static int queue_attn(const Pass& c, GradQueues* q, float* gw, bool view = false) {
   const Dims& d = c.d; const Params& P = c.P; const WS& w = c.w; float* ws = c.ws; const int B = c.B, BT = c.BT;
   G(gemm_queue_add(&q->gq, AT2, 1, BT, ws + w.a2, AT2, ws + w.ds, 1, gw + P.at_w[3], 1));
   G(colsum_queue_add(&q->cq, ws + w.ds, BT, 1, 1, gw + P.at_b[3], 0));
   G(gemm_queue_add(&q->gq, AT1, AT2, BT, ws + w.a1, AT1, ws + w.da2, AT2, gw + P.at_w[2], AT2));
   G(colsum_queue_add(&q->cq, ws + w.da2, BT, AT2, AT2, gw + P.at_b[2], 0));
-  G(gemm_queue_add(&q->gq, 2 * d.Dk, AT1, BT, ws + w.ainp, 2 * d.Dk, ws + w.da1, AT1, ws + w.dweff, AT1));
+  if (view)
+    G(gemm_queue_add_view(&q->gq, c.x3 != 0, 2 * d.Dk, AT1, BT,
+                          gemm_view_attn_rows(c.T, c.H, d.NI, ws + w.q, ws + w.gru_out[0], ws + w.gru_out[1], ws + w.info),
+                          ws + w.da1, AT1, ws + w.dweff, AT1));
+  else
+    G(gemm_queue_add(&q->gq, 2 * d.Dk, AT1, BT, ws + w.ainp, 2 * d.Dk, ws + w.da1, AT1, ws + w.dweff, AT1));
   G(colsum_queue_add(&q->cq, ws + w.da1, BT, AT1, AT1, gw + P.at_b[1], 0));
   G(gemm_queue_add(&q->gq, d.Dk, AT1, B, ws + w.q, d.Dk, ws + w.adzsum, AT1, ws + w.dwq, AT1));
   return 0;
@@ -916,15 +924,23 @@
   G(colsum_queue_add(&q->cq, c.ws + w.dq, c.B, d.Dk, d.Dk, gw + P.at_b[0], 0));
   return 0;
 }
-static int queue_gru_side(const Pass& c, GradQueues* q, float* gw, int sd, int bias_rows) {
+static int queue_gru_side(const Pass& c, GradQueues* q, float* gw, int sd, int bias_rows, bool views = false) {
   const Dims& d = c.d; const Params& P = c.P; const WS& w = c.w; float* ws = c.ws;
   const int H = c.H, BT = c.BT, Is = d.Is[sd], ld = x_ld(d, sd);
   float* dxp = ws + w.dxproj[sd];
   const float* xin = gru_x_rows(c, sd);
   G(gemm_queue_add(&q->gq, Is, 2 * H, BT, xin, ld, dxp, 3 * H, gw + P.gk[sd], 2 * H));
   G(gemm_queue_add(&q->gq, Is, H, BT, xin, ld, dxp + 2 * H, 3 * H, gw + P.ck[sd], H));
-  G(gemm_queue_add(&q->gq, H, 2 * H, BT, ws + w.hprev[sd], H, dxp, 3 * H, gw + P.gk[sd] + (int64_t)Is * 2 * H, 2 * H));
-  G(gemm_queue_add(&q->gq, H, H, BT, ws + w.rh[sd], H, dxp + 2 * H, 3 * H, gw + P.ck[sd] + (int64_t)Is * H, H));
+  if (views) {
+    const float* out = ws + w.gru_out[sd];
+    G(gemm_queue_add_view(&q->gq, c.x3 != 0, H, 2 * H, BT, gemm_view_hprev(c.T, H, out, H, c.bt->length), dxp, 3 * H,
+                          gw + P.gk[sd] + (int64_t)Is * 2 * H, 2 * H));
+    G(gemm_queue_add_view(&q->gq, c.x3 != 0, H, H, BT, gemm_view_rh(c.T, H, ws + w.gates[sd], out, H, c.bt->length), dxp + 2 * H,
+                          3 * H, gw + P.ck[sd] + (int64_t)Is * H, H));
+  } else {
+    G(gemm_queue_add(&q->gq, H, 2 * H, BT, ws + w.hprev[sd], H, dxp, 3 * H, gw + P.gk[sd] + (int64_t)Is * 2 * H, 2 * H));
+    G(gemm_queue_add(&q->gq, H, H, BT, ws + w.rh[sd], H, dxp + 2 * H, 3 * H, gw + P.ck[sd] + (int64_t)Is * H, H));
+  }
   const float* rows = bias_rows > 0 ? gru_bias_slab(c, sd) : dxp;
   const int nrows = bias_rows > 0 ? bias_rows : BT;
   G(colsum_queue_add(&q->cq, rows, nrows, 2 * H, 3 * H, gw + P.gb[sd], 0));
@@ -1376,6 +1392,33 @@
   return 0;
 }
 
+static bool views_possible(const Pass& c) {
+  if (c.d.family != FAM_SLICE || !c.d.attn || c.st->scatter_mode == 2) return false;
+  PsPlan pp;
+  return !ps_path(c.d, c.st, c.bt, c.T, &pp);
+}
+static bool attn_rows_as_view(const Pass& c) {
+  const Dims& d = c.d; const WS& w = c.w;
+  if (!views_possible(c) || c.fl.stored_attn_rows || c.fl.attn_unfused) return false;
+  if (!score_attn_fwd_fused_fits(c.B, c.T, c.H, d.NI, AT1, AT2)) return false;
+  return gemm_queue_view_ok(c.x3 != 0, 2 * d.Dk, AT1, c.BT, c.ws + w.da1, AT1,
+                            gemm_view_attn_rows(c.T, c.H, d.NI, c.ws + w.q, c.ws + w.gru_out[0], c.ws + w.gru_out[1], c.ws + w.info));
+}
+static bool gru_rows_as_views(const Pass& c) {
+  const WS& w = c.w; const int H = c.H;
+  if (!views_possible(c) || c.fl.stored_gru_rows) return false;
+  GruArgs ga;
+  gru_header(c, &ga);
+  if (!ga.x3_rec || !score_gru_x3_ok(H, ga.nw8)) return false;
+  for (int sd = 0; sd < 2; ++sd) {
+    const float* out = c.ws + w.gru_out[sd]; const float* dxp = c.ws + w.dxproj[sd];
+    if (!gemm_queue_view_ok(c.x3 != 0, H, 2 * H, c.BT, dxp, 3 * H, gemm_view_hprev(c.T, H, out, H, c.bt->length)) ||
+        !gemm_queue_view_ok(c.x3 != 0, H, H, c.BT, dxp + 2 * H, 3 * H, gemm_view_rh(c.T, H, c.ws + w.gates[sd], out, H, c.bt->length)))
+      return false;
+  }
+  return true;
+}
+
 int fwd_grus_two_sided(const Pass& c, const FwdState& f, const float* const* xin) {
   const Dims& d = c.d; const WS& w = c.w; float* ws = c.ws; const int H = c.H, BT = c.BT, x3 = c.x3; hipStream_t s = c.s;
   GruArgs ga;
@@ -1409,7 +1452,8 @@
   int frc = c.fl.attn_unfused ? SCORE_E_SHAPE
                 : score_launch_attn_fwd_fused(B, T, H, d.NI, AT1, AT2, ws + w.q, ws + w.gru_out[0], ws + w.gru_out[1],
                                               ws + w.info, ws + w.weff, ws + w.qz, W + P.at_w[2], W + P.at_b[2],
-                                              W + P.at_w[3], W + P.at_b[3], bt->length, ws + w.ainp, ws + w.a1, ws + w.a2,
+                                              W + P.at_w[3], W + P.at_b[3], bt->length,
+                                              attn_rows_as_view(c) ? nullptr : ws + w.ainp, ws + w.a1, ws + w.a2,
                                               ws + w.att_score, ws + w.head_inp, d.Dhead, d.off_u, d.off_i, s,
                                               SCORE_WEFF_COPIES, c.weff_stride);
   if (frc != SCORE_E_SHAPE) return frc;
@@ -1673,7 +1717,7 @@
   const Dims& d = c.d; const Params& P = c.P; const WS& w = c.w; const score_batch_t* bt = c.bt;
   float* ws = c.ws; const float* W = c.W; const int B = c.B, T = c.T, H = c.H, BT = c.BT, x3 = c.x3; hipStream_t s = c.s;
   const int64_t SF = w.scratch_floats;
-  G(queue_attn(c, &b->q, b->gw));
+  G(queue_attn(c, &b->q, b->gw, attn_rows_as_view(c)));
   const bool pool_in_fused = !c.fl.attn_unfused && (int64_t)B * T < 8192 &&
                              score_attn_inp_bwd_fused_fits(B, T, H, d.NI, AT1, AT2, d.Dhead, d.off_u, d.off_i, true);
   int prc = pool_in_fused ? 0 : c.fl.attn_unfused ? SCORE_E_SHAPE
@@ -1756,9 +1800,11 @@
 int bwd_grus_two_sided(const Pass& c, BwdState* b) {
   GruArgs ga;
   gru_header(c, &ga);
+  const bool views = gru_rows_as_views(c);
   for (int sd = 0; sd < 2; ++sd) {
     gru_side(c, sd, &ga.s[sd]);
     gru_side_bwd(c, sd, b->dfinal[sd], &ga.s[sd]);
+    if (views) ga.s[sd].hprev = ga.s[sd].rh = nullptr;
   }
   G(score_gru_bwd_multi(ga, 2, c.s));
   b->gru_bias_rows = ga.bias_slab_rows;
@@ -1768,8 +1814,9 @@
 int bwd_dx_slice(const Pass& c, BwdState* b) {
   const Dims& d = c.d; const WS& w = c.w; float* ws = c.ws; const int H = c.H, BT = c.BT, x3 = c.x3; hipStream_t s = c.s;
   const int64_t SF = w.scratch_floats;
+  const bool views = gru_rows_as_views(c);
   for (int sd = 0; sd < 2; ++sd) {
-    G(queue_gru_side(c, &b->q, b->gw, sd, b->gru_bias_rows));
+    G(queue_gru_side(c, &b->q, b->gw, sd, b->gru_bias_rows, views));
     if (d.Is[sd] != d.I)
       HIPTRY(hipMemsetAsync(ws + w.dxside[sd], 0, (int64_t)BT * d.I * sizeof(float), s));
     if (d.Is[0] != d.Is[1])
diff --git a/score_amd/csrc/gemm.hip b/score_amd/csrc/gemm.hip
--- a/score_amd/csrc/gemm.hip
+++ b/score_amd/csrc/gemm.hip
@@ -209,6 +209,7 @@
                       int ldc, int k_chunk, float* slab, int gx, int gy, int gz) {
   p->A = A; p->B = B; p->C = C; p->slab = slab; p->bias = nullptr; p->M = M; p->N = N; p->K = K; p->lda = lda; p->ldb = ldb;
   p->ldc = ldc; p->k_chunk = k_chunk; p->gx = gx; p->gy = gy; p->nblocks = gx * gy * gz;
+  memset(&p->v, 0, sizeof(p->v));
 }
 
 extern "C" int score_gemm(int32_t trans, int32_t M, int32_t N, int32_t K, const float* A, int32_t lda,
@@ -375,6 +376,95 @@
   if (q->n >= 2 * GEMM_GROUP_MAX) return SCORE_E_WORKSPACE;
   GemmQueueJob& j = q->j[q->n++];
   j.A = A; j.B = B; j.C = C; j.M = M; j.N = N; j.K = K; j.lda = lda; j.ldb = ldb; j.ldc = ldc;
+  memset(&j.v, 0, sizeof(j.v));
+  return 0;
+}
+
+static GemmView view_base(int kind, int T, int H) {
+  GemmView v;
+  memset(&v, 0, sizeof(v));
+  v.kind = kind; v.T = T; v.H = H;
+  v.tmagic = T > 1 ? (uint32_t)((1ull << 32) / (uint64_t)T) + 1u : 0u;
+  return v;
+}
+GemmView gemm_view_attn_rows(int T, int H, int NI, const float* q, const float* ur, const float* ir, const float* info) {
+  GemmView v = view_base(GV_ATTN_ROWS, T, H);
+  v.NI = NI; v.q = q; v.p0 = ur; v.p1 = ir; v.p2 = info;
+  return v;
+}
+GemmView gemm_view_hprev(int T, int H, const float* out, int ldo, const int32_t* len) {
+  GemmView v = view_base(GV_HPREV, T, H);
+  v.p0 = out; v.ldo = ldo; v.len = len;
+  return v;
+}
+GemmView gemm_view_rh(int T, int H, const float* gates, const float* out, int ldo, const int32_t* len) {
+  GemmView v = view_base(GV_RH, T, H);
+  v.p0 = out; v.p1 = gates; v.ldo = ldo; v.len = len;
+  return v;
+}
+bool gemm_queue_job_x3(int x3, int M, int N, int K, const float* A, int lda, const float* B, int ldb) {
+  const bool al = (lda & 3) == 0 && (ldb & 3) == 0 && (reinterpret_cast<uintptr_t>(A) & 15) == 0 &&
+                  (reinterpret_cast<uintptr_t>(B) & 15) == 0 && (M & 3) == 0 && (N & 3) == 0;
+  return x3 && al && M >= 64 && N >= 32 && (int64_t)M * N >= 16384 && K >= 4096;
+}
+static inline bool al16(const void* p) { return p && (reinterpret_cast<uintptr_t>(p) & 15) == 0; }
+static bool view_shape_ok(int M, int K, const GemmView& v) {
+  const int T = v.T, H = v.H;
+  if (T <= 0 || H <= 0 || (H & 3) || K % T != 0 || (int64_t)K * T >= (1ll << 32)) return false;
+  if (v.kind == GV_ATTN_ROWS) {
+    const int Dk = 2 * H + v.NI;
+    return v.NI > 0 && (v.NI & 3) == 0 && M == 2 * Dk && al16(v.p0) && al16(v.p1) && al16(v.p2) && al16(v.q) &&
+           (int64_t)K * (H > v.NI ? H : v.NI) < (1ll << 31);
+  }
+  if (v.kind == GV_HPREV || v.kind == GV_RH)
+    return M == H && v.ldo >= H && (v.ldo & 3) == 0 && al16(v.p0) && v.len && (v.kind == GV_HPREV || al16(v.p1)) &&
+           (int64_t)K * (v.ldo > 3 * H ? v.ldo : 3 * H) < (1ll << 31);
+  return false;
+}
+bool gemm_queue_view_ok(int x3, int M, int N, int K, const float* B, int ldb, const GemmView& v) {
+  return gemm_queue_job_x3(x3, M, N, K, nullptr, 0, B, ldb) && view_shape_ok(M, K, v);
+}
+int gemm_queue_add_view(GemmQueue* q, int x3, int M, int N, int K, const GemmView& v, const float* B, int ldb, float* C, int ldc) {
+  if (!q || !B || !C || M <= 0 || N <= 0 || K <= 0) return SCORE_E_BADARG;
+  if (!gemm_queue_view_ok(x3, M, N, K, B, ldb, v)) return SCORE_E_SHAPE;
+  if (q->n >= 2 * GEMM_GROUP_MAX) return SCORE_E_WORKSPACE;
+  GemmQueueJob& j = q->j[q->n++];
+  j.A = nullptr; j.B = B; j.C = C; j.M = M; j.N = N; j.K = K; j.lda = 0; j.ldb = ldb; j.ldc = ldc;
+  j.v = v;
+  return 0;
+}
+__global__ void view_rows_kernel(const GemmView v, int M, int K, float* __restrict__ dst, int ld) {
+  const int M4 = M >> 2;
+  const int64_t i = (int64_t)blockIdx.x * blockDim.x + threadIdx.x;
+  if (i >= (int64_t)K * M4) return;
+  const int g = (int)(i / M4), c = (int)(i - (int64_t)g * M4) * 4;
+  const int b = g / v.T, t = g - b * v.T, H = v.H;
+  float4 x;
+  if (v.kind == GV_ATTN_ROWS) {
+    const int Dk = 2 * H + v.NI, j = c >= Dk ? c - Dk : c;
+    x = ld4(j < H ? v.p0 + (int64_t)g * H + j : j < 2 * H ? v.p1 + (int64_t)g * H + (j - H) : v.p2 + (int64_t)g * v.NI + (j - 2 * H));
+    if (c >= Dk) {
+      const float4 qq = ld4(v.q + (int64_t)b * Dk + j);
+      x = make_float4(qq.x * x.x, qq.y * x.y, qq.z * x.z, qq.w * x.w);
+    }
+  } else {
+    const int len = v.len[b];
+    const float4 o = ld4(v.p0 + (int64_t)(g > 0 ? g - 1 : 0) * v.ldo + c);
+    const bool ok = t < len && t > 0;
+    x = make_float4(ok ? o.x : 0.f, ok ? o.y : 0.f, ok ? o.z : 0.f, ok ? o.w : 0.f);
+    if (v.kind == GV_RH) {
+      const float4 r = ld4(v.p1 + (int64_t)g * 3 * H + c);
+      const bool live = t < len;
+      x = make_float4((live ? r.x : 0.f) * x.x, (live ? r.y : 0.f) * x.y, (live ? r.z : 0.f) * x.z, (live ? r.w : 0.f) * x.w);
+    }
+  }
+  st4(dst + (int64_t)g * ld + c, x);
+}
+int score_launch_view_rows(const GemmView& v, int M, int K, float* dst, int ld, hipStream_t s) {
+  if (!dst || M <= 0 || K <= 0 || (ld & 3) || ld < M || !al16(dst) || !view_shape_ok(M, K, v)) return SCORE_E_SHAPE;
+  const int64_t n = (int64_t)K * (M >> 2);
+  hipLaunchKernelGGL(view_rows_kernel, dim3((unsigned)cdiv64(n, 256)), dim3(256), 0, s, v, M, K, dst, ld);
+  SCORE_CHECK_LAUNCH();
   return 0;
 }
 
@@ -391,9 +481,8 @@
   int64_t work[2] = {0, 0};
   for (int i = 0; i < q->n; ++i) {
     const GemmQueueJob& j = q->j[i];
-    const bool al = (j.lda & 3) == 0 && (j.ldb & 3) == 0 && (reinterpret_cast<uintptr_t>(j.A) & 15) == 0 &&
-                    (reinterpret_cast<uintptr_t>(j.B) & 15) == 0 && (j.M & 3) == 0 && (j.N & 3) == 0;
-    fam[i] = (x3 && al && j.M >= 64 && j.N >= 32 && (int64_t)j.M * j.N >= 16384 && j.K >= 4096) ? 1 : 0;
+    fam[i] = gemm_queue_job_x3(x3, j.M, j.N, j.K, j.A, j.lda, j.B, j.ldb) ? 1 : 0;
+    if (j.v.kind != GV_NONE && !fam[i]) return SCORE_E_SHAPE;
     const int64_t tiles = fam[i] ? (int64_t)((j.M + 127) / 128) * ((j.N + 127) / 128)
                                  : (int64_t)((j.M + 63) / 64) * ((j.N + 63) / 64);
     work[fam[i]] += tiles * j.K;
@@ -440,6 +529,7 @@
       chunk = j.K;
     }
     fill_prob(&g.p[g.n], j.M, j.N, j.K, j.A, j.lda, j.B, j.ldb, j.C, j.ldc, chunk, sl, gx, gy, ns);
+    g.p[g.n].v = j.v;
     g.total_blocks += (g.p[g.n].nblocks + 7) & ~7;
     ++g.n;
   }
@@ -467,6 +557,39 @@
   }
   q->n = 0;
   return 0;
+}
+
+extern "C" int score_gemm_tn_view(int32_t kind, int32_t M, int32_t N, int32_t K, int32_t T, int32_t H, int32_t NI, const float* p0,
+                                  const float* p1, const float* p2, const float* q, const int32_t* length, int32_t ldo,
+                                  const float* A, const float* Bm, int32_t ldb, float* C, int32_t ldc, int32_t x3, float* scratch,
+                                  int64_t scratch_floats, int32_t* used_view, void* stream) {
+  if (!Bm || !C || !scratch || M <= 0 || N <= 0 || K <= 0 || T <= 0 || H <= 0) return SCORE_E_BADARG;
+  if ((reinterpret_cast<uintptr_t>(scratch) & 15) != 0) return SCORE_E_BADARG;
+  hipStream_t s = (hipStream_t)stream;
+  if (used_view) *used_view = 0;
+  GemmQueue gq;
+  gq.n = 0;
+  int64_t used = 0;
+  if (A) {
+    SCORE_TRY(gemm_queue_add(&gq, M, N, K, A, M, Bm, ldb, C, ldc));
+  } else {
+    GemmView v;
+    if (kind == GV_ATTN_ROWS) v = gemm_view_attn_rows(T, H, NI, q, p0, p1, p2);
+    else if (kind == GV_HPREV) v = gemm_view_hprev(T, H, p0, ldo, length);
+    else if (kind == GV_RH) v = gemm_view_rh(T, H, p1, p0, ldo, length);
+    else return SCORE_E_BADARG;
+    if (gemm_queue_view_ok(x3, M, N, K, Bm, ldb, v)) {
+      SCORE_TRY(gemm_queue_add_view(&gq, x3, M, N, K, v, Bm, ldb, C, ldc));
+      if (used_view) *used_view = 1;
+    } else {
+      used = align_up64((int64_t)K * M, 4);
+      if (used > scratch_floats) return SCORE_E_WORKSPACE;
+      SCORE_TRY(score_launch_view_rows(v, M, K, scratch, M, s));
+      SCORE_TRY(gemm_queue_add(&gq, M, N, K, scratch, M, Bm, ldb, C, ldc));
+    }
+  }
+  if (scratch_floats - used < (int64_t)M * N) return SCORE_E_WORKSPACE;
+  return gemm_queue_flush(&gq, x3, scratch + used, scratch_floats - used, s);
 }
 
 __global__ __launch_bounds__(256) void colsum_stage1(const float* __restrict__ X, int M, int N, int ld, int cols,
diff --git a/score_amd/csrc/gemm_bf16x3.hip b/score_amd/csrc/gemm_bf16x3.hip
--- a/score_amd/csrc/gemm_bf16x3.hip
+++ b/score_amd/csrc/gemm_bf16x3.hip
@@ -1,4 +1,5 @@
 #include <type_traits>
+#include <utility>
 #include "common.h"
 #include "kernels.h"
 
@@ -8,6 +9,9 @@
 #define TBN 128
 #define TBK 32
 #define TLD 40
+
+template <class F, int... G>
+__device__ __forceinline__ void slots(F& f, std::integer_sequence<int, G...>) { (f(G), ...); }
 
 template <int TRANS, int WM>
 __global__ __launch_bounds__(256, 2) void gemm_bf16x3_kernel(const GemmGroup grp, const float* __restrict__ bias, int flags,
@@ -69,6 +73,32 @@
       kb4[rep] = (tid & 7) * 4 + rep;
     }
   }
+  constexpr bool CAN_VIEW = (TRANS == 2 && WM == 2);
+  const int vkind = CAN_VIEW ? pr.v.kind : GV_NONE;
+  const int vT = pr.v.T;
+  const uint32_t vmagic = pr.v.tmagic;
+  const int32_t* __restrict__ vlenp = pr.v.len;
+  const float* vsrc = nullptr;
+  const float* vsrc2 = nullptr;
+  uint32_t vld = 0, vld2 = 0;
+  bool vsecond = false;
+  float xq[16];
+  int vlen[4];
+  if (CAN_VIEW && vkind != GV_NONE) {
+    const int c0 = min(bm + (tid >> 3) * 4, M - 4), vH = pr.v.H;
+    if (vkind == GV_ATTN_ROWS) {
+      const int Dk = 2 * vH + pr.v.NI;
+      vsecond = c0 >= Dk;
+      const int j = vsecond ? c0 - Dk : c0;
+      vsrc = j < vH ? pr.v.p0 + j : j < 2 * vH ? pr.v.p1 + (j - vH) : pr.v.p2 + (j - 2 * vH);
+      vld = j < 2 * vH ? vH : pr.v.NI;
+      vsrc2 = pr.v.q + j; vld2 = Dk;
+    } else {
+      vsrc = pr.v.p0 + c0; vld = pr.v.ldo;
+      vsrc2 = pr.v.p1 + c0; vld2 = 3 * vH;
+    }
+  }
+  auto view_b = [&](int g) -> uint32_t { return vT == 1 ? (uint32_t)g : __umulhi((uint32_t)g, vmagic); };
   constexpr int NQ = NA4 + 4;
   auto quad_src = [&](int qd, int e) -> float& {
     if (qd < NA4) return A_KCONTIG ? xa[qd * 4 + e] : xa[e * 4 + qd];
@@ -82,8 +112,25 @@
     if (qd < NA4) return A_KCONTIG ? pa[p * 2 * NA4 + qd * 2 + d] : pa[p * 8 + qd * 2 + d];
     return B_KCONTIG ? pb[p * 8 + (qd - NA4) * 2 + d] : pb[p * 8 + (qd - NA4) * 2 + d];
   };
-  auto load_one = [&](int which, int rep, int k0, auto kcheck) {
+  auto load_one = [&](int which, int rep, int k0, auto kcheck, auto vw) __attribute__((always_inline)) {
     constexpr bool KCHECK = decltype(kcheck)::value;
+    if (decltype(vw)::value && which == 0) {
+      int g = k0 + ka[rep];
+      if (KCHECK) g = min(g, K - 1);
+      const uint32_t b = view_b(g);
+      float4 v, w = make_float4(0.f, 0.f, 0.f, 0.f);
+      if (vkind == GV_ATTN_ROWS) {
+        v = ld4(vsrc + (uint32_t)g * vld);
+        if (vsecond) w = ld4(vsrc2 + b * vld2);
+      } else {
+        v = ld4(vsrc + (uint32_t)max(g - 1, 0) * vld);
+        vlen[rep] = vlenp[b];
+        if (vkind == GV_RH) w = ld4(vsrc2 + (uint32_t)g * vld2);
+      }
+      xa[rep * 4] = v.x; xa[rep * 4 + 1] = v.y; xa[rep * 4 + 2] = v.z; xa[rep * 4 + 3] = v.w;
+      xq[rep * 4] = w.x; xq[rep * 4 + 1] = w.y; xq[rep * 4 + 2] = w.z; xq[rep * 4 + 3] = w.w;
+      return;
+    }
     const bool kc = which == 0 ? A_KCONTIG : B_KCONTIG;
     const float* X = which == 0 ? A : Bm;
     const int ld = which == 0 ? lda : ldb;
@@ -103,16 +150,39 @@
     float* dst = which == 0 ? &xa[rep * 4] : &xb[rep * 4];
     dst[0] = v.x; dst[1] = v.y; dst[2] = v.z; dst[3] = v.w;
   };
-  auto load_all = [&](int k0, auto kcheck) {
-#pragma unroll
-    for (int rep = 0; rep < NA4; ++rep) load_one(0, rep, k0, kcheck);
-#pragma unroll
-    for (int rep = 0; rep < 4; ++rep) load_one(1, rep, k0, kcheck);
+  auto load_all = [&](int k0, auto kcheck, auto vw) __attribute__((always_inline)) {
+#pragma unroll
+    for (int rep = 0; rep < NA4; ++rep) load_one(0, rep, k0, kcheck, vw);
+#pragma unroll
+    for (int rep = 0; rep < 4; ++rep) load_one(1, rep, k0, kcheck, vw);
+  };
+  auto view_combine = [&](int k1, auto kcheck) __attribute__((always_inline)) {
+    constexpr bool KCHECK = decltype(kcheck)::value;
+    if (vkind == GV_ATTN_ROWS) {
+      if (vsecond) {
+#pragma unroll
+        for (int i = 0; i < 16; ++i) xa[i] = xq[i] * xa[i];
+      }
+      return;
+    }
+#pragma unroll
+    for (int e = 0; e < 4; ++e) {
+      int g = k1 + ka[e < NA4 ? e : 0];
+      if (KCHECK) g = min(g, K - 1);
+      const int t = g - (int)view_b(g) * vT;
+      const bool live = t < vlen[e], ok = live && t > 0;
+#pragma unroll
+      for (int c = 0; c < 4; ++c) {
+        const float hp = ok ? xa[e * 4 + c] : 0.f;
+        xa[e * 4 + c] = vkind == GV_RH ? (live ? xq[e * 4 + c] : 0.f) * hp : hp;
+      }
+    }
   };
   uint32_t sh[4], sm[4], sl[4];
-  auto split_micro = [&](int m, int k1, int k2, auto kcheck) {
+  auto split_micro = [&](int m, int k1, int k2, auto kcheck, auto vw) __attribute__((always_inline)) {
     constexpr bool KCHECK = decltype(kcheck)::value;
     const int qd = m / 5, step = m % 5;
+    if (decltype(vw)::value && m == 0) view_combine(k1, kcheck);
     if (step < 4) {
       float x = quad_src(qd, step);
       if (KCHECK) x = (k1 + quad_k(qd, step) < kend) ? x : 0.f;
@@ -125,10 +195,10 @@
         const bool is_a = qd < NA4;
         const bool kc = is_a ? A_KCONTIG : B_KCONTIG;
         if (kc) {
-          load_one(is_a ? 0 : 1, is_a ? qd : qd - NA4, k2, kcheck);
+          load_one(is_a ? 0 : 1, is_a ? qd : qd - NA4, k2, kcheck, vw);
         } else if (qd == (is_a ? NA4 - 1 : NQ - 1)) {
 #pragma unroll
-          for (int rep = 0; rep < 4; ++rep) load_one(is_a ? 0 : 1, rep, k2, kcheck);
+          for (int rep = 0; rep < 4; ++rep) load_one(is_a ? 0 : 1, rep, k2, kcheck, vw);
         }
       }
     } else {
@@ -137,7 +207,7 @@
       quad_dst(qd, 2, 0) = pack2(sl[0], sl[1]); quad_dst(qd, 2, 1) = pack2(sl[2], sl[3]);
     }
   };
-  auto write_tiles = [&]() {
+  auto write_tiles = [&]() __attribute__((always_inline)) {
 #ifdef X3_PROBE_NOLDSW
     if (pa[0] != 0x12345678u || pb[0] != 0x12345678u) return;
 #endif
@@ -193,7 +263,7 @@
   constexpr int NF1 = 3 * (WM + 2);
   constexpr int MU = NQ * 5;
   bf16x8 af[KS][WM][3], bf[KS][2][3];
-  auto read_frag = [&](int ks, int f) {
+  auto read_frag = [&](int ks, int f) __attribute__((always_inline)) {
     const int p = f / (WM + 2), i = f % (WM + 2);
 #ifdef X3_PROBE_NOLDSR
     {
@@ -210,15 +280,14 @@
       bf[ks][i - WM][p] = __builtin_bit_cast(bf16x8, vb);
     }
   };
-  auto phase = [&](int k0, auto kcheck) {
+  auto phase = [&](int k0, auto kcheck, auto vw) __attribute__((always_inline)) {
     constexpr int TA[6] = {1, 0, 2, 0, 1, 0}, TB[6] = {1, 2, 0, 1, 0, 0};
 #pragma unroll
     for (int f = 0; f < NF1; ++f) read_frag(0, f);
 #ifdef X3_SETPRIO
     __builtin_amdgcn_s_setprio(X3_SETPRIO);
 #endif
-#pragma unroll
-    for (int g = 0; g < NM; ++g) {
+    auto slot = [&](const int g) __attribute__((always_inline)) {
       const int ks = g / NM1, t = (g % NM1) / (WM * 2), i = (g / 2) % WM, j = g % 2;
       if (KS > 1 && g >= NM1 - NF1 - 2 && g < NM1 - 2) read_frag(1, g - (NM1 - NF1 - 2));
 #ifdef X3_PROBE_NOMFMA
@@ -227,8 +296,14 @@
       acc[i][j] = __builtin_amdgcn_mfma_f32_32x32x16_bf16(af[ks][i][TA[t]], bf[ks][j][TB[t]], acc[i][j], 0, 0, 0);
 #endif
 #pragma unroll
-      for (int m = g * MU / NM; m < (g + 1) * MU / NM; ++m) split_micro(m, k0 + TBK, k0 + 2 * TBK, kcheck);
+      for (int m = g * MU / NM; m < (g + 1) * MU / NM; ++m) split_micro(m, k0 + TBK, k0 + 2 * TBK, kcheck, vw);
       __builtin_amdgcn_sched_barrier(0);
+    };
+    if constexpr (decltype(vw)::value) {
+      slots(slot, std::make_integer_sequence<int, NM>());
+    } else {
+#pragma unroll
+      for (int g = 0; g < NM; ++g) slot(g);
     }
 #ifdef X3_SETPRIO
     __builtin_amdgcn_s_setprio(0);
@@ -236,25 +311,30 @@
   };
 
   const int nfull = (kend - kbeg) / TBK;
-  load_all(kbeg, std::true_type());
-#pragma unroll
-  for (int m = 0; m < MU; ++m) {
-    const int qd = m / 5, step = m % 5;
-    (void)qd; (void)step;
-    split_micro(m, kbeg, kbeg + TBK, std::true_type());
-  }
-  int k0 = kbeg;
-  for (int t = 0; t + 2 < nfull; ++t, k0 += TBK) {
-    write_tiles();
-    __syncthreads();
-    phase(k0, std::false_type());
-    __syncthreads();
-  }
-  for (; k0 < kend; k0 += TBK) {
-    write_tiles();
-    __syncthreads();
-    phase(k0, std::true_type());
-    __syncthreads();
+  auto run = [&](auto vw) __attribute__((always_inline)) {
+    load_all(kbeg, std::true_type(), vw);
+#pragma unroll
+    for (int m = 0; m < MU; ++m)
+      split_micro(m, kbeg, kbeg + TBK, std::true_type(), vw);
+    int k0 = kbeg;
+    for (int t = 0; t + 2 < nfull; ++t, k0 += TBK) {
+      write_tiles();
+      __syncthreads();
+      phase(k0, std::false_type(), vw);
+      __syncthreads();
+    }
+    for (; k0 < kend; k0 += TBK) {
+      write_tiles();
+      __syncthreads();
+      phase(k0, std::true_type(), vw);
+      __syncthreads();
+    }
+  };
+  if constexpr (CAN_VIEW) {
+    if (vkind != GV_NONE) run(std::true_type());
+    else run(std::false_type());
+  } else {
+    run(std::false_type());
   }
 
 #pragma unroll
diff --git a/score_amd/csrc/gru_x3.hip b/score_amd/csrc/gru_x3.hip
--- a/score_amd/csrc/gru_x3.hip
+++ b/score_amd/csrc/gru_x3.hip
@@ -199,6 +199,7 @@
   }
 }
 
+template <bool SAVE_H>
 __global__ __launch_bounds__(64 * XNW) void gru_bwd_x3_kernel(const GruArgs a) {
   constexpr int H = XH, PS = XRB * XLD, PS2 = XRB * XLD2;
   __shared__ __attribute__((aligned(16))) unsigned short dpc[3 * PS], dpg[3 * PS2];
@@ -287,7 +288,7 @@
       su += r < nreal ? v_dpu : 0.f;
       sc += r < nreal ? v_dpc : 0.f;
       if (rok[r]) {
-        XG_STORE(*stp(sd.hprev, (int64_t)t * H * 4, rbh[r]), c_hp[r]);
+        if (SAVE_H) XG_STORE(*stp(sd.hprev, (int64_t)t * H * 4, rbh[r]), c_hp[r]);
         XG_STORE(*stp(sd.dxproj, ((int64_t)t * 3 * H + H) * 4, rb3[r]), v_dpu);
         XG_STORE(*stp(sd.dxproj, ((int64_t)t * 3 * H + 2 * H) * 4, rb3[r]), v_dpc);
       }
@@ -318,7 +319,7 @@
         sr += r < nreal ? v_dpr : 0.f;
         if (rok[r]) {
           XG_STORE(*stp(sd.dxproj, (int64_t)t * 3 * H * 4, rb3[r]), v_dpr);
-          XG_STORE(*stp(sd.rh, (int64_t)t * H * 4, rbh[r]), (rr * hp));
+          if (SAVE_H) XG_STORE(*stp(sd.rh, (int64_t)t * H * 4, rbh[r]), (rr * hp));
         }
         put3(dpg, PS2, i * XLD2 + j, v_dpr);
       }
@@ -373,7 +374,11 @@
 int score_gru_bwd_x3(GruArgs& a, int nsides, hipStream_t s) {
   if (!score_gru_x3_ok(a.H, a.nw8) || a.B <= 0 || a.T <= 0 || !x3_fits(a, nsides)) return SCORE_E_SHAPE;
   dim3 grid(nsides * ((a.B + XRB - 1) / XRB));
-  hipLaunchKernelGGL(gru_bwd_x3_kernel, grid, dim3(64 * XNW), 0, s, a);
+  int nsave = 0;
+  for (int i = 0; i < nsides; ++i) nsave += (a.s[i].hprev != nullptr) + (a.s[i].rh != nullptr);
+  if (nsave != 0 && nsave != 2 * nsides) return SCORE_E_BADARG;
+  if (nsave) hipLaunchKernelGGL(gru_bwd_x3_kernel<true>, grid, dim3(64 * XNW), 0, s, a);
+  else hipLaunchKernelGGL(gru_bwd_x3_kernel<false>, grid, dim3(64 * XNW), 0, s, a);
   SCORE_CHECK_LAUNCH();
   bool slabs = true;
   for (int i = 0; i < nsides; ++i) slabs = slabs && a.s[i].bias_slab != nullptr;
diff --git a/score_amd/csrc/head_fused.hip b/score_amd/csrc/head_fused.hip
--- a/score_amd/csrc/head_fused.hip
+++ b/score_amd/csrc/head_fused.hip
@@ -221,8 +221,10 @@
       float4 kk = k[u], qk = make_float4(qq[u].x * kk.x, qq[u].y * kk.y, qq[u].z * kk.z, qq[u].w * kk.w);
       if (ok[u]) {
 #ifndef AFP_NOINP
-        st4(a.inp + (int64_t)gg[u] * K2 + jj[u], kk);
-        st4(a.inp + (int64_t)gg[u] * K2 + Dk + jj[u], qk);
+        if (a.inp) {
+          st4(a.inp + (int64_t)gg[u] * K2 + jj[u], kk);
+          st4(a.inp + (int64_t)gg[u] * K2 + Dk + jj[u], qk);
+        }
 #endif
       } else {
         kk = make_float4(0.f, 0.f, 0.f, 0.f); qk = kk;
@@ -644,13 +646,9 @@
   return 0;
 }
 
-int score_launch_attn_fwd_fused(int B, int T, int H, int NI, int N1, int N2, const float* q, const float* ur,
-                                const float* ir, const float* info, const float* Weff, const float* qz, const float* W4,
-                                const float* b4, const float* w5, const float* b5, const int32_t* length, float* inp,
-                                float* a1, float* a2, float* score, float* head, int ldh, int off_u, int off_i,
-                                hipStream_t s, int weff_copies, int64_t weff_copy_stride) {
+static bool af_plan(int B, int T, int H, int NI, int N1, int N2, int* S_out, size_t* lds_out) {
   if (B <= 0 || T <= 0 || (H & 3) || (NI & 3) || N1 > 16 * 5 || N1 <= 0 || N2 <= 0 || (int64_t)B * T >= (1LL << 30))
-    return SCORE_E_SHAPE;
+    return false;
   const int K2 = 2 * (2 * H + NI), Kp = (K2 + 15) & ~15, LD = Kp + 4;
   int S = B >= 4 * 256 ? 4 : B >= 2 * 256 ? 2 : 1;
   size_t lds = 0;
@@ -658,9 +656,25 @@
     lds = ((size_t)2 * 16 * LD + (size_t)S * T * (N1 + 1) + (size_t)N1 * N2 + (size_t)S * T * (N2 + 1) + (size_t)S * T) * sizeof(float);
     if (lds <= 150 * 1024) break;
   }
-  if (S < 1) return SCORE_E_SHAPE;
+  if (S < 1) return false;
   const int kq = Kp / 4;
-  if (kq != 148 && kq != 52 && kq != 44 && kq != 36 && kq != 84) return SCORE_E_SHAPE;
+  if (kq != 148 && kq != 52 && kq != 44 && kq != 36 && kq != 84) return false;
+  *S_out = S; *lds_out = lds;
+  return true;
+}
+bool score_attn_fwd_fused_fits(int B, int T, int H, int NI, int N1, int N2) {
+  int S; size_t lds;
+  return af_plan(B, T, H, NI, N1, N2, &S, &lds);
+}
+
+int score_launch_attn_fwd_fused(int B, int T, int H, int NI, int N1, int N2, const float* q, const float* ur,
+                                const float* ir, const float* info, const float* Weff, const float* qz, const float* W4,
+                                const float* b4, const float* w5, const float* b5, const int32_t* length, float* inp,
+                                float* a1, float* a2, float* score, float* head, int ldh, int off_u, int off_i,
+                                hipStream_t s, int weff_copies, int64_t weff_copy_stride) {
+  int S; size_t lds;
+  if (!af_plan(B, T, H, NI, N1, N2, &S, &lds)) return SCORE_E_SHAPE;
+  const int K2 = 2 * (2 * H + NI), Kp = (K2 + 15) & ~15;
   static thread_local bool attr_set = false;
   if (!attr_set) {
     for (const void* f : {reinterpret_cast<const void*>(attn_fwd_fused_kernel<148>),
diff --git a/score_amd/csrc/kernels.h b/score_amd/csrc/kernels.h
--- a/score_amd/csrc/kernels.h
+++ b/score_amd/csrc/kernels.h
@@ -2,10 +2,17 @@
 #include "common.h"
 
 #define GEMM_GROUP_MAX 16
+enum { GV_NONE = 0, GV_ATTN_ROWS = 1, GV_HPREV = 2, GV_RH = 3 };
+struct GemmView {
+  const float* p0; const float* p1; const float* p2; const float* q; const int32_t* len;
+  int kind, T, H, NI, ldo;
+  uint32_t tmagic;
+};
 struct GemmProb {
   const float* A; const float* B; float* C; float* slab;
   const float* bias;
   int M, N, K, lda, ldb, ldc, k_chunk, gx, gy, nblocks;
+  GemmView v;
 };
 struct GemmGroup { int n; int total_blocks; GemmProb p[GEMM_GROUP_MAX]; };
 enum { GF_BIAS = 1, GF_RELU = 2, GF_ACC = 4, GF_DROP = 8, GF_X3 = 16, GF_X3F = 32, GF_RELUGRAD = 64 };
@@ -30,10 +37,17 @@
 }
 int score_launch_gemm_bf16x3(int trans, int wm, const GemmGroup& g, const float* bias, int flags, float keep,
                              const uint8_t* mask, uint64_t seed, hipStream_t s);
-struct GemmQueueJob { const float* A; const float* B; float* C; int M, N, K, lda, ldb, ldc; };
+struct GemmQueueJob { const float* A; const float* B; float* C; int M, N, K, lda, ldb, ldc; GemmView v; };
 struct GemmQueue { int n; GemmQueueJob j[2 * GEMM_GROUP_MAX]; };
 int gemm_queue_add(GemmQueue* q, int M, int N, int K, const float* A, int lda, const float* B, int ldb, float* C,
                    int ldc);
+GemmView gemm_view_attn_rows(int T, int H, int NI, const float* q, const float* ur, const float* ir, const float* info);
+GemmView gemm_view_hprev(int T, int H, const float* out, int ldo, const int32_t* len);
+GemmView gemm_view_rh(int T, int H, const float* gates, const float* out, int ldo, const int32_t* len);
+bool gemm_queue_job_x3(int x3, int M, int N, int K, const float* A, int lda, const float* B, int ldb);
+bool gemm_queue_view_ok(int x3, int M, int N, int K, const float* B, int ldb, const GemmView& v);
+int gemm_queue_add_view(GemmQueue* q, int x3, int M, int N, int K, const GemmView& v, const float* B, int ldb, float* C, int ldc);
+int score_launch_view_rows(const GemmView& v, int M, int K, float* dst, int ld, hipStream_t s);
 struct ReduceJob { const float* slab; float* C; int ns, M, N, ldc, first_block, pad; };
 struct ReduceGroup { int n; int blocks; ReduceJob j[2 * GEMM_GROUP_MAX]; };
 struct ColsumJobs;
@@ -140,6 +154,7 @@
                                 const float* b4, const float* w5, const float* b5, const int32_t* length, float* inp,
                                 float* a1, float* a2, float* score, float* head, int ldh, int off_u, int off_i,
                                 hipStream_t s, int weff_copies = 1, int64_t weff_copy_stride = 0);
+bool score_attn_fwd_fused_fits(int B, int T, int H, int NI, int N1, int N2);
 int score_launch_outer_relu_bwd(int B, int NF, const float* dlogit, const float* w, const float* f, float keep,
                                 float* dz, hipStream_t s);
 int score_launch_copy2d(int64_t rows, int cols, const float* src, int lds_, float* dst, int ldd, hipStream_t s);
```

Result: no change. 914,200, median of 6 (+0.5%).
